# geometrian/simple-spectral

Hardware: AMD Instinct MI355X
Metric: Msamples/s (w*h*spp/s) cornell-srgb 512x512 (higher is better)
Workload: dtype f32

## Files before the change

include/ssx.h:

```cpp
#ifndef SSX_H
#define SSX_H

#include <stddef.h>
#include <stdint.h>

#ifdef __cplusplus
extern "C" {
#endif

#define SSX_ABI_VERSION 2

enum {
	SSX_OK = 0,
	SSX_ERR_DATA = -1,
	SSX_ERR_ARG = -2,
	SSX_ERR_SCENE = -3,
	SSX_ERR_DEVICE = -10,
	SSX_ERR_STATE = -11
};

#define SSX_MAX_DEPTH 10u
#define SSX_TILE_SIZE 8u
#define SSX_SAMPLE_WAVELENGTHS 4u
#define SSX_MAX_TEXTURES 64u
// ... 86 lines not shown
enum { SSX_LIBM_BUILD = 0, SSX_LIBM_GLIBC_2_35 = 1 };


typedef struct ssx_ctx ssx_ctx;

int ssx_create(int device, ssx_ctx** out);
void ssx_destroy(ssx_ctx* ctx);

int ssx_upload_scene(ssx_ctx* ctx, const ssx_scene_desc* scene);

int ssx_render_start(ssx_ctx* ctx, const ssx_render_params* params);
int ssx_render_stop(ssx_ctx* ctx);
int ssx_is_rendering(ssx_ctx* ctx);
float ssx_progress(ssx_ctx* ctx);
uint32_t ssx_done_spp(ssx_ctx* ctx);
uint32_t ssx_done_tiles(ssx_ctx* ctx);
int ssx_render_wait(ssx_ctx* ctx, float* xyza_out);

int ssx_render_device(ssx_ctx* ctx, const ssx_render_params* params, void* d_xyza_out, void* hip_stream);
int ssx_render_device_wait(ssx_ctx* ctx);

void* ssx_device_framebuffer(ssx_ctx* ctx);
int ssx_device_index(ssx_ctx* ctx);
int ssx_read_framebuffer(ssx_ctx* ctx, float* xyza_out);
int ssx_accumulate_peer(ssx_ctx* ctx, void* d_dst, int src_device, const void* d_src, uint32_t width, uint32_t height, void* hip_stream);

int ssx_reduce_rccl(ssx_ctx** ctxs, int n, uint32_t width, uint32_t height);
int ssx_rccl_probe(char* report, size_t report_size);
uint64_t ssx_rccl_groups_made(void);

const char* ssx_last_error(const ssx_ctx* ctx);

int ssx_set_timing(ssx_ctx* ctx, int enable);
int ssx_get_timing(ssx_ctx* ctx, float stage_ms[4]);

int ssx_abi_version(void);
int ssx_kernel_info(ssx_ctx* ctx, int* vgprs, int* sgprs, int* lds_bytes, int* scratch_bytes, int* max_blocks_per_cu);
int ssx_plan_info(ssx_ctx* ctx, float* frames_per_sample, int* fold_in_path_kernel);
int ssx_calibration_info(ssx_ctx* ctx, float* frames_per_sample, float* rays_left_per_sample, int* camera_rays_pretraced);
int ssx_scratch_info(ssx_ctx* ctx, uint64_t* sample_bytes, uint64_t* log_bytes);
int ssx_sums_info(ssx_ctx* ctx, uint64_t* units_parked, uint64_t* units_chained);
int ssx_units_info(ssx_ctx* ctx, uint64_t* units_enqueued);
int ssx_generate_info(ssx_ctx* ctx, uint64_t* generate_launches, uint64_t* fused_launches);
int ssx_kernel_variant(ssx_ctx* ctx);
enum { SSX_JIT_OFF = 0, SSX_JIT_AT_UPLOAD = 1, SSX_JIT_BACKGROUND = 2 };
int ssx_set_jit(ssx_ctx* ctx, int mode);
enum { SSX_JIT_STATE_NONE = 0,
       SSX_JIT_STATE_GENERIC_MEANWHILE = 1,
       SSX_JIT_STATE_SPECIALISED = 2,
       SSX_JIT_STATE_FAILED = -1 };
int ssx_jit_status(ssx_ctx* ctx, int wait_ms, char* message, size_t message_size);
void ssx_jit_counters(uint64_t* compiled, uint64_t* disk_hits);
const char* ssx_kernel_name(ssx_ctx* ctx);


int ssx_render_continue(ssx_ctx* ctx, uint32_t spp_more);

typedef struct ssx_sums_info_t {
	uint32_t struct_size;
	uint32_t width, height;
	uint32_t done_spp;
	uint64_t seed;
	uint32_t indirect_only, no_explicit_light_sampling, no_flat_field_correction, libm;
	uint32_t rgb_mode;
	uint32_t tile_first, tile_stride, tile_skew;
	uint32_t noise_batches;
	uint32_t reserved;
	uint64_t scene_digest;
} ssx_sums_info_t;
uint64_t ssx_scene_digest(ssx_ctx* ctx);
int ssx_sums_export(ssx_ctx* ctx, ssx_sums_info_t* info, double* sums, double* noise_s2);
int ssx_sums_import(ssx_ctx* ctx, const ssx_render_params* params, const ssx_sums_info_t* info, const double* sums, const double* noise_s2);

int ssx_set_noise_estimate(ssx_ctx* ctx, int enable);
int ssx_noise_info(ssx_ctx* ctx, double* v_out, double summary[4]);


int ssx_set_spectral_bins(ssx_ctx* ctx, uint32_t bins);
typedef struct ssx_spectral_info_t {
	uint32_t struct_size;
	uint32_t width, height;
	uint32_t bins;
	uint32_t done_spp;
	uint32_t reserved;
	float lambda_min;
	float bin_width;
} ssx_spectral_info_t;
int ssx_spectral_read(ssx_ctx* ctx, ssx_spectral_info_t* info, float* mean, double* sums, uint32_t* counts);
int ssx_spectral_import(ssx_ctx* ctx, const ssx_spectral_info_t* info, const double* sums , const uint32_t* counts );


int ssx_guides(ssx_ctx* ctx, uint32_t width, uint32_t height, uint32_t* prim, float* depth, float* normal, float* albedo);
typedef struct ssx_denoise_params {
	uint32_t struct_size;
	uint32_t levels;
	float sigma_l, sigma_a;
} ssx_denoise_params;
int ssx_denoise_images(ssx_ctx* ctx, const ssx_denoise_params* params, uint32_t width, uint32_t height, const float* xyza, const float* var,
                       const uint32_t* prim, const float* albedo, float* xyza_out, float* var_out);
int ssx_denoise(ssx_ctx* ctx, const ssx_denoise_params* params, float* xyza_out, float* var_out);


int ssx_denoise_channels(ssx_ctx* ctx, const ssx_denoise_params* params, uint32_t width, uint32_t height, const float* xyza, const float* var,
                         const uint32_t* prim, const float* albedo, uint32_t channels, const float* extra ,
                         float* xyza_out, float* var_out, float* extra_out );
int ssx_denoise_spectral(ssx_ctx* ctx, const ssx_denoise_params* params, float* mean_out , float* xyza_out, float* var_out);
// ... 204 lines not shown
```

simple_spectral_amd/_capi.py:

```python
import ctypes as C
import os

from . import build as _build


class SsxSpectrum(C.Structure):
    _fields_ = [("offset", C.c_uint32), ("n", C.c_uint32), ("low", C.c_float), ("high", C.c_float),
                ("delta_recip", C.c_float)]


class SsxVertex(C.Structure):
    _fields_ = [("pos", C.c_float * 3), ("st", C.c_float * 2)]


class SsxQuad(C.Structure):
    _fields_ = [("v00", SsxVertex), ("v10", SsxVertex), ("v11", SsxVertex), ("v01", SsxVertex),
                ("normal0", C.c_float * 3), ("normal1", C.c_float * 3),
                ("material", C.c_uint32), ("flags", C.c_uint32)]


class SsxMaterial(C.Structure):
    _fields_ = [("kind", C.c_uint32), ("albedo_mode", C.c_uint32), ("albedo_spectrum", C.c_uint32),
                ("albedo_texture", C.c_uint32), ("emission_spectrum", C.c_uint32)]

# ... 47 lines not shown
    _fields_ = [("struct_size", C.c_uint32), ("width", C.c_uint32), ("height", C.c_uint32), ("bins", C.c_uint32), ("done_spp", C.c_uint32),
                ("reserved", C.c_uint32), ("lambda_min", C.c_float), ("bin_width", C.c_float)]


class SsxDemodParams(C.Structure):
    _fields_ = [("struct_size", C.c_uint32), ("supersample", C.c_uint32), ("albedo_floor", C.c_float)]


SSX_DEMOD_DEFAULT_SUPERSAMPLE, SSX_DEMOD_DEFAULT_FLOOR, SSX_DEMOD_DEFAULT_SIGMA_L = 2, 0.0625, 1.0


class SsxDenoiseParams(C.Structure):
    _fields_ = [("struct_size", C.c_uint32), ("levels", C.c_uint32), ("sigma_l", C.c_float), ("sigma_a", C.c_float)]


class SsxOpticsParams(C.Structure):
    _fields_ = [("struct_size", C.c_uint32), ("cx", C.c_float), ("cy", C.c_float), ("max_radius", C.c_uint32),
                ("scale", C.c_void_p), ("radius", C.c_void_p), ("taps", C.c_void_p)]


SSX_OPTICS_MAX_RADIUS = 12


class SsxDefocusParams(C.Structure):
    _fields_ = [("struct_size", C.c_uint32), ("max_radius", C.c_uint32), ("gain", C.c_float), ("focus", C.c_void_p)]


SSX_DEFOCUS_MAX_RADIUS = 12


class SsxSensorParams(C.Structure):
    _fields_ = [("struct_size", C.c_uint32), ("cfa", C.c_uint32 * 4), ("noise", C.c_uint32), ("seed", C.c_uint32), ("frame", C.c_uint32),
                ("exposure", C.c_float), ("inv_exposure", C.c_float), ("read_var", C.c_float), ("dn_per_e", C.c_float), ("e_per_dn", C.c_float),
                ("black", C.c_float), ("white", C.c_float), ("weights", C.c_void_p), ("taps", C.c_void_p), ("ccm", C.c_void_p)]


SSH_DEMOSAIC_BILINEAR, SSH_DEMOSAIC_MHC = 0, 1


class SshSpectrum(C.Structure):
    _fields_ = [("samples", C.POINTER(C.c_float)), ("n", C.c_uint32), ("low", C.c_float), ("high", C.c_float)]


SSH_SPACE_XYZ, SSH_SPACE_LRGB = 0, 1
SSX_LIBM_BUILD, SSX_LIBM_GLIBC_2_35 = 0, 1
LIBM_MODES = {"build": SSX_LIBM_BUILD, "glibc-2.35": SSX_LIBM_GLIBC_2_35}


SSX_MODE_RGB, SSX_UPLIFT_OURS, SSX_UPLIFT_MENG, SSX_UPLIFT_JH = 0, 1, 2, 3
SSX_PRIM_LIGHT, SSX_PRIM_TRI = 1, 0x100
SSX_OK, SSX_ERR_DATA, SSX_ERR_ARG, SSX_ERR_SCENE, SSX_ERR_DEVICE, SSX_ERR_STATE = 0, -1, -2, -3, -10, -11
SSX_ABI_VERSION = 2
SSX_JIT_OFF, SSX_JIT_AT_UPLOAD, SSX_JIT_BACKGROUND = 0, 1, 2
SSX_JIT_STATE_NONE, SSX_JIT_STATE_GENERIC_MEANWHILE, SSX_JIT_STATE_SPECIALISED, SSX_JIT_STATE_FAILED = 0, 1, 2, -1

HIP_SYMBOLS = ["ssx_create", "ssx_destroy", "ssx_upload_scene", "ssx_render_start", "ssx_render_stop",
               "ssx_is_rendering", "ssx_progress", "ssx_render_wait", "ssx_render_device", "ssx_last_error",
               "ssx_abi_version", "ssx_kernel_info", "ssx_plan_info", "ssx_set_timing", "ssx_get_timing",
               "ssx_device_framebuffer", "ssx_device_index", "ssx_read_framebuffer", "ssx_accumulate_peer",
               "ssx_debug_eval", "ssx_debug_samples", "ssx_debug_sweep", "ssx_kernel_variant", "ssx_kernel_name", "ssx_scratch_info", "ssx_calibration_info", "ssx_set_jit", "ssx_debug_pass1_source", "ssx_done_spp", "ssx_reduce_rccl", "ssx_sums_info", "ssx_rccl_groups_made", "ssx_jit_status", "ssx_jit_counters", "ssx_done_tiles", "ssx_render_device_wait", "ssx_units_info", "ssx_rccl_probe",
               "ssx_render_continue", "ssx_scene_digest", "ssx_sums_export", "ssx_sums_import", "ssx_set_noise_estimate", "ssx_noise_info",
               "ssx_set_spectral_bins", "ssx_spectral_read", "ssx_debug_sample_flux",
               "ssx_guides", "ssx_denoise_images", "ssx_denoise", "ssx_denoise_channels", "ssx_denoise_spectral",
               "ssx_develop_images", "ssx_spectral_develop",
               "ssx_albedo_bins", "ssx_denoise_spectral_demod", "ssx_spectral_develop_demod",
               "ssx_spectral_import",
               "ssx_set_spectral_moments", "ssx_spectral_variance", "ssx_spectral_probe", "ssx_probe_arrays",
               "ssx_spectral_noise", "ssx_spectral_noise_reduce",
               "ssx_spectral_moments_import",
               "ssx_spectral_compare", "ssx_spectral_compare_arrays",
               "ssx_delta_e_images", "ssx_spectral_delta_e",
               "ssx_optics_images", "ssx_spectral_develop_optics",
               "ssx_defocus_images", "ssx_spectral_develop_lens",
               "ssx_sensor_images", "ssx_demosaic_images", "ssx_spectral_develop_sensor",
               "ssx_debug_tile_mask", "ssx_debug_spectral_accumulate", "ssx_debug_fold", "ssx_debug_step",
               "ssx_debug_generate", "ssx_generate_info"]
SSX_GENERATE_FILL_BYTE = 0xA6
SSX_FOLD_ROW_WORDS, SSX_FOLD_LAMBDA0, SSX_FOLD_CAM_DIR, SSX_FOLD_HIT, SSX_FOLD_N, SSX_FOLD_LEVEL0, SSX_FOLD_LEVEL_WORDS = 160, 0, 1, 4, 5, 10, 15
SSX_FOLD_L_FS, SSX_FOLD_L_NDL, SSX_FOLD_L_PDF, SSX_FOLD_L_FLAGS, SSX_FOLD_L_EMISSION, SSX_FOLD_L_NEE = 0, 4, 5, 6, 7, 11
SSX_FOLD_EMISSION, SSX_FOLD_NEE, SSX_FOLD_NEE_VISIBLE = 1, 2, 4
SSX_STEP_ROW_WORDS, SSX_STEP_R_ORIG, SSX_STEP_R_DIR, SSX_STEP_R_IGNORE, SSX_STEP_R_DEPTH, SSX_STEP_R_LAMBDA0, SSX_STEP_R_RNG, SSX_STEP_R_PREV_SLOT = 16, 0, 3, 6, 7, 8, 9, 13
SSX_STEP_NO_SLOT, SSX_STEP_OUT_WORDS = 0x1FFF, 40
(SSX_STEP_O_FLAGS, SSX_STEP_O_HIT_TRI, SSX_STEP_O_HIT_DIST, SSX_STEP_O_HIT_ST, SSX_STEP_O_EMISSION, SSX_STEP_O_NEE, SSX_STEP_O_NEE_TERM, SSX_STEP_O_FS, SSX_STEP_O_NDL,
 SSX_STEP_O_PDF, SSX_STEP_O_PREV_SLOT, SSX_STEP_O_TAIL_DEPTH, SSX_STEP_O_TAIL_HIT, SSX_STEP_O_NEXT_ORIG, SSX_STEP_O_NEXT_DIR, SSX_STEP_O_NEXT_IGNORE,
 SSX_STEP_O_NEXT_DEPTH, SSX_STEP_O_RNG, SSX_STEP_O_SLOT) = 0, 1, 2, 3, 5, 9, 13, 17, 21, 22, 23, 24, 25, 26, 29, 32, 33, 34, 36
SSX_STEP_HIT, SSX_STEP_CONTINUED, SSX_STEP_EMISSION, SSX_STEP_PARKED, SSX_STEP_VISIBLE = 1, 2, 4, 8, 16
(SSX_SWEEP_RCP, SSX_SWEEP_SQRT, SSX_SWEEP_INVERSESQRT, SSX_SWEEP_SIN, SSX_SWEEP_COS, SSX_SWEEP_ACOS, SSX_SWEEP_DIV_PI,
 SSX_SWEEP_RCP64, SSX_SWEEP_DIV_PAIRS, SSX_SWEEP_ACOS_SIN, SSX_SWEEP_SIN_PROOF, SSX_SWEEP_COS_PROOF, SSX_SWEEP_ACOS_PROOF) = range(1, 14)
(SSX_DBG_FMATH, SSX_DBG_SPHTRI, SSX_DBG_ARVO, SSX_DBG_SAMPLE_LIGHT, SSX_DBG_COSHEMI, SSX_DBG_TRACE, SSX_DBG_RAND_CHOICE,
 SSX_DBG_ALBEDO, SSX_DBG_FLUX_TO_XYZ, SSX_DBG_RAND_1F) = range(1, 11)
(SSX_DBG_GLIBC_MATH, SSX_DBG_SPHTRI_GLIBC, SSX_DBG_ARVO_GLIBC, SSX_DBG_SAMPLE_LIGHT_GLIBC, SSX_DBG_COSHEMI_GLIBC) = range(11, 16)
(SSX_SWEEP_GLIBC_SIN, SSX_SWEEP_GLIBC_COS, SSX_SWEEP_GLIBC_ACOS, SSX_SWEEP_GLIBC_COS_LDS) = range(14, 18)
SSX_DBG_TRACE_TOPO = 17
SSX_DBG_TRACE_MASKED = 16
HOST_SYMBOLS = ["ssh_scene_create", "ssh_scene_create_ex", "ssh_scene_destroy", "ssh_scene_desc", "ssh_xyza_to_srgba", "ssh_save_image",
                "ssh_load_png_rgb8", "ssh_free", "ssh_color_values", "ssh_last_error", "ssh_checkpoint_save", "ssh_checkpoint_load", "ssh_sums_merge", "ssh_save_npy_f32",
                "ssh_develop_weights", "ssh_relight_gain", "ssh_emitter_spectrum",
                "ssh_checkpoint_save_spectral", "ssh_checkpoint_load_spectral", "ssh_spectral_merge",
                "ssh_probe_derive", "ssh_probe_save_csv", "ssh_spectral_noise_derive", "ssh_spectral_noise_save_csv",
                "ssh_checkpoint_save_moments", "ssh_checkpoint_load_moments", "ssh_moments_merge",
                "ssh_compare_derive", "ssh_compare_save_csv",
                "ssh_delta_e_derive", "ssh_delta_e_save_csv", "ssh_develop_white",
                "ssh_optics_lens", "ssh_defocus_thin_lens", "ssh_scene_vfov",
                "ssh_sensor_bayer", "ssh_sensor_exposure", "ssh_sensor_ccm", "ssh_sensor_standin_curve"]

_hip = None
_host = None


def host_lib():
    global _host
    if _host is None:
        path = _build.HOST_LIB
        if not os.path.exists(path):
            _build.build_host()
        lib = C.CDLL(path)
        vp = C.c_void_p
        lib.ssh_last_error.restype = C.c_char_p
        lib.ssh_scene_create.argtypes = [C.c_char_p, C.c_char_p, C.c_int, vp, C.c_uint32, C.c_uint32, C.c_char_p,
                                         C.c_float, C.POINTER(vp)]
        lib.ssh_scene_create_ex.argtypes = [C.c_char_p, C.c_char_p, C.c_int, vp, C.c_uint32, C.c_uint32, C.c_char_p,
                                            C.c_float, C.c_uint32, C.c_char_p, C.c_uint32, C.POINTER(vp)]
        lib.ssh_scene_destroy.argtypes = [vp]
        lib.ssh_scene_desc.restype = C.POINTER(SsxSceneDesc)
        lib.ssh_scene_desc.argtypes = [vp]
        lib.ssh_xyza_to_srgba.argtypes = [vp, vp, vp, C.c_size_t]
        lib.ssh_save_image.argtypes = [C.c_char_p, vp, C.c_uint32, C.c_uint32]
        lib.ssh_load_png_rgb8.argtypes = [C.c_char_p, C.POINTER(C.POINTER(C.c_uint8)), C.POINTER(C.c_uint32),
                                          C.POINTER(C.c_uint32)]
# ... 183 lines not shown
            lib.ssx_denoise.argtypes = [vp, C.POINTER(SsxDenoiseParams), vp, vp]
        if not override or hasattr(lib, "ssx_denoise_spectral"):
            lib.ssx_denoise_channels.argtypes = [vp, C.POINTER(SsxDenoiseParams), C.c_uint32, C.c_uint32, vp, vp, vp, vp, C.c_uint32, vp, vp, vp, vp]
            lib.ssx_denoise_spectral.argtypes = [vp, C.POINTER(SsxDenoiseParams), vp, vp, vp]
        if not override or hasattr(lib, "ssx_spectral_develop"):
            lib.ssx_develop_images.argtypes = [vp, C.c_uint32, C.c_uint32, C.c_uint32, vp, vp, C.c_uint32, vp]
            lib.ssx_spectral_develop.argtypes = [vp, C.POINTER(SsxDenoiseParams), vp, C.c_uint32, vp]
        if not override or hasattr(lib, "ssx_albedo_bins"):
            lib.ssx_albedo_bins.argtypes = [vp, C.c_uint32, C.c_uint32, C.c_uint32, C.c_uint32, vp]
            lib.ssx_denoise_spectral_demod.argtypes = [vp, C.POINTER(SsxDenoiseParams), C.POINTER(SsxDemodParams), vp, vp, vp, vp]
            lib.ssx_spectral_develop_demod.argtypes = [vp, C.POINTER(SsxDenoiseParams), C.POINTER(SsxDemodParams), vp, vp, C.c_uint32, vp]
        if not override or hasattr(lib, "ssx_spectral_import"):
            lib.ssx_spectral_import.argtypes = [vp, C.POINTER(SsxSpectralInfo), vp, vp]
        if not override or hasattr(lib, "ssx_set_spectral_moments"):
            lib.ssx_set_spectral_moments.argtypes = [vp, C.c_int]
            lib.ssx_spectral_variance.argtypes = [vp, C.POINTER(SsxSpectralInfo), vp, vp]
            lib.ssx_spectral_probe.argtypes = [vp, vp, C.c_uint32, vp, vp, vp, vp]
            lib.ssx_probe_arrays.argtypes = [vp, C.c_uint32, C.c_uint32, C.c_uint32, vp, vp, vp, vp, C.c_uint32, vp, vp, vp, vp]
        if not override or hasattr(lib, "ssx_spectral_noise"):
            lib.ssx_spectral_noise.argtypes = [vp] * 10
            lib.ssx_spectral_noise_reduce.argtypes = [vp, C.c_uint32, C.c_uint32] + [vp] * 8
        if not override or hasattr(lib, "ssx_spectral_compare"):
            lib.ssx_spectral_compare.argtypes = [vp, C.POINTER(SsxSpectralInfo), vp, vp, vp, vp, C.c_uint32, C.c_double] + [vp] * 8
            lib.ssx_spectral_compare_arrays.argtypes = [vp, C.c_uint32, C.c_uint32, C.c_uint32] + [vp] * 7 + [C.c_uint32, C.c_double] + [vp] * 8
        if not override or hasattr(lib, "ssx_delta_e_images"):
            lib.ssx_delta_e_images.argtypes = [vp, C.c_uint32, C.c_uint32] + [vp] * 5 + [C.c_uint32] + [vp] * 9
            lib.ssx_spectral_delta_e.argtypes = [vp, C.POINTER(SsxDenoiseParams), C.c_int, C.c_int] + [vp] * 5 + [C.c_uint32] + [vp] * 9
        if not override or hasattr(lib, "ssx_optics_images"):
            lib.ssx_optics_images.argtypes = [vp, C.c_uint32, C.c_uint32, C.c_uint32, vp, C.POINTER(SsxOpticsParams), vp]
            lib.ssx_spectral_develop_optics.argtypes = [vp, C.POINTER(SsxDenoiseParams), C.POINTER(SsxOpticsParams), vp, C.c_uint32, vp, vp]
        if not override or hasattr(lib, "ssx_defocus_images"):
            lib.ssx_defocus_images.argtypes = [vp, C.c_uint32, C.c_uint32, C.c_uint32, vp, vp, C.POINTER(SsxDefocusParams), vp]
            lib.ssx_spectral_develop_lens.argtypes = [vp, C.POINTER(SsxDenoiseParams), C.POINTER(SsxDefocusParams), C.POINTER(SsxOpticsParams), vp, C.c_uint32, vp, vp]
        if not override or hasattr(lib, "ssx_sensor_images"):
            lib.ssx_sensor_images.argtypes = [vp, C.c_uint32, C.c_uint32, C.c_uint32, vp, C.POINTER(SsxSensorParams), vp, vp]
            lib.ssx_demosaic_images.argtypes = [vp, C.c_uint32, C.c_uint32, vp, C.POINTER(SsxSensorParams), vp]
            lib.ssx_spectral_develop_sensor.argtypes = [vp, C.POINTER(SsxDenoiseParams), C.POINTER(SsxDefocusParams), C.POINTER(SsxOpticsParams), C.POINTER(SsxSensorParams), vp, vp, vp]
        if not override or hasattr(lib, "ssx_spectral_moments_import"):
            lib.ssx_spectral_moments_import.argtypes = [vp, C.POINTER(SsxSpectralInfo), vp]
        if not override or hasattr(lib, "ssx_debug_tile_mask"):
            lib.ssx_debug_tile_mask.argtypes = [vp, C.POINTER(SsxRenderParams), vp]
        if not override or hasattr(lib, "ssx_debug_spectral_accumulate"):
            lib.ssx_debug_spectral_accumulate.argtypes = [vp] + [C.c_uint32] * 6 + [C.c_float, C.c_float, C.c_uint32] + [vp] * 6
        if not override or hasattr(lib, "ssx_debug_fold"):
            lib.ssx_debug_fold.argtypes = [vp, C.POINTER(SsxRenderParams), C.c_uint32, C.c_uint32, vp, C.c_uint32, C.c_uint32, vp, vp, vp]
        if not override or hasattr(lib, "ssx_debug_step"):
            lib.ssx_debug_step.argtypes = [vp, C.POINTER(SsxRenderParams), C.c_uint32, C.c_uint32, vp, vp]
        if not override or hasattr(lib, "ssx_debug_generate"):
            lib.ssx_debug_generate.argtypes = [vp, C.POINTER(SsxRenderParams), C.c_uint32, C.c_uint32, C.c_int, vp, vp, vp]
            lib.ssx_generate_info.argtypes = [vp, C.POINTER(C.c_uint64), C.POINTER(C.c_uint64)]
        lib.ssx_kernel_variant.argtypes = [vp]
        lib.ssx_kernel_name.argtypes = [vp]
        lib.ssx_kernel_name.restype = C.c_char_p
        _hip = lib
    return _hip
```

simple_spectral_amd/csrc/ssx_api.hip:

```cpp
#include "ssx_kernels.hip"
#include "ssx_debug.hip"

#include "../../include/ssx.h"

#include <chrono>
#include <array>
#include <atomic>
#include <cstdarg>
#include <cstdio>
#include <cstdlib>
#include <cmath>
#include <algorithm>
#include <cstring>
#include <mutex>
#include <string>
#include <thread>
#include <vector>

#include <limits.h>
#include <set>

#include "ssx_jit.h"

namespace {
// ... 5 lines not shown
	if (!m || m[0] != '1' || m[1] != '\0') return nullptr;
	return getenv(name);
}
bool env_on(const char* name) { const char* e = debug_env(name); return e && e[0] != '\0' && e[0] != '0'; }

std::string fmt(const char* f, ...) {
	char buf[512];
	va_list ap; va_start(ap, f); vsnprintf(buf, sizeof buf, f, ap); va_end(ap);
	return buf;
}

struct DeviceBuffer {
	void* ptr = nullptr;
	size_t bytes = 0;
	DeviceBuffer() = default;
	DeviceBuffer(DeviceBuffer&& o) noexcept : ptr(o.ptr), bytes(o.bytes) { o.ptr = nullptr; o.bytes = 0; }
	DeviceBuffer& operator=(DeviceBuffer&& o) noexcept { std::swap(ptr, o.ptr); std::swap(bytes, o.bytes); return *this; }
	~DeviceBuffer() { release(); }
	void release() { if (ptr) (void)hipFree(ptr); ptr = nullptr; bytes = 0; }
	hipError_t reserve(size_t n) {
		if (n <= bytes) return hipSuccess;
		release();
		const hipError_t e = hipMalloc(&ptr, n);
		if (e == hipSuccess) bytes = n; else ptr = nullptr;
		return e;
	}
	template <class T> T* as() const { return static_cast<T*>(ptr); }
};

}

#include "ssx_pack.h"

struct ssx_ctx {
	int device = 0;
	int n_cus = 0;
	hipStream_t stream = nullptr;
	DeviceBuffer d_blob;
	uint32_t blob_words = 0;
	uint32_t path_blob_words = 0;
	uint32_t topology = 0;
	int jit_mode = SSX_JIT_BACKGROUND;
	const ssx_jit::Kernels* jit_kernels[ssx_jit::kVariants] = {};
	uint32_t libm = SSX_LIBM_BUILD;
	uint32_t variant = SSX_LIBM_BUILD;
	bool jit_pending = false, jit_requested = false;
	ssx_jit::VidTable jit_vid;
	DeviceBuffer d_blob_jit; uint32_t blob_jit_words = 0, path_blob_jit_words = 0;
	uint64_t generic_samples = 0;
	int jit_state = SSX_JIT_STATE_NONE; std::string jit_message;
	std::vector<DeviceBuffer> d_textures;
	DeviceBuffer d_jh_data;
	bool rgb_mode = false;
	bool fuse_resolve = true;
	float calib_frames = 0.0f;
	float calib_left = 0.0f;
	bool pre_hits = false;
	DeviceBuffer d_accum;
	DeviceBuffer d_unit_counter;
	int resident_blocks = 0;
	int gen_blocks = 0;
	uint32_t max_wave_slots = 0;
	uint32_t queue_words = SSX_QUEUE_WORDS_WIDE;
	DeviceBuffer d_samples;
	DeviceBuffer d_logs;
	DeviceBuffer d_out;
	DeviceBuffer d_peer;
	bool have_scene = false;
	bool have_cam_dir = false;

	std::thread worker;
	std::atomic<int> rendering{0};
	std::atomic<int> stop_flag{0};
	std::atomic<uint32_t> done_spp{0};
	std::atomic<uint32_t> done_tiles{0};
	uint32_t total_spp = 0;
	int worker_rc = 0;
	std::atomic<uint64_t> units_enqueued{0};
	std::atomic<uint64_t> launches_generated{0}, launches_fused{0};
	ssx_render_params cur{};
	struct SumsState { bool continuable = false, noise_valid = false, spectral_valid = false, moments_valid = false, imported = false, spectral_imported = false; uint32_t noise_batches = 0; } sums;
	uint32_t k_begin = 0;
	uint64_t scene_digest = 0;
	bool noise_on = false;
	DeviceBuffer d_noise;
	DeviceBuffer d_stage;
	uint32_t spectral_bins = 0;
	DeviceBuffer d_spectral_sums, d_spectral_counts;
	std::string spectral_note;
	float lambda_min = 0.0f, lambda_step = 0.0f;
	uint32_t n_quads = 0;
	bool spectral_moments = false;
	DeviceBuffer d_spectral_moments, d_probe;
	std::string moments_note;
	DeviceBuffer d_guides, d_denoise, d_denoise_channels;
	DeviceBuffer d_develop;
	DeviceBuffer d_optics;
	DeviceBuffer d_defocus;
	DeviceBuffer d_sensor;
	uint32_t guides_width = 0, guides_height = 0;
	DeviceBuffer d_albedo_bins, d_demod;
	uint32_t abins_width = 0, abins_height = 0, abins_bins = 0, abins_supersample = 0;
	uint64_t abins_serial = 0;
	const void* demod_rc_base = nullptr; uint64_t demod_rc_bins_serial = 0; float demod_rc_floor = 0.0f; std::vector<float> demod_rc_weights;

	bool timing = false;
// ... 47 lines not shown
int begin_render(ssx_ctx* ctx, const ssx_render_params* in, ssx_render_params* out, const char* busy) {
	const int rc = take_params(ctx, in, out);
	if (rc) return rc;
	return ctx->rendering.load() ? fail(ctx, SSX_ERR_STATE, busy) : SSX_OK;
}

int wait_device_pending(ssx_ctx* ctx) {
	if (ctx->device_pending) { SSX_HIP(ctx, hipEventSynchronize(ctx->ev_device_done)); ctx->device_pending = false; }
	return SSX_OK;
}

int idle_on_device(ssx_ctx* ctx) {
	if (ctx->rendering.load()) return fail(ctx, SSX_ERR_STATE, "render in progress");
	SSX_HIP(ctx, hipSetDevice(ctx->device));
	return wait_device_pending(ctx);
}

uint32_t tiles_across(uint32_t pixels) { return (pixels + 7u) / 8u; }
size_t accum_bytes(uint32_t width, uint32_t height) { return (size_t)tiles_across(width) * tiles_across(height) * 64u * 4 * sizeof(double); }
size_t image_bytes(uint32_t width, uint32_t height) { return (size_t)width * height * 4 * sizeof(float); }

SsxPixelGrid pixel_grid(const ssx_render_params* p) {
	const uint32_t tx = tiles_across(p->width);
	return SsxPixelGrid{ p->width, p->height, tx, p->tile_first, p->tile_stride, p->tile_skew % tx };
}
uint32_t owned_tiles(const ssx_render_params& p) {
	const uint32_t n_tiles = tiles_across(p.width) * tiles_across(p.height);
	return n_tiles > p.tile_first ? (n_tiles - p.tile_first + p.tile_stride - 1u) / p.tile_stride : 0u;
}
dim3 pixel_blocks(const ssx_render_params* p) { return dim3((p->width * p->height + 255u) / 256u); }

int clear_sums(ssx_ctx* ctx, uint32_t width, uint32_t height, hipStream_t stream) {
	SSX_HIP(ctx, hipMemsetAsync(ctx->d_accum.ptr, 0, accum_bytes(width, height), stream));
	return SSX_OK;
}
void sums_invalidate(ssx_ctx* ctx) { ctx->sums = ssx_ctx::SumsState{}; }
void sums_publish(ssx_ctx* ctx, uint32_t done_spp, int64_t noise_batches = -1) {
	if (noise_batches >= 0) { ctx->sums.noise_valid = true; ctx->sums.noise_batches = (uint32_t)noise_batches; }
	ctx->done_spp.store(done_spp); ctx->sums.continuable = true;
}

constexpr size_t kSampleBufferBudget = (size_t)16 << 30;
size_t bytes_per_sample(const ssx_ctx* ctx) { return ctx->spectral_bins ? SSX_BYTES_PER_SAMPLE_FLUX : SSX_BYTES_PER_SAMPLE; }
constexpr size_t kAuxWordsPer64Records = 5;
size_t bytes_per_64_records(const ssx_ctx* ctx) { return 64u * bytes_per_sample(ctx) + kAuxWordsPer64Records * sizeof(uint32_t); }
size_t sample_bytes(const ssx_ctx* ctx, size_t records) { return records / 64u * bytes_per_64_records(ctx); }
size_t sample_slots(const ssx_ctx* ctx) { return ctx->d_samples.bytes / bytes_per_64_records(ctx) * 64u; }
size_t log_records(const ssx_ctx* ctx) { return ctx->d_logs.bytes / SSX_LOG_BYTES_PER_RECORD; }
constexpr uint32_t kMinUnits = 3072;
constexpr uint64_t kSamplesPerSync = (uint64_t)32 << 20;

struct LaunchPlan { SsxKernelArgs args; uint32_t max_spp_per_launch; };

LaunchPlan make_plan(ssx_ctx* ctx, const ssx_render_params* p, bool ask_device = true) {
	LaunchPlan pl{};
	SsxKernelArgs& a = pl.args;
	a.blob = ctx->d_blob.as<uint32_t>(); a.blob_words = ctx->path_blob_words;
	a.width = p->width; a.height = p->height;
	a.inv_width = 1.0 / (double)p->width; a.inv_height = 1.0 / (double)p->height;
	a.tiles_x = tiles_across(p->width);
	a.n_tiles = a.tiles_x * tiles_across(p->height);
	a.tile_first = p->tile_first; a.tile_stride = p->tile_stride; a.tile_skew = p->tile_skew % a.tiles_x;
	a.indirect_only = p->indirect_only ? 1u : 0u;
	a.no_els = p->no_explicit_light_sampling ? 1u : 0u;
	a.no_flat_field = p->no_flat_field_correction ? 1u : 0u;
	a.seed = p->seed;
	a.rgb_mode = ctx->rgb_mode ? 1u : 0u;
	a.fuse_resolve = ctx->fuse_resolve ? 1u : 0u;
	a.pre_hits = ctx->pre_hits ? 1u : 0u;
	a.my_tiles = owned_tiles(*p);
	size_t per_spp = (size_t)(a.my_tiles ? a.my_tiles : 1u) * 64u * bytes_per_sample(ctx);
	size_t budget = kSampleBufferBudget, free_b = 0, total_b = 0;
	if (ask_device && hipMemGetInfo(&free_b, &total_b) == hipSuccess) {
		const size_t avail = (size_t)((double)(free_b + sample_slots(ctx) * bytes_per_sample(ctx)) * 0.8);
		if (avail < budget) budget = avail;
	}
	size_t cap = budget / per_spp;
	const size_t idx_cap = (size_t)0xFFFFFFFFu / ((size_t)(a.my_tiles ? a.my_tiles : 1u) * 64u);
	if (cap > idx_cap) cap = idx_cap;
	pl.max_spp_per_launch = (uint32_t)(cap < 1 ? 1 : (cap > 65536 ? 65536 : cap));
	return pl;
}

void cap_to_allocation(const ssx_ctx* ctx, LaunchPlan& pl) {
	const size_t per_spp = (size_t)(pl.args.my_tiles ? pl.args.my_tiles : 1u) * 64u;
	const size_t fit = sample_slots(ctx) / per_spp;
	if (fit >= 1 && fit < pl.max_spp_per_launch) pl.max_spp_per_launch = (uint32_t)fit;
}

int ensure_samples(ssx_ctx* ctx, const LaunchPlan& pl, uint32_t n_k) {
	const size_t need = (size_t)pl.args.my_tiles * 64u * n_k;
	const hipError_t e = ctx->d_samples.reserve(sample_bytes(ctx, need));
	if (e == hipErrorOutOfMemory) { (void)hipGetLastError(); return fail(ctx, SSX_ERR_DEVICE, fmt("out of device memory for %zu samples in flight; lower spp_per_launch", need)); }
	SSX_HIP(ctx, e);
	return SSX_OK;
}

int ensure_logs(ssx_ctx* ctx, uint32_t unit_cohorts) {
	const size_t need = (size_t)ctx->max_wave_slots * 2u * unit_cohorts * SSX_COHORT_RECORDS, bytes = need * SSX_LOG_BYTES_PER_RECORD;
	if (bytes >= ((size_t)1 << 32)) return fail(ctx, SSX_ERR_DEVICE, "level logs beyond 4 GiB: the kernels address them with 32-bit offsets");
	if (ctx->d_logs.bytes >= bytes) return SSX_OK;
	if (ctx->d_logs.ptr) {
		const int rc = wait_device_pending(ctx);
		if (rc) return rc;
		SSX_HIP(ctx, hipStreamSynchronize(ctx->stream));
	}
// ... 39 lines not shown
	return SSX_OK;
}

struct Batch { SsxKernelArgs a; uint32_t units; uint64_t n_rec; hipEvent_t* tev; int rc; };

uint32_t unit_spp_of(const ssx_ctx* ctx) { return ctx->calib_frames >= 2.0f ? SSX_MAX_UNIT_KS / 2u : SSX_MAX_UNIT_KS; }

Batch make_batch(ssx_ctx* ctx, const LaunchPlan& pl, uint32_t k0, uint32_t k1) {
	Batch b{};
	b.a = pl.args;
	SsxKernelArgs& a = b.a;
	const uint32_t n_k = k1 - k0;
	a.k0 = k0; a.k1 = k1;
	a.n_records = (uint64_t)a.my_tiles * n_k * 64u;
	uint32_t g = unit_spp_of(ctx);
	while (g > 1u && (uint64_t)((n_k + g - 1u) / g) * a.my_tiles < kMinUnits) g >>= 1;
	a.group_spp = g;
	if (a.group_spp > n_k) a.group_spp = n_k;
	a.unit_cohorts = (a.group_spp + SSX_COHORT_KS - 1u) / SSX_COHORT_KS;
	a.unit_grab = ctx->calib_frames >= 2.0f ? 1u : 4u;
	if (a.unit_grab < 1u || a.unit_grab > 32u || a.group_spp == 0u || a.unit_cohorts == 0u) {
		b.rc = fail(ctx, SSX_ERR_STATE, fmt("internal: launch with unit_grab = %u (1..32), group_spp = %u, unit_cohorts = %u", a.unit_grab, a.group_spp, a.unit_cohorts));
		return b;
	}
	a.n_groups = (n_k + a.group_spp - 1) / a.group_spp;
	b.units = a.my_tiles * a.n_groups;
	b.n_rec = a.n_records;
	b.rc = ensure_logs(ctx, a.unit_cohorts);
	if (b.rc == SSX_OK) bind_arrays(a, ctx->d_samples.as<uint8_t>(), a.n_records, ctx->d_logs.as<uint8_t>(), log_records(ctx), ctx->spectral_bins != 0u);
	a.accum = ctx->d_accum.as<double>();
	uint32_t* const aux = reinterpret_cast<uint32_t*>(ctx->d_samples.as<uint8_t>() + sample_slots(ctx) * bytes_per_sample(ctx));
	a.unit_state = aux;
	a.tile_mask = aux + b.units;
	if (b.rc == SSX_OK && (size_t)a.my_tiles * 4u + b.units > (sample_slots(ctx) / 64u) * kAuxWordsPer64Records) b.rc = fail(ctx, SSX_ERR_STATE, "internal: launch larger than the sample allocation");
	return b;
}

size_t staged_blob_lds(uint32_t blob_words) { return ((size_t)blob_words + SSX_LDS_PREFIX_WORDS) * 4; }
size_t path_lds_bytes(uint32_t blob_words, uint32_t queue_words) {
	size_t n = staged_blob_lds(blob_words) + 4u * ((size_t)SSX_QUEUE_ENTRIES * queue_words + SSX_WAVE_COUNTER_WORDS) * 4u;
#ifdef SSX_REGTIME
	n += 4u * SSX_NTIME * 8u;
#endif
	return n;
}
struct PathKernel { const char* name; void (*host)(SsxKernelArgs); };
#define SSX_PK(k) { #k, k }
static const PathKernel kPathKernels[ssx_jit::kVariants][3][2] = {
	{ { SSX_PK(ssx_render_kernel), SSX_PK(ssx_render_kernel_nq) }, { SSX_PK(ssx_render_kernel_cornell), SSX_PK(ssx_render_kernel_cornell_nq) },
	  { SSX_PK(ssx_render_kernel_plane), SSX_PK(ssx_render_kernel_plane_nq) } },
	{ { SSX_PK(ssx_render_kernel_glibc), SSX_PK(ssx_render_kernel_nq_glibc) }, { SSX_PK(ssx_render_kernel_cornell_glibc), SSX_PK(ssx_render_kernel_cornell_nq_glibc) },
	  { SSX_PK(ssx_render_kernel_plane_glibc), SSX_PK(ssx_render_kernel_plane_nq_glibc) } },
	{ { SSX_PK(ssx_render_kernel_flux), SSX_PK(ssx_render_kernel_nq_flux) }, { SSX_PK(ssx_render_kernel_cornell_flux), SSX_PK(ssx_render_kernel_cornell_nq_flux) },
	  { SSX_PK(ssx_render_kernel_plane_flux), SSX_PK(ssx_render_kernel_plane_nq_flux) } } };
#undef SSX_PK
static const char* const kJitKernelNames[2] = { "ssx_render_kernel_jit", "ssx_render_kernel_jit_nq" };
const PathKernel& path_kernel_of(const ssx_ctx* ctx, bool narrow) { return kPathKernels[ctx->variant][ctx->topology < 3u ? ctx->topology : 0u][narrow]; }
struct KernelRef { const void* host = nullptr; hipFunction_t mod = nullptr; };
KernelRef path_kernel_ref(const ssx_ctx* ctx, bool narrow) {
	KernelRef k;
	const ssx_jit::Kernels* jk = ctx->jit_kernels[ctx->variant];
	if (ctx->topology == 3u && jk) k.mod = narrow ? jk->path_nq : jk->path;
	else k.host = (const void*)path_kernel_of(ctx, narrow).host;
	return k;
}
int occupancy_of(ssx_ctx* ctx, const KernelRef& k, size_t lds, int* per_cu) {
	if (k.mod) SSX_HIP(ctx, hipModuleOccupancyMaxActiveBlocksPerMultiprocessor(per_cu, k.mod, 256, lds));
	else SSX_HIP(ctx, hipOccupancyMaxActiveBlocksPerMultiprocessor(per_cu, k.host, 256, lds));
	return SSX_OK;
}
int blocks_that_fit(ssx_ctx* ctx, const KernelRef& k, size_t lds, int* blocks) {
	int per_cu = 0;
	const int rc = occupancy_of(ctx, k, lds, &per_cu);
	if (rc) return rc;
	*blocks = (per_cu > 0 ? per_cu : 1) * ctx->n_cus;
	return SSX_OK;
}
int launch_kernel(ssx_ctx* ctx, const KernelRef& k, uint32_t blocks, size_t lds, hipStream_t stream, SsxKernelArgs& a) {
	if (k.mod) {
		size_t size = sizeof a;
		void* config[] = { HIP_LAUNCH_PARAM_BUFFER_POINTER, &a, HIP_LAUNCH_PARAM_BUFFER_SIZE, &size, HIP_LAUNCH_PARAM_END };
		SSX_HIP(ctx, hipModuleLaunchKernel(k.mod, blocks, 1, 1, 256, 1, 1, (unsigned)lds, stream, nullptr, config));
	} else {
		void* args[] = { &a };
		SSX_HIP(ctx, hipLaunchKernel(k.host, dim3(blocks), dim3(256), args, lds, stream));
	}
	return SSX_OK;
}
int pick_queue(ssx_ctx* ctx, uint32_t blob_words, uint32_t* queue_words, int* blocks_per_cu) {
	int wide = 0, narrow = 0, rc;
	if (path_lds_bytes(blob_words, SSX_QUEUE_WORDS_WIDE) <= 65536u)
		if ((rc = occupancy_of(ctx, path_kernel_ref(ctx, false), path_lds_bytes(blob_words, SSX_QUEUE_WORDS_WIDE), &wide))) return rc;
	if ((rc = occupancy_of(ctx, path_kernel_ref(ctx, true), path_lds_bytes(blob_words, SSX_QUEUE_WORDS_NARROW), &narrow))) return rc;
	const bool use_narrow = narrow > wide || env_on("SSX_NARROW_QUEUE");
	*queue_words = use_narrow ? SSX_QUEUE_WORDS_NARROW : SSX_QUEUE_WORDS_WIDE;
	if (blocks_per_cu) *blocks_per_cu = use_narrow ? narrow : wide;
	return SSX_OK;
}

bool fuses_generate(const ssx_ctx* ctx, const SsxKernelArgs& a) {
	const char* fuse_env = debug_env("SSX_FUSE_GEN");
	const bool tiles_fit = a.tiles_x <= 0xFFFFu && tiles_across(a.height) <= 0xFFFFu;
	return ctx->topology == 2u && !a.pre_hits && tiles_fit && !(fuse_env && fuse_env[0] == '0');
}

int enqueue_generate(ssx_ctx* ctx, const Batch& b, hipStream_t stream) {
	SsxKernelArgs ga = b.a;
	ga.blob_words = ctx->blob_words;
	if (ga.pre_hits) {
		hipLaunchKernelGGL(ssx_tile_mask_kernel, dim3((ga.my_tiles + 3u) / 4u), dim3(256), 0, stream, ga);
		SSX_HIP(ctx, hipGetLastError());
	}
	const KernelRef gen_kernel{ (const void*)ssx_generate_kernel };
	const size_t gen_lds = staged_blob_lds(ga.blob_words);
	if (ctx->gen_blocks == 0) { const int rc = blocks_that_fit(ctx, gen_kernel, gen_lds, &ctx->gen_blocks); if (rc) return rc; }
	const uint64_t want = (b.n_rec + 255u) / 256u;
	return launch_kernel(ctx, gen_kernel, (uint32_t)(want < (uint64_t)ctx->gen_blocks ? want : (uint64_t)ctx->gen_blocks), gen_lds, stream, ga);
}

int enqueue_path(ssx_ctx* ctx, Batch& b, const KernelRef& kernel, uint32_t queue_words, uint32_t blob_words, int resident_blocks, hipStream_t stream) {
	if (!ctx->d_unit_counter.ptr) {
		SSX_HIP(ctx, ctx->d_unit_counter.reserve(4 * sizeof(uint32_t)));
		SSX_HIP(ctx, hipMemsetAsync(ctx->d_unit_counter.ptr, 0, 4 * sizeof(uint32_t), stream));
	}
	b.a.blob_words = blob_words; b.a.queue_words = queue_words;
	SSX_HIP(ctx, hipMemsetAsync(ctx->d_unit_counter.ptr, 0, 2 * sizeof(uint32_t), stream));
	SSX_HIP(ctx, hipMemsetAsync(b.a.unit_state, 0, (size_t)b.units * sizeof(uint32_t), stream));
	b.a.unit_counter = ctx->d_unit_counter.as<uint32_t>();
	const uint32_t want_blocks = (b.units + 3u) / 4u;
	uint32_t blocks = want_blocks < (uint32_t)resident_blocks ? want_blocks : (uint32_t)resident_blocks;
	if (blocks * 4u > ctx->max_wave_slots) blocks = ctx->max_wave_slots / 4u;
	return launch_kernel(ctx, kernel, blocks, path_lds_bytes(blob_words, queue_words), stream, b.a);
}

int launch_batch(ssx_ctx* ctx, Batch& b, hipStream_t stream) {
	if (b.rc) return b.rc;
	int rc;
	if (ctx->timing) { if ((rc = timing_events(ctx, &b.tev))) return rc; SSX_HIP(ctx, hipEventRecord(b.tev[0], stream)); }
	b.a.fuse_gen = fuses_generate(ctx, b.a) ? 1u : 0u;
	if (!b.a.fuse_gen && (rc = enqueue_generate(ctx, b, stream))) return rc;
	if (ctx->timing) SSX_HIP(ctx, hipEventRecord(b.tev[1], stream));
	const bool plan = ctx->resident_blocks == 0;
	if (plan && (rc = pick_queue(ctx, b.a.blob_words, &ctx->queue_words, nullptr))) return rc;
	const KernelRef path_kernel = path_kernel_ref(ctx, ctx->queue_words == SSX_QUEUE_WORDS_NARROW);
	if (plan && (rc = blocks_that_fit(ctx, path_kernel, path_lds_bytes(b.a.blob_words, ctx->queue_words), &ctx->resident_blocks))) return rc;
	if ((rc = enqueue_path(ctx, b, path_kernel, ctx->queue_words, b.a.blob_words, ctx->resident_blocks, stream))) return rc;
	ctx->units_enqueued.fetch_add(b.units);
	(b.a.fuse_gen ? ctx->launches_fused : ctx->launches_generated).fetch_add(1u);
	if (ctx->timing) for (int k = 2; k < 6; ++k) SSX_HIP(ctx, hipEventRecord(b.tev[k], stream));
	return SSX_OK;
}

constexpr uint64_t kJitAfterSamples = kSamplesPerSync;
void maybe_swap_jit(ssx_ctx* ctx, uint64_t samples) {
	if (!ctx->jit_pending) return;
	std::string err;
	const ssx_jit::Kernels* k = nullptr;
	const ssx_jit::State st = ssx_jit::lookup(ctx->device, ctx->jit_vid, &k, &err, ctx->variant);
	if (st == ssx_jit::State::Ready) {
		std::swap(ctx->d_blob, ctx->d_blob_jit);
		ctx->blob_words = ctx->blob_jit_words; ctx->path_blob_words = ctx->path_blob_jit_words;
		ctx->topology = 3u;
		ctx->jit_kernels[ctx->variant] = k;
		ctx->resident_blocks = 0; ctx->gen_blocks = 0;
		ctx->jit_pending = false; ctx->jit_state = SSX_JIT_STATE_SPECIALISED;
	} else if (st == ssx_jit::State::Failed) {
		ctx->jit_pending = false; ctx->jit_state = SSX_JIT_STATE_FAILED; ctx->jit_message = err;
	} else {
		ctx->generic_samples += samples;
		if (!ctx->jit_requested && ctx->generic_samples >= kJitAfterSamples) { ssx_jit::request(ctx->jit_vid, ctx->variant); ctx->jit_requested = true; }
	}
}

int ensure_libm_kernels(ssx_ctx* ctx, uint32_t libm) {
	const ssx_jit::Kernels*& have = ctx->jit_kernels[libm];
	if (ctx->topology != 3u || have) return SSX_OK;
	std::string err;
	const ssx_jit::Kernels* k = ssx_jit::get(ctx->device, ctx->jit_vid, &err, libm);
	if (!k) return fail(ctx, SSX_ERR_STATE, "the scene's specialised kernels for this libm could not be compiled: " + err);
	have = k;
	return SSX_OK;
}

int ready_to_launch(ssx_ctx* ctx, const ssx_render_params* p, bool need_out) {
	const uint32_t variant = (ctx->spectral_bins && p->libm == SSX_LIBM_BUILD && !ctx->rgb_mode) ? ssx_jit::kVariantFlux : p->libm;
	const int rc = ensure_libm_kernels(ctx, variant);
	if (rc) return rc;
	ctx->libm = p->libm;
	if (ctx->variant != variant) { ctx->variant = variant; ctx->resident_blocks = 0; ctx->jit_requested = false; }
	SSX_HIP(ctx, ctx->d_accum.reserve(accum_bytes(p->width, p->height)));
	if (need_out) SSX_HIP(ctx, ctx->d_out.reserve(image_bytes(p->width, p->height)));
	return SSX_OK;
}

int launch_range(ssx_ctx* ctx, LaunchPlan& pl, uint32_t k0, uint32_t k1, hipStream_t stream) {
	if (pl.args.my_tiles == 0 || k1 <= k0) return SSX_OK;
	Batch b = make_batch(ctx, pl, k0, k1);
	return launch_batch(ctx, b, stream);
}

int launch_batches(ssx_ctx* ctx, LaunchPlan& pl, uint32_t spp, uint32_t batch, hipStream_t stream) {
	for (uint32_t k0 = 0; k0 < spp; k0 += batch) {
		int rc = launch_range(ctx, pl, k0, (spp - k0 < batch) ? spp : k0 + batch, stream);
		if (rc) return rc;
	}
	return SSX_OK;
}

int calibrate(ssx_ctx* ctx) {
	ssx_render_params cp{};
	cp.struct_size = sizeof cp; cp.width = 64; cp.height = 64; cp.spp = 4; cp.tile_stride = 1;
	ctx->fuse_resolve = false;
	ctx->pre_hits = false;
	LaunchPlan pl = make_plan(ctx, &cp);
	int rc = ensure_samples(ctx, pl, cp.spp);
	if (rc) return rc;
	Batch b = make_batch(ctx, pl, 0, cp.spp);
	if (b.rc) return b.rc;
	if ((rc = enqueue_generate(ctx, b, ctx->stream))) return rc;
	const KernelRef kernel{ (const void*)ssx_calibrate_kernel };
	int blocks = 0;
	if ((rc = blocks_that_fit(ctx, kernel, path_lds_bytes(ctx->blob_words, SSX_QUEUE_WORDS_NARROW), &blocks))) return rc;
	if ((rc = enqueue_path(ctx, b, kernel, SSX_QUEUE_WORDS_NARROW, ctx->blob_words, blocks, ctx->stream))) return rc;
	SSX_HIP(ctx, hipStreamSynchronize(ctx->stream));
	std::vector<uint4> recs((size_t)b.n_rec);
	SSX_HIP(ctx, hipMemcpy(recs.data(), b.a.st, recs.size() * sizeof(uint4), hipMemcpyDeviceToHost));
	uint64_t frames = 0;
	for (const uint4& r : recs) frames += (r.y >> 2) & 0xFu;
	ctx->calib_frames = (float)((double)frames / (double)recs.size());
	uint32_t counters[2] = { 0u, 0u };
	SSX_HIP(ctx, hipMemcpy(counters, ctx->d_unit_counter.ptr, sizeof counters, hipMemcpyDeviceToHost));
	ctx->calib_left = (float)((double)counters[1] / (double)recs.size());
	ctx->pre_hits = ctx->calib_left >= 0.3f;
	if (const char* e = debug_env("SSX_PRE_HITS")) { if (e[0] != '\0') ctx->pre_hits = e[0] != '0'; }
	ctx->fuse_resolve = true;
	return ensure_logs(ctx, (unit_spp_of(ctx) + SSX_COHORT_KS - 1u) / SSX_COHORT_KS);
}

// ... 235 lines not shown
	if ((e = hipSetDevice(device)) != hipSuccess || (e = hipStreamCreateWithFlags(&ctx->stream, hipStreamNonBlocking)) != hipSuccess) {
		g_create_error = hipGetErrorString(e);
		delete ctx;
		return SSX_ERR_DEVICE;
	}
	*out = ctx;
	return SSX_OK;
}

void ssx_destroy(ssx_ctx* ctx) {
	if (!ctx) return;
	if (ctx->worker.joinable()) { ctx->stop_flag.store(1); ctx->worker.join(); }
	(void)hipSetDevice(ctx->device);
	if (ctx->rccl_comm) { std::lock_guard<std::mutex> g(rccl_api().mutex); drop_rccl_comm(ctx); }
	if (ctx->ev_device_done) (void)hipEventDestroy(ctx->ev_device_done);
	for (hipEvent_t e : ctx->ev_pool) (void)hipEventDestroy(e);
	const hipStream_t stream = ctx->stream;
	delete ctx;
	if (stream) (void)hipStreamDestroy(stream);
}

int ssx_upload_scene(ssx_ctx* ctx, const ssx_scene_desc* s) {
	if (!ctx) return SSX_ERR_ARG;
	ssx_scene_desc local;
	bool have_cam_dir = true;
	if (s && (s->struct_size == offsetof(ssx_scene_desc, meng) || s->struct_size == offsetof(ssx_scene_desc, cam_dir))) {
		memset(&local, 0, sizeof local);
		memcpy(&local, s, s->struct_size);
		local.struct_size = sizeof(ssx_scene_desc);
		have_cam_dir = false;
		s = &local;
	}
	if (!s || s->struct_size != sizeof(ssx_scene_desc)) return fail(ctx, SSX_ERR_ARG, "ssx_scene_desc.struct_size mismatch");
	if (ctx->rendering.load()) return fail(ctx, SSX_ERR_STATE, "render in progress");
	SSX_HIP(ctx, hipSetDevice(ctx->device));
	SSX_HIP(ctx, hipDeviceSynchronize());
	ctx->device_pending = false;
	ctx->d_textures.clear();
	ctx->have_scene = false;
	sums_invalidate(ctx); ctx->scene_digest = 0;
	ctx->guides_width = ctx->guides_height = 0;
	ctx->abins_width = ctx->abins_height = 0;
	for (uint32_t i = 0; i < s->n_textures && i < SSX_MAX_TEXTURES; ++i) {
		const ssx_texture& t = s->textures[i];
		if (!t.rgb || t.width == 0 || t.height == 0) return fail(ctx, SSX_ERR_DATA, "Could not load texture");
		const size_t bytes = (size_t)3 * t.width * t.height;
		ctx->d_textures.emplace_back();
		SSX_HIP(ctx, ctx->d_textures.back().reserve(bytes));
		SSX_HIP(ctx, hipMemcpy(ctx->d_textures.back().ptr, t.rgb, bytes, hipMemcpyHostToDevice));
	}
	if (s->uplift != SSX_MODE_RGB && s->uplift != SSX_UPLIFT_OURS && s->uplift != SSX_UPLIFT_JH && s->uplift != SSX_UPLIFT_MENG)
		return fail(ctx, SSX_ERR_SCENE, "unsupported uplift variant (0 = RGB mode, 1 = basis, 2 = Meng et al., 3 = Jakob-Hanika)");
	ctx->rgb_mode = (s->uplift == SSX_MODE_RGB);
	ctx->d_jh_data.release();
	if (s->uplift == SSX_UPLIFT_MENG) {
		const ssx_meng_grid* g = s->meng;
		if (!g || !g->cells || !g->points || g->grid_w == 0 || g->grid_h == 0 || g->grid_w > 4096 || g->grid_h > 4096 ||
		    g->n_points == 0 || g->n_points > (1u << 20) || g->n_samples < 2 || g->n_samples > 4096 || !(g->sample_max > g->sample_min))
			return fail(ctx, SSX_ERR_DATA, "Meng grid missing or invalid");
		const size_t n_cells = (size_t)g->grid_w * g->grid_h;
		for (size_t c = 0; c < n_cells; ++c) {
			const int32_t* cell = g->cells + 8 * c;
			const int32_t inside = cell[0], num = cell[1];
			const bool shape_ok = inside ? (num == 4) : (num == 0 || (num >= 3 && num <= 6));
			if (!shape_ok) return fail(ctx, SSX_ERR_DATA, "Meng grid: cell with an unusable point count");
			for (int32_t k = 0; k < num; ++k) if (cell[2 + k] < 0 || (uint32_t)cell[2 + k] >= g->n_points) return fail(ctx, SSX_ERR_DATA, "Meng grid: point index out of range");
		}
		const size_t words = 16 + n_cells * 8 + (size_t)g->n_points * (4 + (size_t)g->n_samples);
		std::vector<uint32_t> tab(words, 0u);
		tab[0] = g->grid_w; tab[1] = g->grid_h; tab[2] = g->n_points; tab[3] = g->n_samples;
		memcpy(&tab[4], &g->sample_min, 4); memcpy(&tab[5], &g->sample_max, 4);
		memcpy(&tab[6], g->xy_to_uv, 24);
		memcpy(&tab[16], g->cells, n_cells * 32);
		memcpy(&tab[16 + n_cells * 8], g->points, (size_t)g->n_points * (4 + (size_t)g->n_samples) * 4);
		SSX_HIP(ctx, ctx->d_jh_data.reserve(words * 4));
		SSX_HIP(ctx, hipMemcpy(ctx->d_jh_data.ptr, tab.data(), words * 4, hipMemcpyHostToDevice));
	}
	if (s->uplift == SSX_UPLIFT_JH) {
		if (!s->jh_scale || !s->jh_data || s->jh_res < 2 || s->jh_res > 256) return fail(ctx, SSX_ERR_DATA, "Jakob-Hanika model missing or invalid");
		size_t bytes = (size_t)3 * s->jh_res * s->jh_res * s->jh_res * 3 * sizeof(float);
		SSX_HIP(ctx, ctx->d_jh_data.reserve(bytes));
		SSX_HIP(ctx, hipMemcpy(ctx->d_jh_data.ptr, s->jh_data, bytes, hipMemcpyHostToDevice));
	}
	std::vector<uint32_t> blob, blob_jit;
	for (auto& k : ctx->jit_kernels) k = nullptr;
	ctx->jit_pending = ctx->jit_requested = false; ctx->generic_samples = 0; ctx->jit_vid.clear();
	ctx->jit_state = SSX_JIT_STATE_NONE; ctx->jit_message.clear();
	ctx->d_blob_jit.release();
	std::vector<const void*> tex;
	for (const DeviceBuffer& t : ctx->d_textures) tex.push_back(t.ptr);
	PackInfo info;
	std::string pack_err;
	int rc = pack_blob(s, tex, ctx->d_jh_data.ptr, blob, pack_err, -1, &info);
	if (rc) return fail(ctx, rc, pack_err);
	const int jit_mode = env_on("SSX_JIT_PASS1") ? SSX_JIT_AT_UPLOAD : ctx->jit_mode;
	if (info.candidate && jit_mode != SSX_JIT_OFF) {
		std::string err;
		const ssx_jit::Kernels* k = nullptr;
		ssx_jit::State st = ssx_jit::lookup(ctx->device, info.vid, &k, &err);
		if (st != ssx_jit::State::Ready && st != ssx_jit::State::Failed && jit_mode == SSX_JIT_AT_UPLOAD) {
			k = ssx_jit::get(ctx->device, info.vid, &err);
			st = k ? ssx_jit::State::Ready : ssx_jit::State::Failed;
		}
		if (st == ssx_jit::State::Failed) { ctx->jit_state = SSX_JIT_STATE_FAILED; ctx->jit_message = err; }
		else if ((rc = pack_blob(s, tex, ctx->d_jh_data.ptr, blob_jit, pack_err, 3))) return fail(ctx, rc, pack_err);
		else if (st == ssx_jit::State::Ready) { blob.swap(blob_jit); blob_jit.clear(); ctx->jit_kernels[SSX_LIBM_BUILD] = k; ctx->jit_vid = info.vid; ctx->jit_state = SSX_JIT_STATE_SPECIALISED; }
		else { ctx->jit_pending = true; ctx->jit_vid = info.vid; ctx->jit_state = SSX_JIT_STATE_GENERIC_MEANWHILE; ctx->jit_requested = (st == ssx_jit::State::Pending); }
	}
	if (ctx->jit_pending) {
		SSX_HIP(ctx, ctx->d_blob_jit.reserve(blob_jit.size() * 4));
		SSX_HIP(ctx, hipMemcpy(ctx->d_blob_jit.ptr, blob_jit.data(), blob_jit.size() * 4, hipMemcpyHostToDevice));
		const SsxBlobHeader* bh = reinterpret_cast<const SsxBlobHeader*>(blob_jit.data());
		ctx->blob_jit_words = (uint32_t)blob_jit.size(); ctx->path_blob_jit_words = bh->words_without_perm;
	}
	SSX_HIP(ctx, ctx->d_blob.reserve(blob.size() * 4));
	SSX_HIP(ctx, hipMemcpy(ctx->d_blob.ptr, blob.data(), blob.size() * 4, hipMemcpyHostToDevice));
	ctx->blob_words = (uint32_t)blob.size();
	{
		SsxBlobHeader* bh = reinterpret_cast<SsxBlobHeader*>(blob.data());
		ctx->topology = bh->topology;
		ctx->path_blob_words = (bh->topology || bh->perm_hbm) ? bh->words_without_perm : ctx->blob_words;
		if (bh->perm_hbm) {
			const uint64_t at = (uint64_t)(uintptr_t)(ctx->d_blob.as<uint32_t>() + bh->off_perm);
			bh->perm_ptr_lo = (uint32_t)at; bh->perm_ptr_hi = (uint32_t)(at >> 32);
			SSX_HIP(ctx, hipMemcpy(ctx->d_blob.ptr, blob.data(), sizeof(SsxBlobHeader), hipMemcpyHostToDevice));
			ctx->blob_words = bh->words_without_perm;
		}
	}
	ctx->have_cam_dir = have_cam_dir;
	ctx->lambda_min = s->lambda_min; ctx->lambda_step = s->lambda_step;
	ctx->n_quads = s->n_quads;
	ctx->resident_blocks = 0; ctx->gen_blocks = 0;
	ctx->have_scene = true;
	ctx->scene_digest = scene_digest_of(s);
	return calibrate(ctx);
}

static uint32_t device_batch(const ssx_render_params* p, const LaunchPlan& pl) {
	uint32_t batch = p->spp_per_launch ? p->spp_per_launch : p->spp;
	if (batch > p->spp) batch = p->spp;
	if (batch > pl.max_spp_per_launch) {
		const uint32_t n = (p->spp + pl.max_spp_per_launch - 1u) / pl.max_spp_per_launch;
		batch = (p->spp + n - 1u) / n;
	}
	return batch;
}

int ssx_render_device(ssx_ctx* ctx, const ssx_render_params* p_in, void* d_xyza_out, void* hip_stream) {
	if (!ctx) return SSX_ERR_ARG;
	ssx_render_params pp;
	int rc = take_params(ctx, p_in, &pp);
	if (rc) return rc;
	const ssx_render_params* const p = &pp;
	if (!d_xyza_out) return fail(ctx, SSX_ERR_ARG, "d_xyza_out is NULL");
	if (ctx->spectral_bins) return fail(ctx, SSX_ERR_ARG, "spectral output is on (ssx_set_spectral_bins): ssx_render_device does not bin its samples; use ssx_render_start");
	if (ctx->rendering.load()) return fail(ctx, SSX_ERR_STATE, "asynchronous render in progress");
	hipStream_t stream = (hipStream_t)hip_stream;
	SSX_HIP(ctx, hipSetDevice(ctx->device));
	if (!ctx->ev_device_done) SSX_HIP(ctx, hipEventCreateWithFlags(&ctx->ev_device_done, hipEventDisableTiming));
	hipStreamCaptureStatus capture = hipStreamCaptureStatusNone;
	(void)hipStreamIsCapturing(stream, &capture);
	const bool capturing = capture == hipStreamCaptureStatusActive;
	if (ctx->device_pending && capturing) return fail(ctx, SSX_ERR_STATE, "a render of this context may still be queued: ssx_render_device_wait before capturing another into a graph");
	if (capturing && ctx->variant != p->libm) return fail(ctx, SSX_ERR_STATE, "ssx_render_params.libm differs from the context's last render: run it once outside the stream capture first");
	if (ctx->device_pending) SSX_HIP(ctx, hipStreamWaitEvent(stream, ctx->ev_device_done, 0));
	{
		LaunchPlan probe = make_plan(ctx, p, !capturing);
		if (capturing) cap_to_allocation(ctx, probe);
		const uint32_t probe_batch = device_batch(p, probe);
		const size_t need = (size_t)probe.args.my_tiles * 64u * probe_batch;
		const bool grow = ctx->d_accum.bytes < accum_bytes(p->width, p->height) || ctx->d_samples.bytes < sample_bytes(ctx, need);
		if (grow && capturing) return fail(ctx, SSX_ERR_STATE, "the context's buffers have to grow for this render: run it once outside the stream capture first");
		if (grow && (rc = wait_device_pending(ctx))) return rc;
	}
	if ((rc = ready_to_launch(ctx, p, false))) return rc;
	sums_invalidate(ctx);
	if ((rc = clear_sums(ctx, p->width, p->height, stream))) return rc;
	if (!capturing) maybe_swap_jit(ctx, (uint64_t)p->width * p->height * p->spp / p->tile_stride);
	LaunchPlan pl = make_plan(ctx, p, !capturing);
	if (capturing) cap_to_allocation(ctx, pl);
	const uint32_t batch = device_batch(p, pl);
	if ((rc = ensure_samples(ctx, pl, batch))) return rc;
	if ((rc = launch_batches(ctx, pl, p->spp, batch, stream))) return rc;
	if ((rc = launch_finalize(ctx, p, p->spp, (float*)d_xyza_out, stream))) return rc;
	if (!capturing) {
		SSX_HIP(ctx, hipEventRecord(ctx->ev_device_done, stream));
		ctx->device_pending = true;
	}
	return SSX_OK;
}

int ssx_render_device_wait(ssx_ctx* ctx) {
	if (!ctx) return SSX_ERR_ARG;
	if (!ctx->device_pending) return SSX_OK;
	SSX_HIP(ctx, hipSetDevice(ctx->device));
	return wait_device_pending(ctx);
}

int ssx_render_start(ssx_ctx* ctx, const ssx_render_params* p_in) {
	if (!ctx) return SSX_ERR_ARG;
	ssx_render_params pp;
	int rc = begin_render(ctx, p_in, &pp, "render already in progress");
	if (rc) return rc;
	SSX_HIP(ctx, hipSetDevice(ctx->device));
	if ((rc = wait_device_pending(ctx))) return rc;
	return start_worker(ctx, pp, 0, false, pp.spp);
}

int ssx_render_stop(ssx_ctx* ctx) {
	if (!ctx) return SSX_ERR_ARG;
	ctx->stop_flag.store(1);
	return SSX_OK;
}

int ssx_is_rendering(ssx_ctx* ctx) { return ctx ? ctx->rendering.load() : 0; }

float ssx_progress(ssx_ctx* ctx) {
// ... 85 lines not shown
		if (ctx->topology == 0u) return fail(ctx, SSX_ERR_STATE, "SSX_DBG_TRACE_TOPO: the context runs the generic trace (topology 0); that is SSX_DBG_TRACE");
		const uint32_t* d_rows = d_in.as<uint32_t>(); uint32_t* d_res = d_out.as<uint32_t>();
		void* args[] = { &a, &d_rows, &in_words, &d_res, &out_words, &n };
		if (ctx->topology == 3u) {
			std::string err;
			const ssx_jit::Kernels* k = ssx_jit::get(ctx->device, ctx->jit_vid, &err, ssx_jit::kVariantDebug);
			if (!k || !k->debug_trace) return fail(ctx, SSX_ERR_STATE, "SSX_DBG_TRACE_TOPO: the debug kernel of the scene's pattern could not be compiled: " + err);
			SSX_HIP(ctx, hipModuleLaunchKernel(k->debug_trace, (n + 255u) / 256u, 1, 1, 256, 1, 1, (unsigned)lds, ctx->stream, args, nullptr));
		} else {
			const void* host = ctx->topology == 1u ? (const void*)ssx_debug_trace_cornell_kernel : (const void*)ssx_debug_trace_plane_kernel;
			SSX_HIP(ctx, hipLaunchKernel(host, dim3((n + 255u) / 256u), dim3(256), args, lds, ctx->stream));
		}
		SSX_HIP(ctx, hipStreamSynchronize(ctx->stream));
		SSX_HIP(ctx, hipMemcpy(out, d_out.ptr, (size_t)n * out_words * 4, hipMemcpyDeviceToHost));
		return SSX_OK;
	}
	const auto kernel =op >= SSX_DBG_GLIBC_MATH && op <= SSX_DBG_COSHEMI_GLIBC ? ssx_debug_eval_glibc_kernel : ssx_debug_eval_kernel;
	hipLaunchKernelGGL(kernel, dim3((n + 255u) / 256u), dim3(256), lds, ctx->stream, a, op, d_in.as<uint32_t>(), in_words, d_out.as<uint32_t>(), out_words, n);
	SSX_HIP(ctx, hipGetLastError());
	SSX_HIP(ctx, hipStreamSynchronize(ctx->stream));
	SSX_HIP(ctx, hipMemcpy(out, d_out.ptr, (size_t)n * out_words * 4, hipMemcpyDeviceToHost));
	return SSX_OK;
}

int ssx_debug_sweep(ssx_ctx* ctx, uint32_t op, uint32_t lo, uint64_t count, uint64_t result[11]) {
	if (!ctx || !result || count == 0 || count > (1ull << 32)) return SSX_ERR_ARG;
	if (!ctx->have_scene) return fail(ctx, SSX_ERR_STATE, "no scene uploaded");
	if (ctx->rendering.load()) return fail(ctx, SSX_ERR_STATE, "render in progress");
	SSX_HIP(ctx, hipSetDevice(ctx->device));
	DeviceBuffer d_res;
	SSX_HIP(ctx, d_res.reserve(11 * sizeof(unsigned long long)));
	SSX_HIP(ctx, hipMemsetAsync(d_res.ptr, 0, 11 * sizeof(unsigned long long), ctx->stream));
	SsxKernelArgs a{};
	a.blob = ctx->d_blob.as<uint32_t>(); a.blob_words = ctx->blob_words;
	const size_t lds = staged_blob_lds(ctx->blob_words);
	const auto kernel = op >= SSX_SWEEP_GLIBC_SIN ? ssx_debug_sweep_glibc_kernel : ssx_debug_sweep_kernel;
	hipLaunchKernelGGL(kernel, dim3(256 * 16), dim3(256), lds, ctx->stream, a, op, lo, (uint64_t)count, d_res.as<unsigned long long>());
	SSX_HIP(ctx, hipGetLastError());
	SSX_HIP(ctx, hipStreamSynchronize(ctx->stream));
	SSX_HIP(ctx, hipMemcpy(result, d_res.ptr, 11 * sizeof(unsigned long long), hipMemcpyDeviceToHost));
	return SSX_OK;
}

int ssx_debug_samples(ssx_ctx* ctx, const ssx_render_params* p_in, float* xyza, uint64_t* rng_state, uint32_t* levels) {
	if (!ctx) return SSX_ERR_ARG;
	ssx_render_params pp;
	int rc = begin_render(ctx, p_in, &pp, "render in progress");
	if (rc) return rc;
	const ssx_render_params* const p = &pp;
	if (p->tile_first != 0 || p->tile_stride != 1) return fail(ctx, SSX_ERR_ARG, "ssx_debug_samples renders the whole image");
	if ((rc = spectral_refuses(ctx, pp, false))) return rc;
	SSX_HIP(ctx, hipSetDevice(ctx->device));
	if ((rc = wait_device_pending(ctx))) return rc;
	if ((rc = ready_to_launch(ctx, p, false))) return rc;
	LaunchPlan pl = make_plan(ctx, p);
	if (p->spp > pl.max_spp_per_launch) return fail(ctx, SSX_ERR_ARG, "ssx_debug_samples: too many samples for one launch");
	if ((rc = ensure_samples(ctx, pl, p->spp))) return rc;
	sums_invalidate(ctx);
	if ((rc = clear_sums(ctx, p->width, p->height, ctx->stream))) return rc;
	Batch b = make_batch(ctx, pl, 0, p->spp);
	b.a.keep_samples = 1u;
	if ((rc = launch_batch(ctx, b, ctx->stream))) return rc;
	SSX_HIP(ctx, hipStreamSynchronize(ctx->stream));
	std::vector<float4> ray((size_t)b.n_rec);
	std::vector<uint4> st((size_t)b.n_rec);
	SSX_HIP(ctx, hipMemcpy(ray.data(), b.a.ray, ray.size() * sizeof(float4), hipMemcpyDeviceToHost));
	SSX_HIP(ctx, hipMemcpy(st.data(), b.a.st, st.size() * sizeof(uint4), hipMemcpyDeviceToHost));
	const uint32_t spp = p->spp, tiles_x = tiles_across(p->width);
	for (uint32_t j = 0; j < p->height; ++j) for (uint32_t i = 0; i < p->width; ++i) {
		const uint32_t tile = (j >> 3) * tiles_x + (i >> 3), lane = (j & 7u) * 8u + (i & 7u);
		for (uint32_t k = 0; k < spp; ++k) {
			const size_t r = ((size_t)tile * spp + k) * 64u + lane, o = ((size_t)j * p->width + i) * spp + k;
			if (xyza) { xyza[4 * o + 0] = ray[r].x; xyza[4 * o + 1] = ray[r].y; xyza[4 * o + 2] = ray[r].z; xyza[4 * o + 3] = ray[r].w; }
			if (rng_state) rng_state[o] = ((uint64_t)st[r].w << 32) | st[r].z;
			if (levels) levels[o] = (st[r].y >> 2) & 0xFu;
		}
	}
	return SSX_OK;
}

int ssx_debug_tile_mask(ssx_ctx* ctx, const ssx_render_params* p_in, uint32_t* out) {
	if (!ctx || !out) return SSX_ERR_ARG;
	ssx_render_params pp;
	int rc = begin_render(ctx, p_in, &pp, "render in progress");
	if (rc) return rc;
	SSX_HIP(ctx, hipSetDevice(ctx->device));
	if ((rc = wait_device_pending(ctx))) return rc;
	const LaunchPlan pl = make_plan(ctx, &pp);
	SsxKernelArgs ga = pl.args;
	if (ga.my_tiles == 0u) return SSX_OK;
	ga.blob_words = ctx->blob_words;
	const size_t bytes = (size_t)ga.my_tiles * 4u * sizeof(uint32_t);
	DeviceBuffer d_mask;
	if (d_mask.reserve(bytes) != hipSuccess) { (void)hipGetLastError(); return fail(ctx, SSX_ERR_DEVICE, "out of device memory (ssx_debug_tile_mask)"); }
	ga.tile_mask = d_mask.as<uint32_t>();
	hipLaunchKernelGGL(ssx_tile_mask_kernel, dim3((ga.my_tiles + 3u) / 4u), dim3(256), 0, ctx->stream, ga);
	SSX_HIP(ctx, hipGetLastError());
	SSX_HIP(ctx, hipStreamSynchronize(ctx->stream));
	SSX_HIP(ctx, hipMemcpy(out, d_mask.ptr, bytes, hipMemcpyDeviceToHost));
	return SSX_OK;
}

int ssx_debug_generate(ssx_ctx* ctx, const ssx_render_params* p_in, uint32_t k0, uint32_t n_k, int pre_hits, float* ray, uint32_t* st, float* hit) {
	if (!ctx || !ray || !st) return SSX_ERR_ARG;
	ssx_render_params pp;
	int rc = begin_render(ctx, p_in, &pp, "render in progress");
	if (rc) return rc;
// ... 214 lines not shown
}

int ssx_calibration_info(ssx_ctx* ctx, float* frames_per_sample, float* rays_left_per_sample, int* camera_rays_pretraced) {
	if (!ctx) return SSX_ERR_ARG;
	if (!ctx->have_scene) return fail(ctx, SSX_ERR_STATE, "no scene uploaded");
	if (frames_per_sample) *frames_per_sample = ctx->calib_frames;
	if (rays_left_per_sample) *rays_left_per_sample = ctx->calib_left;
	if (camera_rays_pretraced) *camera_rays_pretraced = ctx->pre_hits ? 1 : 0;
	return SSX_OK;
}

int ssx_scratch_info(ssx_ctx* ctx, uint64_t* sample_bytes, uint64_t* log_bytes) {
	if (!ctx) return SSX_ERR_ARG;
	if (sample_bytes) *sample_bytes = (uint64_t)sample_slots(ctx) * bytes_per_sample(ctx) + (ctx->spectral_moments ? (uint64_t)ctx->d_spectral_moments.bytes : 0u);
	if (log_bytes) *log_bytes = (uint64_t)ctx->d_logs.bytes;
	return SSX_OK;
}

int ssx_sums_info(ssx_ctx* ctx, uint64_t* units_parked, uint64_t* units_chained) {
	if (!ctx) return SSX_ERR_ARG;
	uint32_t c[4] = { 0u, 0u, 0u, 0u };
	if (ctx->d_unit_counter.ptr) {
		SSX_HIP(ctx, hipSetDevice(ctx->device));
		const int rc = wait_device_pending(ctx);
		if (rc) return rc;
		SSX_HIP(ctx, hipMemcpy(c, ctx->d_unit_counter.ptr, sizeof c, hipMemcpyDeviceToHost));
	}
	if (units_parked) *units_parked = c[2];
	if (units_chained) *units_chained = c[3];
	return SSX_OK;
}

int ssx_units_info(ssx_ctx* ctx, uint64_t* units_enqueued) {
	if (!ctx) return SSX_ERR_ARG;
	if (units_enqueued) *units_enqueued = ctx->units_enqueued.load();
	return SSX_OK;
}

int ssx_generate_info(ssx_ctx* ctx, uint64_t* generate_launches, uint64_t* fused_launches) {
	if (!ctx) return SSX_ERR_ARG;
	if (generate_launches) *generate_launches = ctx->launches_generated.load();
	if (fused_launches) *fused_launches = ctx->launches_fused.load();
	return SSX_OK;
}

int ssx_kernel_variant(ssx_ctx* ctx) { return (ctx && ctx->have_scene) ? (int)ctx->topology : -1; }

const char* ssx_kernel_name(ssx_ctx* ctx) {
	if (!ctx || !ctx->have_scene) return nullptr;
	if (hipSetDevice(ctx->device) != hipSuccess) return nullptr;
	uint32_t qw = 0;
	if (pick_queue(ctx, ctx->path_blob_words, &qw, nullptr) != SSX_OK) return nullptr;
	const bool narrow = qw == SSX_QUEUE_WORDS_NARROW;
	return ctx->topology == 3u ? kJitKernelNames[narrow] : path_kernel_of(ctx, narrow).name;
}

int ssx_plan_info(ssx_ctx* ctx, float* frames_per_sample, int* fold_in_path_kernel) {
	if (!ctx) return SSX_ERR_ARG;
	if (!ctx->have_scene) return fail(ctx, SSX_ERR_STATE, "no scene uploaded");
	if (frames_per_sample) *frames_per_sample = ctx->calib_frames;
	if (fold_in_path_kernel) *fold_in_path_kernel = ctx->fuse_resolve ? 1 : 0;
	return SSX_OK;
}

int ssx_kernel_info(ssx_ctx* ctx, int* vgprs, int* sgprs, int* lds_bytes, int* scratch_bytes, int* max_blocks_per_cu) {
	if (!ctx) return SSX_ERR_ARG;
	SSX_HIP(ctx, hipSetDevice(ctx->device));
	hipFuncAttributes at;
	uint32_t qw = 0; int nb = 0;
	int r = pick_queue(ctx, ctx->path_blob_words, &qw, &nb);
	if (r) return r;
	const KernelRef k = path_kernel_ref(ctx, qw == SSX_QUEUE_WORDS_NARROW);
	if (k.mod) {
		int v = 0;
		SSX_HIP(ctx, hipFuncGetAttribute(&v, HIP_FUNC_ATTRIBUTE_NUM_REGS, k.mod)); at.numRegs = v;
		SSX_HIP(ctx, hipFuncGetAttribute(&v, HIP_FUNC_ATTRIBUTE_SHARED_SIZE_BYTES, k.mod)); at.sharedSizeBytes = (size_t)v;
		SSX_HIP(ctx, hipFuncGetAttribute(&v, HIP_FUNC_ATTRIBUTE_LOCAL_SIZE_BYTES, k.mod)); at.localSizeBytes = (size_t)v;
	} else SSX_HIP(ctx, hipFuncGetAttributes(&at, k.host));
	if (vgprs) *vgprs = at.numRegs;
	if (sgprs) *sgprs = 0;
	if (lds_bytes) *lds_bytes = (int)at.sharedSizeBytes + (int)path_lds_bytes(ctx->path_blob_words, qw);
	if (scratch_bytes) *scratch_bytes = (int)at.localSizeBytes;
	if (max_blocks_per_cu) *max_blocks_per_cu = nb;
	return SSX_OK;
}

}

#include "ssx_progressive.hip"
#include "ssx_spectral.hip"
#include "ssx_denoise.hip"
#include "ssx_develop.hip"
#include "ssx_optics.hip"
#include "ssx_defocus.hip"
#include "ssx_sensor.hip"
#include "ssx_demod.hip"
#include "ssx_spectral_stats.hip"
#include "ssx_spectral_noise.hip"
#include "ssx_spectral_compare.hip"
#include "ssx_delta_e.hip"
```

simple_spectral_amd/csrc/ssx_jit.h:

```cpp
#pragma once
#include <hip/hip_runtime.h>
#include <dlfcn.h>

#include <sys/stat.h>
#include <unistd.h>

#include <algorithm>
#include <array>
#include <chrono>
#include <condition_variable>
#include <cstdint>
#include <cstdio>
#include <cstdlib>
#include <cstring>
#include <deque>
#include <map>
#include <mutex>
#include <set>
#include <string>
#include <thread>
#include <utility>
#include <vector>

#include "ssx_sources_gen.h"
// ... 84 lines not shown
	void* lib = nullptr;
	typedef void* Program;
	int (*create)(Program*, const char*, const char*, int, const char**, const char**) = nullptr;
	int (*compile)(Program, int, const char**) = nullptr;
	int (*log_size)(Program, size_t*) = nullptr;
	int (*log)(Program, char*) = nullptr;
	int (*code_size)(Program, size_t*) = nullptr;
	int (*code)(Program, char*) = nullptr;
	int (*destroy)(Program*) = nullptr;
	bool open(std::string* err) {
		if (lib) return true;
		for (const char* name : { "libhiprtc.so.7", "libhiprtc.so", "/opt/rocm/lib/libhiprtc.so" }) if ((lib = dlopen(name, RTLD_NOW | RTLD_LOCAL))) break;
		if (!lib) { const char* why = dlerror(); *err = std::string("hipRTC is not available (") + (why ? why : "dlopen failed") + ")"; return false; }
		bool ok = true;
		auto sym = [&](const char* n) { void* s = dlsym(lib, n); ok = ok && s; return s; };
		create = (decltype(create))sym("hiprtcCreateProgram"); compile = (decltype(compile))sym("hiprtcCompileProgram");
		log_size = (decltype(log_size))sym("hiprtcGetProgramLogSize"); log = (decltype(log))sym("hiprtcGetProgramLog");
		code_size = (decltype(code_size))sym("hiprtcGetCodeSize"); code = (decltype(code))sym("hiprtcGetCode");
		destroy = (decltype(destroy))sym("hiprtcDestroyProgram");
		if (!ok) { *err = "hipRTC lacks an entry point"; dlclose(lib); lib = nullptr; }
		return ok;
	}
};

struct Kernels {
	hipModule_t module = nullptr;
	hipFunction_t path = nullptr, path_nq = nullptr;
	hipFunction_t debug_trace = nullptr;
};

enum class State { Missing, Pending, Ready, Failed };

inline uint64_t fnv64(const void* data, size_t n, uint64_t h = 0xCBF29CE484222325ull) {
	const unsigned char* p = static_cast<const unsigned char*>(data);
	for (size_t i = 0; i < n; ++i) { h ^= p[i]; h *= 0x100000001B3ull; }
	return h;
}

struct Shared {
	std::mutex m;
	std::condition_variable cv;
	std::map<std::string, std::string> code, errors;
	std::set<std::string> queued;
	std::deque<std::pair<std::string, std::pair<VidTable, uint32_t>>> jobs;
	bool worker_running = false;
	std::map<std::pair<int, std::string>, Kernels> modules;
	std::set<std::string> disk_missed;
	std::mutex rtc_mutex;
	Rtc rtc;
	uint64_t compiled = 0, disk_hits = 0;
};
inline Shared& shared() { static Shared* s = new Shared; return *s; }

constexpr uint32_t kVariantFlux = 2, kVariants = 3;
constexpr uint32_t kVariantDebug = 3;
inline std::string pattern_key(const VidTable& vids, uint32_t libm = 0) {
	std::string key;
	if (libm == 1u) key = "libm=glibc-2.35|";
	if (libm == kVariantFlux) key = "flux|";
	if (libm == kVariantDebug) key = "debug|";
	for (const auto& r : vids) key.append(reinterpret_cast<const char*>(r.data()), 4);
	return key;
}
inline const char* libm_flag(uint32_t libm) { return libm == kVariantDebug ? "-DSSX_JIT_DEBUG=1" : libm == kVariantFlux ? "-DSSX_JIT_FLUX=1" : libm ? "-DSSX_JIT_GLIBC=1" : nullptr; }

inline const char* const* compile_flags(size_t* n) {
	static const char* const flags[] = { "--offload-arch=gfx950", "-O3", "-std=c++17", "-ffp-contract=off", "-fno-slp-vectorize", "-DSSX_JIT_BUILD",
#ifdef SSX_ACCUM_FORMAL
		"-DSSX_ACCUM_FORMAL",
#endif
	};
	*n = sizeof flags / sizeof flags[0];
	return flags;
}

inline std::string cache_dir_name() {
	if (const char* e = getenv("SSX_CACHE_DIR")) return e;
	if (const char* x = getenv("XDG_CACHE_HOME")) if (x[0]) return std::string(x) + "/ssx";
	if (const char* h = getenv("HOME")) if (h[0]) return std::string(h) + "/.cache/ssx";
	return "";
}
inline std::string cache_dir() {
	const std::string dir = cache_dir_name();
	if (dir.empty()) return dir;
	struct stat st;
	if (lstat(dir.c_str(), &st) != 0) return dir;
	if (!S_ISDIR(st.st_mode) || st.st_uid != geteuid() || (st.st_mode & (S_IWGRP | S_IWOTH))) return "";
	return dir;
}
inline void cache_id(const std::string& key, const VidTable& vids, uint32_t libm, uint64_t id[2]) {
	static const std::pair<uint64_t, uint64_t> base = [] {
		uint64_t a = 0xCBF29CE484222325ull, b = 0x9E3779B97F4A7C15ull;
		const char* texts[] = { ssx_src_kernels_hip, ssx_src_blob_h, ssx_src_exact_h, ssx_src_lanestat_h, ssx_src_fmath_h, ssx_src_pass1_gen_h, ssx_src_glibc_math_h };
		for (const char* t : texts) { a = fnv64(t, strlen(t), a); b = fnv64(t, strlen(t), b); }
		size_t nf = 0; const char* const* flags = compile_flags(&nf);
		for (size_t i = 0; i < nf; ++i) { a = fnv64(flags[i], strlen(flags[i]) + 1, a); b = fnv64(flags[i], strlen(flags[i]) + 1, b); }
		int ver = 0;
		(void)hipRuntimeGetVersion(&ver);
		a = fnv64(&ver, sizeof ver, a); b = fnv64(&ver, sizeof ver, b);
		return std::make_pair(a, b);
	}();
	const std::string pass1 = pass1_source("jit", vids);
	uint64_t a = fnv64(key.data(), key.size(), base.first), b = fnv64(key.data(), key.size(), base.second);
	a = fnv64(pass1.data(), pass1.size(), a); b = fnv64(pass1.data(), pass1.size(), b);
	if (const char* lf = libm_flag(libm)) { a = fnv64(lf, strlen(lf) + 1, a); b = fnv64(lf, strlen(lf) + 1, b); }
	id[0] = a; id[1] = b;
}
inline std::string cache_file(const std::string& dir, const uint64_t id[2]) {
	char name[64];
	snprintf(name, sizeof name, "/pass1-%016llx%016llx.co", (unsigned long long)id[0], (unsigned long long)id[1]);
	return dir + name;
}
inline bool disk_load(const std::string& key, const VidTable& vids, uint32_t libm, std::string* obj) {
	const std::string dir = cache_dir();
	if (dir.empty()) return false;
	uint64_t id[2]; cache_id(key, vids, libm, id);
	FILE* f = fopen(cache_file(dir, id).c_str(), "rb");
// ... 170 lines not shown
```

simple_spectral_amd/csrc/ssx_kernels.hip:

```cpp
#include <hip/hip_runtime.h>
#ifndef __HIPCC_RTC__
#include <stdint.h>
#endif

#include "ssx_blob.h"
#include "ssx_exact.h"
#include "ssx_lanestat.h"
extern __shared__ __attribute__((aligned(16))) uint32_t ssx_lds[];
#define SSX_FM_TABLE (reinterpret_cast<const double*>(ssx_lds))
#ifdef SSX_JIT_BUILD
#include "ssx_fmath.h"
#else
#include "../../include/ssx_fmath.h"
#endif
#define SSX_GM_TABLE (SSX_FM_TABLE + SSX_FM_I_A11)
#ifdef SSX_JIT_BUILD
#include "ssx_glibc_math.h"
#else
#include "../../include/ssx_glibc_math.h"
#endif
__device__ const double ssx_fm_coeff_values[SSX_FM_N_COEFF] = SSX_FM_COEFF_INIT;
__device__ const double ssx_gm_coeff_values[SSX_GM_N_COEFF] = SSX_GM_COEFF_INIT;
static_assert(2 * SSX_FM_N_COEFF <= SSX_LDS_PREFIX_WORDS, "coefficient table");
static_assert(SSX_FM_I_A11 + SSX_GM_N_COEFF <= SSX_FM_N_COEFF, "glibc coefficients in the arc-cosine slots");
// ... 233 lines not shown
			const float area = e0x * e1y - e1x * e0y;
			const float u = uu / area, v = vv / area;
			const float w = 1.0f - u - v;
			if (u < 0.0f || v < 0.0f || w < 0.0f) { uu = -vv; e0x = e1x; e0y = e1y; continue; }
			pa = cell[2]; pb = cell[2 + i + 1]; pc = cell[2 + third];
			wa = w; wb = v; wc = u;
			found = true;
			break;
		}
	}
	if (!found) {
		return out;
	}
	const float* Sa = pts + stride * pa + 4;
	const float* Sb = pts + stride * pb + 4;
	const float* Sc = pts + stride * pc + 4;
	const float* Sd = pts + stride * pd + 4;
#pragma unroll
	for (int k = 0; k < 4; ++k) {
		const float lambda = lambda_0 + (float)k * h.lambda_step;
		const float sb = (lambda - smin) / (smax - smin) * (float)(ns - 1);
		const int sb0 = (int)sb;
		const int sb1 = (int)((sb + 1.0f < (float)ns) ? sb + 1.0f : (float)(ns - 1));
		const float sbf = sb - (float)sb0;
		const float qa = Sa[sb0] * (1.0f - sbf) + Sa[sb1] * sbf;
		const float qb = Sb[sb0] * (1.0f - sbf) + Sb[sb1] * sbf;
		const float qc = Sc[sb0] * (1.0f - sbf) + Sc[sb1] * sbf;
		float ip;
		if (inside) {
			const float qd = Sd[sb0] * (1.0f - sbf) + Sd[sb1] * sbf;
			const float u = wa, v = wb;
			ip = ((qa * (1.0f - u) * (1.0f - v) + qb * (1.0f - u) * v) + qc * u * v) + qd * u * (1.0f - v);
		} else {
			ip = (qa * wa + qb * wb) + qc * wc;
		}
		out.v[k] = ip / norm;
	}
	return out;
}

__device__ __forceinline__ void texel_lrgb(const Lds& L, uint32_t tex_index, float st_x, float st_y, float& r, float& g, float& b) {
	const SsxBlobTexture t = L.texture(tex_index);
	const uint8_t* rgb = reinterpret_cast<const uint8_t*>(((uint64_t)t.ptr_hi << 32) | (uint64_t)t.ptr_lo);
	float uvx = st_x * (float)t.w, uvy = st_y * (float)t.h;
	float index_x = uvx, index_y = (float)t.h - uvy;
	int i = (int)__builtin_floorf(index_x), j = (int)__builtin_floorf(index_y);
	int hi_i = (int)t.w - 1, hi_j = (int)t.h - 1;
	i = (i < 0) ? 0 : i; i = (hi_i < i) ? hi_i : i;
	j = (j < 0) ? 0 : j; j = (hi_j < j) ? hi_j : j;
	const uint8_t* px = rgb + 3u * ((size_t)j * (size_t)t.w + (size_t)i);
	r = L.lut(px[0]); g = L.lut(px[1]); b = L.lut(px[2]);
}

__device__ __forceinline__ Hero texture_sample(const Lds& L, uint32_t tex_index, float st_x, float st_y, float lambda_0) {
	float r, g, b;
	texel_lrgb(L, tex_index, st_x, st_y, r, g, b);
	const SsxBlobHeader& h = L.hdr();
	if (h.uplift == 0u) { Hero o; o.v[0] = r; o.v[1] = g; o.v[2] = b; o.v[3] = 0.0f; return o; }
	if (h.uplift == 3u) return jh_uplift(L, r, g, b, lambda_0);
	if (h.uplift == 2u) return meng_uplift(L, r, g, b, lambda_0);
	Hero br, bg, bb;
	const SsxBlobSpectrum sr = L.spectrum(h.spec_basis_r), sg = L.spectrum(h.spec_basis_g), sb = L.spectrum(h.spec_basis_b);
	if (h.basis_one_grid) {
		hero_gather3(L, h.off_basis4, hero_index(h, sr, lambda_0), br, bg, bb);
	} else {
		br = spectrum_hero(L, sr, lambda_0, h.lambda_step);
		bg = spectrum_hero(L, sg, lambda_0, h.lambda_step);
		bb = spectrum_hero(L, sb, lambda_0, h.lambda_step);
	}
	Hero out;
#pragma unroll
	for (int k = 0; k < 4; ++k) out.v[k] = (r * br.v[k] + g * bg.v[k]) + b * bb.v[k];
	return out;
}

__device__ __forceinline__ Hero material_albedo(const Lds& L, const SsxBlobQuad& Q, float st_x, float st_y, float lambda_0) {
	const SsxBlobHeader& h = L.hdr();
	if (h.uplift == 1u && h.basis_one_grid) {
		const bool tex = Q.albedo_mode != 0u;
		const SsxBlobSpectrum* desc = tex ? reinterpret_cast<const SsxBlobSpectrum*>(L.w + h.off_spectra) + h.spec_basis_r : &Q.albedo;
		const SsxBlobSpectrum sp = *desc;
		const HeroIndex hi = hero_index(h, sp, lambda_0);
		if (!tex) return hero_gather(L, sp.offset, hi);
		float r, g, b;
		texel_lrgb(L, Q.albedo_tex, st_x, st_y, r, g, b);
		Hero br, bg, bb, out;
		hero_gather3(L, h.off_basis4, hi, br, bg, bb);
#pragma unroll
		for (int k = 0; k < 4; ++k) out.v[k] = (r * br.v[k] + g * bg.v[k]) + b * bb.v[k];
		return out;
	}
	if (Q.albedo_mode == 0u) return spectrum_hero(L, Q.albedo, lambda_0, h.lambda_step);
	return texture_sample(L, Q.albedo_tex, st_x, st_y, lambda_0);
}

__device__ __forceinline__ void flux_to_xyz(const Lds& L, const Hero& flux, float lambda_0, float out[3]) {
	const SsxBlobHeader& h = L.hdr();
	Hero bar[3];
	if (h.observer_one_grid) {
		hero_gather3(L, h.off_observer4, hero_index(h, L.spectrum(h.spec_xbar), lambda_0), bar[0], bar[1], bar[2]);
	} else {
		bar[0] = spectrum_hero(L, h.spec_xbar, lambda_0, h.lambda_step);
		bar[1] = spectrum_hero(L, h.spec_ybar, lambda_0, h.lambda_step);
		bar[2] = spectrum_hero(L, h.spec_zbar, lambda_0, h.lambda_step);
	}
#pragma unroll
	for (int ch = 0; ch < 3; ++ch) {
		float acc = 0.0f;
#pragma unroll
		for (int i = 0; i < 4; ++i) acc += (bar[ch].v[i] * flux.v[i]) * h.lambda_step;
		out[ch] = acc;
	}
}

struct RaySetup {
	float okx, oky, okz;
	float Sx, Sy, Sz;
	uint32_t perm;
};

__device__ __forceinline__ RaySetup ray_setup(V3 orig, V3 dir) {
	const float ax = __builtin_fabsf(dir.x), ay = __builtin_fabsf(dir.y), az = __builtin_fabsf(dir.z);
	const bool xy = ax > ay;
	const bool k0 = xy && ax > az;
	const bool k1 = !xy && ay > az;
	const float dkz = k0 ? dir.x : (k1 ? dir.y : dir.z);
	const float da = k0 ? dir.y : dir.x, db = k0 ? dir.z : (k1 ? dir.z : dir.y);
	RaySetup rs;
	const double dkz_recip = ssx_exact::div64_rcp_any(dkz);
	rs.Sx = ssx_exact::div64_by(da, dkz_recip);
	rs.Sy = ssx_exact::div64_by(db, dkz_recip);
	rs.Sz = ssx_exact::div64_by(1.0f, dkz_recip);
	rs.okx = k0 ? orig.y : orig.x; rs.oky = k0 ? orig.z : (k1 ? orig.z : orig.y);
	rs.okz = k0 ? orig.x : (k1 ? orig.y : orig.z);
	rs.perm = k0 ? 0u : (k1 ? 1u : 2u);
	return rs;
}

struct HitInfo {
	int tri;
	float dist;
	float U, V, W, det_recip;
};

__device__ __forceinline__ void load_perm(const float* p, float out[12]) {
	const float4* p4 = reinterpret_cast<const float4*>(p);
// ... 218 lines not shown
	const float denom1 = sin_c * sin_a;
	const float denom2 = sin_a * sin_b;
	const float dsum = (da + db) + dc;
	const bool fast = (dsum == dsum) && denom0 > 0 && denom1 > 0 && denom2 > 0;
	const float cos_alpha = __builtin_amdgcn_fmed3f(numer0 / denom0, -1.0f, 1.0f);
	const float cos_beta  = __builtin_amdgcn_fmed3f(numer1 / denom1, -1.0f, 1.0f);
	const float cos_gamma = __builtin_amdgcn_fmed3f(numer2 / denom2, -1.0f, 1.0f);
	const float alpha = ssx_acos_sin_lds(cos_alpha, under_pi, &sin_alpha, &ok_al);
	if (!ok_al) sin_alpha = ssx_sinf_lds(alpha);
	const float beta  = __builtin_fminf(ssx_acosf_lds(cos_beta ), under_pi);
	const float gamma = __builtin_fminf(ssx_acosf_lds(cos_gamma), under_pi);
	float area = alpha + beta + gamma - SSX_PI_F;
	if (area >= 0); else area = 0;
	t.b = b; t.cos_c = cos_c;
	t.alpha = alpha; t.cos_alpha = cos_alpha; t.sin_alpha = sin_alpha; t.area = area;
	if (!fast) sphtri_make_general(A, B, C, t);
}

__device__ __forceinline__ V3 func_bar(V3 x, V3 y) {
	V3 dir = sub(x, scl(dot3(x, y), y));
	float lensq = dot3(dir, dir);
	if (lensq == 0.0f) return mk(0, 0, 0);
	float is = inversesqrt_(lensq);
	if (lensq < 0x1p-100f) is = 1.0f / __builtin_sqrtf(lensq);
	return mk(dir.x * is, dir.y * is, dir.z * is);
}

template <bool GLIBC = false>
__device__ __forceinline__ V3 rand_toward_sphericaltri(Rng& rng, const SphTri& tri) {
	float r0 = rand_1f(rng);
	float r1 = rand_1f(rng);
	float sin_alpha = tri.sin_alpha;
	float q;
	if (sin_alpha > 0) {
		float random_area = r0 * tri.area;
		float phi = random_area - tri.alpha;
		float s, t;
		if (GLIBC) ssx_glibc_sincosf(phi, &s, &t); else ssx_sincosf(phi, &s, &t);
		float u = t - tri.cos_alpha;
		float v = s + sin_alpha * tri.cos_c;
		float denom = (v * s + u * t) * sin_alpha;
		if (denom != 0.0f) q = ((v * t - u * s) * tri.cos_alpha - v) / denom;
		else q = tri.cos_c;
	} else {
		q = ssx_cosf_lds(tri.b * r0);
	}
	q = clamp_glm(q, -1.0f, 1.0f);
	V3 C_hat = add(scl(q, tri.A), scl(ssx_exact::sqrt_normal(1 - q * q), func_bar(tri.C, tri.A)));
	float z = 1.0f - r1 * (1.0f - dot3(C_hat, tri.B));
	z = clamp_glm(z, -1.0f, 1.0f);
	return add(scl(z, tri.B), scl(ssx_exact::sqrt_normal(1 - z * z), func_bar(C_hat, tri.B)));
}

template <bool GLIBC = false>
__device__ __forceinline__ void sample_light(const Lds& L, Rng& rng, V3 from, V3& dir, uint32_t& light_quad, float& pdf) {
	const uint32_t nl = L.hdr().n_lights;
	uint32_t pick = 0u;
	if (nl == 1u) (void)rng_next(rng); else pick = rand_choice(rng, nl);
	light_quad = L.light(pick);
	const SsxBlobQuad& Q = L.quad(light_quad);
	const bool is_tri = Q.is_tri != 0u;
	bool first = true;
	if (!is_tri) first = rand_1f(rng) <= 0.5f;
	const float* p0 = Q.pos[0];
	const float* p1 = first ? Q.pos[1] : Q.pos[2];
	const float* p2 = first ? Q.pos[2] : Q.pos[3];
	SphTri st;
	sphtri_make<GLIBC>(normalize3_any(sub(mk(p0[0], p0[1], p0[2]), from)),
	            normalize3_any(sub(mk(p1[0], p1[1], p1[2]), from)),
	            normalize3_any(sub(mk(p2[0], p2[1], p2[2]), from)), st);
	dir = rand_toward_sphericaltri<GLIBC>(rng, st);
	pdf = ssx_exact::rcp(st.area);
	if (!is_tri) pdf *= 0.5f;
	pdf = ssx_exact::div64_by(pdf, L.hdr().n_lights_recip);
}

__device__ __forceinline__ void skip_light_draws(const Lds& L, Rng& rng) {
	const uint32_t nl = L.hdr().n_lights;
	uint32_t pick = 0u;
	if (nl == 1u) (void)rng_next(rng); else pick = rand_choice(rng, nl);
	if (L.quad(L.light(pick)).is_tri == 0u) (void)rng_next(rng);
	(void)rng_next(rng); (void)rng_next(rng);
}
__device__ __forceinline__ void skip_coshemi_draws(Rng& rng) {
	float pdf;
	do {
		(void)rng_next(rng);
		pdf = ssx_exact::sqrt_normal(1 - rand_1f(rng));
	} while (pdf <= SSX_EPS);
}

template <bool GLIBC = false>
__device__ __forceinline__ V3 rand_coshemi(Rng& rng, float& pdf) {
	V3 result;
	do {
		float angle = rand_1f(rng) * (2.0f * SSX_PI_F);
		float s, c;
		if (GLIBC) ssx_glibc_sincosf(angle, &s, &c); else ssx_sincosf(angle, &s, &c);
		float radius_sq = rand_1f(rng);
		float radius = ssx_exact::sqrt_normal(radius_sq);
		result = mk(radius * c, ssx_exact::sqrt_normal(1 - radius_sq), radius * s);
		pdf = result.y;
	} while (pdf <= SSX_EPS);
	pdf *= 1.0f / SSX_PI_F;
	return result;
}
__device__ __forceinline__ V3 get_rotated_to(V3 dir, V3 n) {
	float sign = __builtin_copysignf(1.0f, n.z);
	float a = -ssx_exact::rcp(sign + n.z);
	float b = n.x * n.y * a;
	V3 bx = mk(1.0f + sign * n.x * n.x * a, sign * b, -sign * n.x);
	V3 bz = mk(b, sign + n.y * n.y * a, -n.y);
	return add(add(scl(dir.x, bx), scl(dir.y, n)), scl(dir.z, bz));
}
__device__ __forceinline__ V3 reflect3(V3 vec, V3 n) {
	return add(mk(-vec.x, -vec.y, -vec.z), scl(2.0f * dot3(vec, n), n));
}


struct Path {
	Rng rng;
	V3 orig, dir;
	float lambda_0;
	int ignore;
	uint32_t depth;
	uint32_t rec_index;
	uint32_t prev_slot;
	int hit_tri;
	float hit_dist;
	float hit_st_x, hit_st_y;
};

__device__ __forceinline__ float4& log_fs(const SsxKernelArgs& a, uint32_t i) { return *reinterpret_cast<float4*>(a.logs + i * 16u); }
__device__ __forceinline__ float4& log_nee(const SsxKernelArgs& a, uint32_t i) { return *reinterpret_cast<float4*>(a.logs + (a.log_cap * (16u * SSX_MAX_FRAMES) + i * 16u)); }
// ... 9 lines not shown
	__device__ __forceinline__ uint32_t group() const { return tagw & (2u * SSX_UNIT_COHORTS - 1u); }
	__device__ __forceinline__ uint32_t log_rec() const { return (wave_base + ((tagw >> 3) & 7u)) * SSX_COHORT_RECORDS; }
	__device__ __forceinline__ uint32_t rc(uint32_t rec_index) const { return ((tagw >> 8) << 6) | (rec_index & 63u); }
};
__device__ __forceinline__ uint32_t log_tag_word(uint32_t cohort, uint32_t tag, uint32_t unit_cohorts, uint32_t k_in_cohort) {
	return cohort | (tag << 2) | ((tag * unit_cohorts + cohort) << 3) | (k_in_cohort << 8);
}
__device__ __forceinline__ uint32_t log_region(const SsxKernelArgs& a, uint32_t wave_slot, uint32_t tag, uint32_t cohort) {
	return ((wave_slot * 2u + tag) * a.unit_cohorts + cohort) * SSX_COHORT_RECORDS;
}
__device__ __forceinline__ void wave_release(uint32_t* cnt) { (void)__hip_atomic_fetch_add(cnt + 4u * SSX_UNIT_COHORTS, 1u, __ATOMIC_RELEASE, __HIP_MEMORY_SCOPE_WAVEFRONT); }
__device__ __forceinline__ void wave_acquire(uint32_t* cnt) { (void)__hip_atomic_load(cnt + 4u * SSX_UNIT_COHORTS, __ATOMIC_ACQUIRE, __HIP_MEMORY_SCOPE_WAVEFRONT); }
__device__ __forceinline__ uint32_t log_append(const LogRef& lg, uint32_t which) {
	return __hip_atomic_fetch_add(lg.cnt + 2u * lg.group() + which, 1u, __ATOMIC_RELAXED, __HIP_MEMORY_SCOPE_WAVEFRONT);
}
__device__ __forceinline__ uint32_t level_word_none() { return SSX_NO_SLOT << 13; }
__device__ __forceinline__ uint32_t level_word_emission(uint32_t w) { return w | (1u << 26); }
__device__ __forceinline__ uint32_t level_word_nee(uint32_t w, uint32_t nslot) { return (w & ~(SSX_NO_SLOT << 13)) | (nslot << 13); }
__device__ __forceinline__ uint32_t tail_word(uint32_t level_word, uint32_t hit_anything, uint32_t depth, uint32_t prev_slot) {
	return hit_anything | ((level_word >> 26) << 1) | (depth << 2) | (prev_slot << 6) | ((level_word >> 13) << 19);
}
__device__ __forceinline__ void store_emission(const SsxKernelArgs& a, const LogRef& lg, uint32_t depth, uint32_t rec_index, const float (&e)[4]) {
	log_direct(a, lg.log_rec() * SSX_MAX_LEVELS + depth * SSX_COHORT_RECORDS + lg.rc(rec_index)) = make_float4(e[0], e[1], e[2], e[3]);
}
__device__ __forceinline__ uint32_t nee_index(const LogRef& lg, uint32_t nslot) { return lg.log_rec() * SSX_MAX_LEVELS + nslot; }
__device__ __forceinline__ void store_parked_term(const SsxKernelArgs& a, uint32_t ni, const float (&c)[4]) { log_nee(a, ni) = make_float4(c[0], c[1], c[2], c[3]); }
template <bool NARROW>
__device__ __forceinline__ void store_shadow_outcome(const SsxKernelArgs& a, uint32_t ni, bool visible, float c0, float c1, float c2, float c3) {
	if (NARROW) log_vis(a, ni) = visible ? (uint8_t)1 : (uint8_t)0;
	else log_nee(a, ni) = visible ? make_float4(c0, c1, c2, c3) : make_float4(0.0f, 0.0f, 0.0f, 0.0f);
}
__device__ __forceinline__ void store_level_entry(const SsxKernelArgs& a, const LogRef& lg, uint32_t slot, const float (&f_s)[4], float n_dot_l, float pdf, uint32_t prev_slot, uint32_t level_word) {
	const uint32_t entry = lg.log_rec() * SSX_MAX_FRAMES + slot;
	log_fs(a, entry) = make_float4(f_s[0], f_s[1], f_s[2], f_s[3]);
	log_np(a, entry) = make_float2(n_dot_l, pdf);
	log_link(a, entry) = prev_slot | level_word;
}

template <typename Args>
__device__ __forceinline__ void camera_dir(const SsxBlobHeader& h, const Args& a, double x, double y, double& dx, double& dy, double& dz) {
	const bool pow2 = ((a.width & (a.width - 1u)) | (a.height & (a.height - 1u))) == 0u;
	double st_x, st_y;
	if (pow2) { st_x = x * a.inv_width; st_y = y * a.inv_height; }
	else { st_x = x / (double)a.width; st_y = y / (double)a.height; }
	double ndc_x = st_x * 2.0 - 1.0, ndc_y = st_y * 2.0 - 1.0;
	double q[4];
#pragma unroll
	for (int r = 0; r < 4; ++r)
		q[r] = (h.pv_inv[0 * 4 + r] * ndc_x + h.pv_inv[1 * 4 + r] * ndc_y) + h.q_const[r];
	double w = q[3];
	double px = q[0] / w, py = q[1] / w, pz = q[2] / w;
	dx = px - h.cam_pos_d[0]; dy = py - h.cam_pos_d[1]; dz = pz - h.cam_pos_d[2];
}
template <typename Args>
__device__ __forceinline__ void generate_sample(const SsxBlobHeader& h, const Args& a, uint32_t i, uint32_t j, uint32_t k, float4& ray, uint4& st) {
	const uint64_t pixel = (uint64_t)j * (uint64_t)a.width + (uint64_t)i;
	const uint64_t pa = mix64(a.seed + 0x9E3779B97F4A7C15ull * (pixel + 1ull));
	const uint64_t b = mix64(pa + 0x9E3779B97F4A7C15ull * ((uint64_t)k + 1ull));
	Rng rng;
	rng.state = b;
	rng.inc = mix64(b ^ 0xDA3E39CB94B95BDBull) | 1ull;
	double sub_y = rand_1d(rng);
	double sub_x = rand_1d(rng);
	double dx, dy, dz;
	camera_dir(h, a, (double)i + sub_x, (double)j + sub_y, dx, dy, dz);
	double inv = 1.0 / __builtin_sqrt((dx * dx + dy * dy) + dz * dz);
	const float lambda_0 = a.rgb_mode ? 0.0f : h.lambda_min + rand_1f(rng) * h.lambda_step;
	ray = make_float4((float)(dx * inv), (float)(dy * inv), (float)(dz * inv), lambda_0);
	st = make_uint4((uint32_t)rng.state, (uint32_t)(rng.state >> 32), (uint32_t)rng.inc, (uint32_t)(rng.inc >> 32));
}

#define SSX_SQ_FLUSH_AT 64u
#define SSX_SQ_CAPACITY 128u
struct ShadowQ {
	float4* e;
	uint32_t count;
	uint32_t* cnt;
};

__device__ __forceinline__ void hit_st(const SsxBlobQuad& Q, uint32_t which, const HitInfo& hit, float& st_x, float& st_y) {
	float bx = hit.U * hit.det_recip, by = hit.V * hit.det_recip, bz = hit.W * hit.det_recip;
	const float* s0 = Q.st[0];
	const float* s1 = which ? Q.st[2] : Q.st[1];
	const float* s2 = which ? Q.st[3] : Q.st[2];
	st_x = (bx * s0[0] + by * s1[0]) + bz * s2[0];
	st_y = (bx * s0[1] + by * s1[1]) + bz * s2[1];
}

template <int TOPO>
__device__ __forceinline__ void debug_trace_rows(const SsxKernelArgs& a, const uint32_t* in, uint32_t in_words, uint32_t* out, uint32_t out_words, uint32_t n) {
	Lds L; L.w = stage_lds(a);
	const uint32_t gid = blockIdx.x * blockDim.x + threadIdx.x;
	const uint32_t item = gid < n ? gid : n - 1u;
	const uint32_t* x = in + (size_t)item * in_words;
	HitInfo h;
	trace<TOPO>(L, mk(__uint_as_float(x[0]), __uint_as_float(x[1]), __uint_as_float(x[2])), mk(__uint_as_float(x[3]), __uint_as_float(x[4]), __uint_as_float(x[5])),
	            (int)x[6], x[7] != 0u, h);
	uint32_t o[5] = { h.tri < 0 ? 0xFFFFFFFFu : (uint32_t)h.tri >> 1, h.tri < 0 ? 0u : (uint32_t)h.tri & 1u, __float_as_uint(h.dist), 0u, 0u };
	if (h.tri >= 0) { float sx, sy; hit_st(L.quad((uint32_t)h.tri >> 1), (uint32_t)h.tri & 1u, h, sx, sy); o[3] = __float_as_uint(sx); o[4] = __float_as_uint(sy); }
	if (gid < n)
		for (uint32_t k = 0; k < out_words && k < 5u; ++k) out[(size_t)gid * out_words + k] = o[k];
}

template <bool NARROW, bool BLACK, bool GLIBC = false>
__device__ __forceinline__ bool path_step(const Lds& L, const ShadowQ& q, const SsxKernelArgs& a, const LogRef& lg, Path& p, bool& pushed, uint32_t& level_word) {
	const SsxBlobHeader& h = L.hdr();
	level_word = level_word_none();
	SSX_STAT(4);
	const uint32_t hq = (uint32_t)p.hit_tri >> 1, which = (uint32_t)p.hit_tri & 1u;
	const SsxBlobQuad& Q = L.quad(hq);
	const SsxBlobQuad& M = Q;
	V3 N = mk(Q.normal[which][0], Q.normal[which][1], Q.normal[which][2]);

	float direct[4] = { 0.0f, 0.0f, 0.0f, 0.0f };
	const bool els = a.no_els == 0u;
	if ((els ? (p.depth == 0u && !a.indirect_only) : true) && M.is_emissive != 0u) {
		SSX_STAT(5);
		Hero em = spectrum_hero(L, M.emission, p.lambda_0, h.lambda_step);
#pragma unroll
		for (int k = 0; k < 4; ++k) direct[k] += em.v[k];
		store_emission(a, lg, p.depth, p.rec_index, direct);
		level_word = level_word_emission(level_word);
	}
	if (p.depth + 1u >= SSX_MAX_DEPTH_) return false;
	const V3 hit_pos = add(p.orig, scl(p.hit_dist, p.dir));
	p.orig = hit_pos;
	if (M.albedo_mode != 0u) { SSX_STAT(6); } else { SSX_STAT(7); }
	Hero alb = material_albedo(L, Q, p.hit_st_x, p.hit_st_y, p.lambda_0);
	float f_lamb[4];
#pragma unroll
	for (int k = 0; k < 4; ++k) f_lamb[k] = SSX_DIV_CONST(alb.v[k], SSX_PI_F);

	if (BLACK && M.kind == 0u && h.black_ends_path != 0u && f_lamb[0] == 0.0f && f_lamb[1] == 0.0f && f_lamb[2] == 0.0f && f_lamb[3] == 0.0f) {
		SSX_STAT(18);
		if (els && (!a.indirect_only || p.depth > 0u)) skip_light_draws(L, p.rng);
		skip_coshemi_draws(p.rng);
		return false;
	}
	if (els && (!a.indirect_only || p.depth > 0u)) {
		V3 sdir; uint32_t light; float spdf;
		SSX_STAT(8);
		sample_light<GLIBC>(L, p.rng, hit_pos, sdir, light, spdf);
		float n_dot_l = dot3(sdir, N);
		if (n_dot_l > 0.0f) {
			SSX_STAT(9);
			Hero emitted = spectrum_hero(L, L.quad(light).emission, p.lambda_0, h.lambda_step);
			float c[4];
			const double spdf_recip = ssx_exact::div64_rcp_any(spdf);
#pragma unroll
			for (int k = 0; k < 4; ++k) {
				float fs = (M.kind == 0u) ? f_lamb[k] : 0.0f;
				c[k] = ssx_exact::div64_by((emitted.v[k] * n_dot_l) * fs, spdf_recip);
			}
			if (c[0] != 0.0f || c[1] != 0.0f || c[2] != 0.0f || c[3] != 0.0f) {
				SSX_STAT(10);
				const uint64_t pushing = __ballot(1);
				const uint32_t slot = q.count + __builtin_amdgcn_mbcnt_hi((uint32_t)(pushing >> 32), __builtin_amdgcn_mbcnt_lo((uint32_t)pushing, 0u));
				const uint32_t nslot = log_append(lg, 1u);
				const uint32_t ni = nee_index(lg, nslot);
				if (NARROW) {
					store_parked_term(a, ni, c);
					float4* E = q.e + 2u * slot;
					E[0] = make_float4(hit_pos.x, hit_pos.y, hit_pos.z, sdir.x);
					E[1] = make_float4(sdir.y, sdir.z, __uint_as_float((light << 8) | hq), __uint_as_float(ni));
				} else {
					float4* E = q.e + 3u * slot;
					E[0] = make_float4(hit_pos.x, hit_pos.y, hit_pos.z, sdir.x);
					E[1] = make_float4(sdir.y, sdir.z, c[0], c[1]);
					E[2] = make_float4(c[2], c[3], __uint_as_float((light << 8) | hq), __uint_as_float(ni));
				}
				level_word = level_word_nee(level_word, nslot);
				pushed = true;
			}
		}
	}

	V3 w_i; float pdf_w_i; float f_s[4];
	if (M.kind == 0u) {
		SSX_STAT(11);
		w_i = rand_coshemi<GLIBC>(p.rng, pdf_w_i);
		w_i = get_rotated_to(w_i, N);
#pragma unroll
		for (int k = 0; k < 4; ++k) f_s[k] = f_lamb[k];
	} else {
		w_i = reflect3(mk(-p.dir.x, -p.dir.y, -p.dir.z), N);
		pdf_w_i = __builtin_inff();
#pragma unroll
		for (int k = 0; k < 4; ++k) f_s[k] = alb.v[k];
	}
	bool cont = false;
	float n_dot_l = 0.0f;
	float dotfs = (f_s[0] * f_s[0] + f_s[1] * f_s[1]) + (f_s[2] * f_s[2] + f_s[3] * f_s[3]);
	if (dotfs > 0.0f) {
		if (__builtin_isfinite(pdf_w_i)) n_dot_l = dot3(w_i, N);
		else { n_dot_l = 1.0f; pdf_w_i = 1.0f; }
		cont = n_dot_l > 0.0f;
	}
	if (!cont || (els && p.depth + 2u >= SSX_MAX_DEPTH_)) return false;
	SSX_STAT(12);
	const uint32_t slot = log_append(lg, 0u);
	store_level_entry(a, lg, slot, f_s, n_dot_l, pdf_w_i, p.prev_slot, level_word);
	wave_release(lg.cnt);
	p.prev_slot = slot;
	p.dir = w_i; p.ignore = (int)hq;
	++p.depth;
	return true;
}

template <int TOPO, bool NARROW>
__device__ __forceinline__ void shadow_flush(const Lds& L, const SsxKernelArgs& a, const ShadowQ& q, uint32_t first, uint32_t n, SsxTimer& tm) {
	const uint32_t lane = threadIdx.x & 63u;
	const bool have = lane < n;
	const bool narrow = NARROW;
	float4 e0 = make_float4(0.0f, 0.0f, 0.0f, 0.0f), e1 = make_float4(0.0f, 1.0f, 0.0f, 0.0f), e2 = e0;
	if (have) {
		if (narrow) { const float4* E = q.e + 2u * (first + lane); e0 = E[0]; e1 = E[1]; e2.z = e1.z; e2.w = e1.w; }
		else { const float4* E = q.e + 3u * (first + lane); e0 = E[0]; e1 = E[1]; e2 = E[2]; }
	}
	const uint32_t tag = __float_as_uint(e2.z);
	HitInfo sh;
	trace<TOPO>(L, mk(e0.x, e0.y, e0.z), mk(e0.w, e1.x, e1.y), (int)(tag & 0xFFu), have, sh, 2, nullptr, &tm);
	if (have) {
		const bool visible = sh.tri >= 0 && ((uint32_t)sh.tri >> 1) == (tag >> 8);
		store_shadow_outcome<NARROW>(a, __float_as_uint(e2.w), visible, e1.z, e1.w, e2.x, e2.y);
		wave_release(q.cnt);
	}
}

__device__ __forceinline__ const __attribute__((address_space(4))) SsxKernelArgs& cold_args() {
	auto p = __builtin_amdgcn_kernarg_segment_ptr();
	asm volatile("" : "+s"(p));
	return *(const __attribute__((address_space(4))) SsxKernelArgs*)p;
}
__device__ __forceinline__ double ld_agent(const double* p) { return __hip_atomic_load(p, __ATOMIC_RELAXED, __HIP_MEMORY_SCOPE_AGENT); }
__device__ __forceinline__ void st_agent(double* p, double v) { __hip_atomic_store(p, v, __ATOMIC_RELAXED, __HIP_MEMORY_SCOPE_AGENT); }
__device__ __forceinline__ void add_sample(bool rgb_mode, double acc[4], float x, float y, float z, float alpha) {
	if (rgb_mode) { acc[0] += (double)x; acc[1] += (double)y; acc[2] += (double)z; acc[3] += (double)alpha; }
	else { acc[0] += (double)(x * 0.001f); acc[1] += (double)(y * 0.001f); acc[2] += (double)(z * 0.001f); acc[3] += (double)(alpha * 0.001f); }
}
__device__ __forceinline__ void stage_sample(float4* rec, float x, float y, float z, float alpha) {
	uint64_t* const q = reinterpret_cast<uint64_t*>(rec);
	__hip_atomic_store(q, (uint64_t)__float_as_uint(x) | ((uint64_t)__float_as_uint(y) << 32), __ATOMIC_RELAXED, __HIP_MEMORY_SCOPE_AGENT);
	__hip_atomic_store(q + 1, (uint64_t)__float_as_uint(z) | ((uint64_t)__float_as_uint(alpha) << 32), __ATOMIC_RELAXED, __HIP_MEMORY_SCOPE_AGENT);
}
__device__ __forceinline__ void add_staged_sample(bool rgb_mode, double acc[4], const float4* rec) {
	const uint64_t* const q = reinterpret_cast<const uint64_t*>(rec);
	const uint64_t lo = __hip_atomic_load(q, __ATOMIC_RELAXED, __HIP_MEMORY_SCOPE_AGENT), hi = __hip_atomic_load(q + 1, __ATOMIC_RELAXED, __HIP_MEMORY_SCOPE_AGENT);
	add_sample(rgb_mode, acc, __uint_as_float((uint32_t)lo), __uint_as_float((uint32_t)(lo >> 32)), __uint_as_float((uint32_t)hi), __uint_as_float((uint32_t)(hi >> 32)));
}
template <bool NARROW>
__device__ __forceinline__ float4 nee_term(const SsxKernelArgs& a, uint32_t i, bool has) {
	uint32_t v = 1u;
	float4 c = make_float4(0.0f, 0.0f, 0.0f, 0.0f);
	if (has) {
		if (NARROW) v = log_vis(a, i);
		c = log_nee(a, i);
	}
	if (!NARROW) return c;
	return make_float4(v ? c.x : 0.0f, v ? c.y : 0.0f, v ? c.z : 0.0f, v ? c.w : 0.0f);
}
template <uint32_t WAYS, bool NARROW, bool FLUX = false>
__device__ __forceinline__ void resolve_records(const Lds& L, const SsxKernelArgs& a, uint32_t r0, uint32_t stride, uint32_t count, uint32_t fs_base, uint32_t nee_base, uint32_t rc0, double acc[4], bool stage) {
	float rad[WAYS][4];
	uint32_t depth[WAYS];
	uint32_t K[WAYS];
	uint32_t at[WAYS];
	uint32_t top = 0;
	const float4 zero4 = make_float4(0.0f, 0.0f, 0.0f, 0.0f);
#pragma unroll
	for (uint32_t s = 0; s < WAYS; ++s) {
		depth[s] = 0; K[s] = 0; at[s] = 0;
		rad[s][0] = rad[s][1] = rad[s][2] = rad[s][3] = 0.0f;
		if (s < count) {
			const uint32_t y = a.st[r0 + s * stride].y;
			const uint32_t dep = (y >> 2) & 0xFu;
			depth[s] = dep | ((y & 1u) << 4);
			at[s] = (y >> 6) & SSX_NO_SLOT;
			const uint32_t ns = y >> 19;
			float4 last = zero4;
			if ((y >> 1) & 1u) {
				last = log_direct(a, nee_base + dep * SSX_COHORT_RECORDS + rc0 + s * 64u);
				last = make_float4(0.0f + last.x, 0.0f + last.y, 0.0f + last.z, 0.0f + last.w);
			}
			const float4 ne = nee_term<NARROW>(a, nee_base + ns, ns != SSX_NO_SLOT);
			if (dep) K[s] = log_link(a, fs_base + at[s]);
			rad[s][0] = last.x + ne.x; rad[s][1] = last.y + ne.y; rad[s][2] = last.z + ne.z; rad[s][3] = last.w + ne.w;
			top = max(top, dep);
		}
	}
	for (uint32_t d = top; d-- > 0u;) {
		float4 D[WAYS], F[WAYS]; float2 NP[WAYS];
#pragma unroll
		for (uint32_t s = 0; s < WAYS; ++s)
			if (d < (depth[s] & 0xFu)) {
				const uint32_t i = fs_base + at[s];
				F[s] = log_fs(a, i); NP[s] = log_np(a, i);
				const uint32_t ns = (K[s] >> 13) & SSX_NO_SLOT;
				const bool has_ne = ns != SSX_NO_SLOT;
				D[s] = nee_term<NARROW>(a, nee_base + ns, has_ne);
				if ((K[s] >> 26) & 1u) {
					const float4 em = log_direct(a, nee_base + d * SSX_COHORT_RECORDS + rc0 + s * 64u);
					D[s] = make_float4((0.0f + em.x) + D[s].x, (0.0f + em.y) + D[s].y, (0.0f + em.z) + D[s].z, (0.0f + em.w) + D[s].w);
				}
				at[s] = K[s] & SSX_NO_SLOT;
				if (d) K[s] = log_link(a, fs_base + at[s]);
			}
#pragma unroll
		for (uint32_t s = 0; s < WAYS; ++s)
			if (d < (depth[s] & 0xFu)) {
				SSX_STAT(14);
				const double pdf_recip = ssx_exact::div64_rcp_any(NP[s].y);
				rad[s][0] = (0.0f + D[s].x) + ssx_exact::div64_by((rad[s][0] * NP[s].x) * F[s].x, pdf_recip);
				rad[s][1] = (0.0f + D[s].y) + ssx_exact::div64_by((rad[s][1] * NP[s].x) * F[s].y, pdf_recip);
				rad[s][2] = (0.0f + D[s].z) + ssx_exact::div64_by((rad[s][2] * NP[s].x) * F[s].z, pdf_recip);
				rad[s][3] = (0.0f + D[s].w) + ssx_exact::div64_by((rad[s][3] * NP[s].x) * F[s].w, pdf_recip);
			}
	}
	const __attribute__((address_space(4))) SsxKernelArgs& c = cold_args();
	const bool rgb_mode = c.rgb_mode != 0u, keep_samples = c.keep_samples != 0u, no_flat_field = c.no_flat_field != 0u;
#pragma unroll
	for (uint32_t s = 0; s < WAYS; ++s)
		if (s < count) {
			SSX_STAT(15);
			if (no_flat_field) {
				const float4 cr = a.ray[r0 + s * stride];
				const SsxBlobHeader& hh = L.hdr();
				const float d = dot3(mk(cr.x, cr.y, cr.z), mk(hh.cam_dir[0], hh.cam_dir[1], hh.cam_dir[2]));
				rad[s][0] *= d; rad[s][1] *= d; rad[s][2] *= d; rad[s][3] *= d;
			}
			Hero flux; flux.v[0] = rad[s][0]; flux.v[1] = rad[s][1]; flux.v[2] = rad[s][2]; flux.v[3] = rad[s][3];
			if (FLUX) c.flux[r0 + s * stride] = make_float4(rad[s][0], rad[s][1], rad[s][2], rad[s][3]);
			float xyz[3];
			if (rgb_mode) { xyz[0] = rad[s][0]; xyz[1] = rad[s][1]; xyz[2] = rad[s][2]; }
			else flux_to_xyz(L, flux, __uint_as_float(a.st[r0 + s * stride].x), xyz);
			const float alpha = (depth[s] >> 4) ? 1.0f : 0.0f;
			if (stage) stage_sample(a.ray + (r0 + s * stride), xyz[0], xyz[1], xyz[2], alpha);
			else {
				add_sample(rgb_mode, acc, xyz[0], xyz[1], xyz[2], alpha);
				if (keep_samples) a.ray[r0 + s * stride] = make_float4(xyz[0], xyz[1], xyz[2], alpha);
			}
		}
}

}

template <typename Args>
__device__ __forceinline__ uint32_t tile_of_slot(const Args& a, uint32_t slot, uint32_t& tx, uint32_t& ty) {
	const uint32_t t = a.tile_first + slot * a.tile_stride;
	ty = t / a.tiles_x;
	const uint32_t txr = t - ty * a.tiles_x, rot = (ty * a.tile_skew) % a.tiles_x;
	tx = txr >= rot ? txr - rot : txr + a.tiles_x - rot;
	return ty * a.tiles_x + tx;
}
__device__ __forceinline__ void generate_body(const SsxKernelArgs& a) {
	Lds L; L.w = stage_lds(a);
	const SsxBlobHeader& h = L.hdr();
	const V3 cam = mk(h.cam_pos[0], h.cam_pos[1], h.cam_pos[2]);
	const uint32_t n_k = a.k1 - a.k0;
	const uint32_t lane = threadIdx.x & 63u;
	const uint64_t n_waves = a.n_records >> 6;
	for (uint64_t sk = (uint64_t)blockIdx.x * (blockDim.x >> 6) + (threadIdx.x >> 6); sk < n_waves; sk += (uint64_t)gridDim.x * (blockDim.x >> 6)) {
		const uint32_t slot = (uint32_t)(sk / n_k), kk = a.k0 + (uint32_t)(sk % n_k);
		uint32_t tx, ty;
		(void)tile_of_slot(a, slot, tx, ty);
		const uint32_t i = tx * 8u + (lane & 7u), j = ty * 8u + (lane >> 3);
		const bool inside = i < a.width && j < a.height;
		float4 ray = make_float4(0.0f, 0.0f, 1.0f, 0.0f); uint4 st = make_uint4(0u, 0u, 0u, 0u);
		if (inside) generate_sample(h, a, i, j, kk, ray, st);
		const uint64_t r = sk * 64u + lane;
		if (!a.pre_hits) {
			if (inside) { a.ray[r] = ray; a.st[r] = st; }
			continue;
// ... 65 lines not shown
#endif

struct WorkUnit {
	uint32_t slot, grp;
	uint32_t tile;
	uint32_t txy;
	uint32_t dims;
	__device__ __forceinline__ uint32_t tw() const { return dims & 15u; }
	__device__ __forceinline__ uint32_t th() const { return (dims >> 4) & 15u; }
	__device__ __forceinline__ uint32_t n_kq() const { return dims >> 8; }
	__device__ __forceinline__ uint32_t npx() const { return tw() * th(); }
	__device__ __forceinline__ uint32_t n_items() const { return npx() * n_kq(); }
	__device__ __forceinline__ uint32_t k_off(const SsxKernelArgs& a) const { return grp * a.group_spp; }
	__device__ __forceinline__ uint32_t rec_base(const SsxKernelArgs& a) const { return (slot * (a.k1 - a.k0) + grp * a.group_spp) * 64u; }
};
__device__ __forceinline__ void unit_setup(const SsxKernelArgs& hot, uint32_t unit, WorkUnit& u) {
	(void)hot;
	const __attribute__((address_space(4))) SsxKernelArgs& a = cold_args();
	const uint32_t slot = unit % a.my_tiles, grp = unit / a.my_tiles;
	uint32_t tx, ty;
	const uint32_t tile = tile_of_slot(a, slot, tx, ty);
	const uint32_t ka = a.k0 + grp * a.group_spp;
	const uint32_t kb = min(ka + a.group_spp, a.k1);
	u.dims = min(8u, a.width - tx * 8u) | (min(8u, a.height - ty * 8u) << 4) | ((kb - ka) << 8);
	u.slot = slot; u.grp = grp;
	u.tile = tile; u.txy = tx | (ty << 16);
}
__device__ __forceinline__ void sums_release(uint32_t* cnt) {
#ifdef SSX_ACCUM_FORMAL
	wave_release(cnt);
	wave_acquire(cnt);
#else
	(void)cnt;
	__builtin_amdgcn_fence(__ATOMIC_RELEASE, "workgroup");
	asm volatile("s_waitcnt vmcnt(0)" ::: "memory");
#endif
}
__device__ __forceinline__ void sums_acquire(uint32_t* cnt) {
#ifdef SSX_ACCUM_FORMAL
	wave_release(cnt);
	wave_acquire(cnt);
#else
	(void)cnt;
	__builtin_amdgcn_fence(__ATOMIC_ACQUIRE, "workgroup");
#endif
}
#ifdef SSX_ACCUM_FORMAL
#define SSX_SUMS_ACQ __ATOMIC_ACQUIRE
#define SSX_SUMS_ACQ_REL __ATOMIC_ACQ_REL
#else
#define SSX_SUMS_ACQ __ATOMIC_RELAXED
#define SSX_SUMS_ACQ_REL __ATOMIC_RELAXED
#endif
__device__ __forceinline__ void sums_chain(uint32_t slot, uint32_t grp, uint32_t lane, uint32_t* cnt) {
	const __attribute__((address_space(4))) SsxKernelArgs& a = cold_args();
	uint32_t tx, ty;
	const uint32_t tile = tile_of_slot(a, slot, tx, ty);
	const bool has_px = (lane & 7u) < min(8u, a.width - tx * 8u) && (lane >> 3) < min(8u, a.height - ty * 8u);
	double* const px = a.accum + (size_t)tile * 256u + lane;
	uint32_t* state = a.unit_state + (slot * a.n_groups + grp);
	uint32_t rec_at = (slot * (a.k1 - a.k0) + grp * a.group_spp) * 64u;
	double acc[4] = { 0.0, 0.0, 0.0, 0.0 };
	if (has_px) { acc[0] = ld_agent(px); acc[1] = ld_agent(px + 64); acc[2] = ld_agent(px + 128); acc[3] = ld_agent(px + 192); }
	for (;;) {
		const uint32_t n = min(a.group_spp, (a.k1 - a.k0) - grp * a.group_spp);
		if (has_px) {
			for (uint32_t kq = 0; kq < n; ++kq) add_staged_sample(a.rgb_mode != 0u, acc, a.ray + (rec_at + kq * 64u + lane));
			st_agent(px, acc[0]); st_agent(px + 64, acc[1]); st_agent(px + 128, acc[2]); st_agent(px + 192, acc[3]);
		}
		if (++grp >= a.n_groups) return;
		sums_release(cnt);
		++state; rec_at += a.group_spp * 64u;
		uint32_t was = 0u;
		if (lane == 0u) was = __hip_atomic_fetch_or(state, SSX_UNIT_TURN, SSX_SUMS_ACQ_REL, __HIP_MEMORY_SCOPE_AGENT);
		was = (uint32_t)__builtin_amdgcn_readfirstlane((int)was);
		sums_acquire(cnt);
		if (was != SSX_UNIT_PARKED) return;
		if (lane == 0u) atomicAdd(a.unit_counter + 3, 1u);
	}
}
template <bool NARROW, bool FLUX = false>
__device__ __forceinline__ void unit_fold(const Lds& L, const SsxKernelArgs& a, const WorkUnit& u, uint32_t wave_slot, uint32_t tag, uint32_t* cnt) {
	wave_acquire(cnt);
	__builtin_amdgcn_fence(__ATOMIC_RELEASE, "workgroup");
	__builtin_amdgcn_fence(__ATOMIC_ACQUIRE, "agent");
	const uint32_t lane = threadIdx.x & 63u;
	const bool has_px = (lane & 7u) < u.tw() && (lane >> 3) < u.th();
	const __attribute__((address_space(4))) SsxKernelArgs& c = cold_args();
	uint32_t* const state = c.unit_state + (u.slot * c.n_groups + u.grp);
	double* const px = c.accum + (size_t)u.tile * 256u + lane;
	bool mine = true;
	if (u.grp) {
		mine = ((uint32_t)__builtin_amdgcn_readfirstlane((int)__hip_atomic_load(state, SSX_SUMS_ACQ, __HIP_MEMORY_SCOPE_AGENT)) & SSX_UNIT_TURN) != 0u;
		sums_acquire(cnt);
	}
	double acc[4] = { 0.0, 0.0, 0.0, 0.0 };
	if (mine && has_px) { acc[0] = ld_agent(px); acc[1] = ld_agent(px + 64); acc[2] = ld_agent(px + 128); acc[3] = ld_agent(px + 192); }
	if (has_px)
		for (uint32_t kq = 0, n_kq = u.n_kq(), rec_base = u.rec_base(a); kq < n_kq; kq += SSX_COHORT_KS) {
			const uint32_t log_rec = log_region(a, wave_slot, tag, kq / SSX_COHORT_KS);
			resolve_records<SSX_COHORT_KS, NARROW, FLUX>(L, a, rec_base + kq * 64u + lane, 64u, min(SSX_COHORT_KS, n_kq - kq), log_rec * SSX_MAX_FRAMES, log_rec * SSX_MAX_LEVELS, lane, acc, !mine);
		}
	if (mine) {
		if (has_px) { st_agent(px, acc[0]); st_agent(px + 64, acc[1]); st_agent(px + 128, acc[2]); st_agent(px + 192, acc[3]); }
		if (u.grp + 1u >= c.n_groups) return;
		sums_release(cnt);
		uint32_t was = 0u;
		if (lane == 0u) was = __hip_atomic_fetch_or(state + 1, SSX_UNIT_TURN, SSX_SUMS_ACQ_REL, __HIP_MEMORY_SCOPE_AGENT);
		was = (uint32_t)__builtin_amdgcn_readfirstlane((int)was);
		sums_acquire(cnt);
		if (was != SSX_UNIT_PARKED) return;
		if (lane == 0u) atomicAdd(c.unit_counter + 3, 1u);
		sums_chain(u.slot, u.grp + 1u, lane, cnt);
	} else {
		sums_release(cnt);
		uint32_t was = 0u;
		if (lane == 0u) {
			atomicAdd(c.unit_counter + 2, 1u);
			uint32_t expected = 0u;
			(void)__hip_atomic_compare_exchange_strong(state, &expected, SSX_UNIT_PARKED, SSX_SUMS_ACQ_REL, SSX_SUMS_ACQ, __HIP_MEMORY_SCOPE_AGENT);
			was = expected;
		}
		was = (uint32_t)__builtin_amdgcn_readfirstlane((int)was);
		sums_acquire(cnt);
		if (was == SSX_UNIT_TURN) sums_chain(u.slot, u.grp, lane, cnt);
	}
}

template <int TOPO, bool NARROW, bool CALIB = false, bool GLIBC = false, bool FLUX = false>
__device__ __forceinline__ void render_body(const SsxKernelArgs& a) {
	constexpr bool FUSE_GEN = TOPO == 2;
	uint32_t* const lds_words = stage_lds<GLIBC>(a);
	Lds L; L.w = lds_words;

	const uint32_t wave = (uint32_t)__builtin_amdgcn_readfirstlane((int)(threadIdx.x >> 6)), lane = threadIdx.x & 63u;
	const uint32_t wave_slot = blockIdx.x * 4u + wave;
	const SsxBlobHeader& hg = *reinterpret_cast<const SsxBlobHeader*>(a.blob);
	const V3 cam = mk(hg.cam_pos[0], hg.cam_pos[1], hg.cam_pos[2]);

	Path p;
	p.orig = mk(0.0f, 0.0f, 0.0f); p.dir = mk(0.0f, 0.0f, 1.0f); p.ignore = -1; p.depth = 0; p.rec_index = 0; p.lambda_0 = 0.0f; p.prev_slot = SSX_NO_SLOT;
	p.hit_tri = 0; p.hit_dist = 0.0f; p.hit_st_x = p.hit_st_y = 0.0f;
	p.rng.state = 0; p.rng.inc = 1;
	bool active = false;
	uint32_t p_tag = 0;
	constexpr uint32_t queue_words = SSX_QUEUE_ENTRIES * (NARROW ? SSX_QUEUE_WORDS_NARROW : SSX_QUEUE_WORDS_WIDE);
	uint32_t* const log_cnt = lds_words + a.blob_words + 4u * queue_words + wave * SSX_WAVE_COUNTER_WORDS;
	SsxTimer tm;
#ifdef SSX_REGTIME
	tm.acc = reinterpret_cast<unsigned long long*>(lds_words + a.blob_words + 4u * queue_words + 4u * SSX_WAVE_COUNTER_WORDS) + wave * SSX_NTIME;
	if (lane < (uint32_t)SSX_NTIME) tm.acc[lane] = 0ull;
	tm.last = __builtin_amdgcn_s_memtime();
#endif
	ShadowQ sq;
	sq.e = reinterpret_cast<float4*>(lds_words + a.blob_words + wave * queue_words);
	sq.count = 0; sq.cnt = log_cnt;
	WorkUnit cur, old;
	bool cur_valid = false, old_pending = false, more = true;
	uint32_t cur_tag = 0, old_tag = 0;
	uint32_t next_item = 0;
	uint32_t grab = 0;
	auto end_path = [&](uint32_t level_word, uint32_t hit_anything) {
		const uint32_t tail = tail_word(level_word, hit_anything, p.depth, p.prev_slot);
		a.st[p.rec_index] = make_uint4(__float_as_uint(p.lambda_0), tail, (uint32_t)p.rng.state, (uint32_t)(p.rng.state >> 32));
		wave_release(log_cnt);
		active = false;
	};
	auto refill = [&](bool with_hit) {
		const uint32_t n_items = cur.n_items();
		if (!(cur_valid && next_item < n_items)) return;
		const uint64_t idle = __ballot(!active);
		if (!active) {
			const uint32_t item = next_item + __builtin_amdgcn_mbcnt_hi((uint32_t)(idle >> 32), __builtin_amdgcn_mbcnt_lo((uint32_t)idle, 0u));
			if (item < n_items) {
				SSX_STAT(19);
				uint32_t in_tile, kq;
				const uint32_t npx = cur.npx(), tw = cur.tw();
				if (npx == 64u) { in_tile = item & 63u; kq = item >> 6; }
				else { const uint32_t r = item % npx; kq = item / npx; in_tile = (r / tw) * 8u + r % tw; }
				p.rec_index = cur.rec_base(a) + kq * 64u + in_tile;
				float4 ray; uint4 st;
				if (FUSE_GEN && a.fuse_gen) {
					const __attribute__((address_space(4))) SsxKernelArgs& c = cold_args();
					generate_sample(L.hdr(), c, (cur.txy & 0xFFFFu) * 8u + (in_tile & 7u), (cur.txy >> 16) * 8u + (in_tile >> 3), c.k0 + cur.grp * c.group_spp + kq, ray, st);
					if (c.no_flat_field) c.ray[p.rec_index] = ray;
				} else {
					ray = a.ray[p.rec_index];
					st = a.st[p.rec_index];
				}
				p.dir = mk(ray.x, ray.y, ray.z);
				p.lambda_0 = ray.w;
				p.rng.state = ((uint64_t)st.y << 32) | st.x;
				p.rng.inc = ((uint64_t)st.w << 32) | st.z;
				p.orig = cam;
				p.ignore = -1;
				p.depth = 0;
				p.prev_slot = SSX_NO_SLOT;
				const uint32_t cohort = kq / SSX_COHORT_KS;
				p_tag = log_tag_word(cohort, cur_tag, a.unit_cohorts, kq % SSX_COHORT_KS);
				active = true;
				if (with_hit) {
					const float4 ht = a.hit[p.rec_index];
					p.hit_dist = ht.x; p.hit_st_x = ht.y; p.hit_st_y = ht.z; p.hit_tri = __float_as_int(ht.w);
					active = p.hit_tri >= 0;
				}
			}
		}
		next_item = min(n_items, next_item + (uint32_t)__popcll(idle));
	};
	auto flush_fold = [&]() {
		const bool busy = __any(active);
		const bool fold_old = old_pending && !__any(active && ((p_tag >> 2) & 1u) == old_tag);
		const bool drain = (fold_old && a.fuse_resolve) || !busy;
		while (sq.count >= SSX_SQ_FLUSH_AT || (drain && sq.count)) {
			const uint32_t take = min(sq.count, 64u);
			sq.count -= take;
			shadow_flush<TOPO, NARROW>(L, a, sq, sq.count, take, tm);
			SSX_TIME(tm, 5);
		}
		if (fold_old) {
			if (a.fuse_resolve) unit_fold<NARROW, FLUX>(L, a, old, wave_slot, old_tag, log_cnt);
			old_pending = false;
			SSX_TIME(tm, 6);
		}
	};
	auto rotate_fetch = [&]() {
		if (cur_valid && next_item >= cur.n_items() && !old_pending) {
			old = cur; old_tag = cur_tag; old_pending = true;
			cur_valid = false;
		}
		if (!cur_valid && more) {
			const __attribute__((address_space(4))) SsxKernelArgs& c = cold_args();
			uint32_t u = 0;
			const uint32_t total = c.my_tiles * c.n_groups;
			if (TOPO != 1 && ((grab >> 26) & 31u)) { u = grab & 0x3FFFFFFu; grab += 1u - (1u << 26); }
			else {
				const uint32_t single = TOPO != 1 ? grab >> 31 : 1u, want = single ? 1u : c.unit_grab;
				if (lane == 0u) u = atomicAdd(c.unit_counter, want);
				u = (uint32_t)__builtin_amdgcn_readfirstlane((int)u);
				if (u < total) {
					const uint32_t got = min(want, total - u);
					if (TOPO != 1) grab = (u + 1u) | ((got - 1u) << 26) | ((single | (total - u < gridDim.x * 4u * want * 4u ? 1u : 0u)) << 31);
				}
			}
			if (u < total) {
				unit_setup(a, u, cur); cur_tag ^= 1u; next_item = 0; cur_valid = true;
				if (lane < 2u * SSX_UNIT_COHORTS) log_cnt[2u * SSX_UNIT_COHORTS * cur_tag + lane] = 0u;
			}
			else more = false;
		}
	};
	for (;;) {
		{
			bool pushed = false;
			if (active) {
				SSX_STAT(13);
				LogRef lg;
				lg.cnt = log_cnt; lg.wave_base = wave_slot * 2u * a.unit_cohorts; lg.tagw = p_tag;
				uint32_t level_word;
				if (!path_step<NARROW, TOPO != 1, GLIBC>(L, sq, a, lg, p, pushed, level_word)) end_path(level_word, 1u);
			}
			sq.count += (uint32_t)__popcll(__ballot(pushed));
		}
		SSX_TIME(tm, 3);
		rotate_fetch();
		if (!a.pre_hits) refill(false);
		SSX_TIME(tm, 4);
		flush_fold();
		SSX_TIME(tm, 14);
		if (__any(active)) {
			HitInfo hit;
			trace<TOPO>(L, p.orig, p.dir, p.ignore, active, hit, 0, nullptr, &tm);
			p.hit_tri = hit.tri; p.hit_dist = hit.dist;
			float st_x = 0.0f, st_y = 0.0f;
			if (CALIB) { const uint32_t left = (uint32_t)__popcll(__ballot(active && hit.tri < 0)); if (lane == 0u && left) atomicAdd(a.unit_counter + 1, left); }
			if (active) {
				if (hit.tri < 0) end_path(level_word_none(), p.depth ? 1u : 0u);
				else {
					const SsxBlobQuad& Q = L.quad((uint32_t)hit.tri >> 1);
					if (Q.albedo_mode != 0u) hit_st(Q, (uint32_t)hit.tri & 1u, hit, st_x, st_y);
				}
			}
			p.hit_st_x = st_x; p.hit_st_y = st_y;
		}
		SSX_TIME(tm, 9);
		if (a.pre_hits) refill(true);
		SSX_TIME(tm, 10);
		if (!__any(active) && !cur_valid && !more && !old_pending && sq.count == 0u) break;
	}
#ifdef SSX_REGTIME
	if (lane < (uint32_t)SSX_NTIME) atomicAdd(&g_regtime[lane], tm.acc[lane]);
#endif
}

#ifndef SSX_WAVES_PER_EU
#define SSX_WAVES_PER_EU 4
#endif
#ifndef SSX_JIT_GLIBC
#define SSX_JIT_GLIBC 0
#endif
#ifndef SSX_JIT_FLUX
#define SSX_JIT_FLUX 0
#endif
#define SSX_PATH_KERNEL(name, topo, narrow, glibc, flux) \
	extern "C" __global__ void __launch_bounds__(256) __attribute__((amdgpu_waves_per_eu(SSX_WAVES_PER_EU))) name(SsxKernelArgs a) { render_body<topo, narrow, false, glibc, flux>(a); }
#ifdef SSX_JIT_BUILD
#ifdef SSX_JIT_DEBUG
extern "C" __global__ void __launch_bounds__(256) ssx_debug_trace_jit(SsxKernelArgs a, const uint32_t* in, uint32_t in_words, uint32_t* out, uint32_t out_words, uint32_t n) {
	debug_trace_rows<3>(a, in, in_words, out, out_words, n);
}
#else
SSX_PATH_KERNEL(ssx_render_kernel_jit, 3, false, SSX_JIT_GLIBC, SSX_JIT_FLUX)
SSX_PATH_KERNEL(ssx_render_kernel_jit_nq, 3, true, SSX_JIT_GLIBC, SSX_JIT_FLUX)
#endif
#else
SSX_PATH_KERNEL(ssx_render_kernel, 0, false, false, false)
SSX_PATH_KERNEL(ssx_render_kernel_cornell, 1, false, false, false)
#ifndef SSX_PROBE_BUILD
SSX_PATH_KERNEL(ssx_render_kernel_plane, 2, false, false, false)
SSX_PATH_KERNEL(ssx_render_kernel_nq, 0, true, false, false)
SSX_PATH_KERNEL(ssx_render_kernel_cornell_nq, 1, true, false, false)
SSX_PATH_KERNEL(ssx_render_kernel_plane_nq, 2, true, false, false)
SSX_PATH_KERNEL(ssx_render_kernel_glibc, 0, false, true, false)
SSX_PATH_KERNEL(ssx_render_kernel_cornell_glibc, 1, false, true, false)
SSX_PATH_KERNEL(ssx_render_kernel_plane_glibc, 2, false, true, false)
SSX_PATH_KERNEL(ssx_render_kernel_nq_glibc, 0, true, true, false)
SSX_PATH_KERNEL(ssx_render_kernel_cornell_nq_glibc, 1, true, true, false)
SSX_PATH_KERNEL(ssx_render_kernel_plane_nq_glibc, 2, true, true, false)
SSX_PATH_KERNEL(ssx_render_kernel_flux, 0, false, false, true)
SSX_PATH_KERNEL(ssx_render_kernel_cornell_flux, 1, false, false, true)
SSX_PATH_KERNEL(ssx_render_kernel_plane_flux, 2, false, false, true)
SSX_PATH_KERNEL(ssx_render_kernel_nq_flux, 0, true, false, true)
SSX_PATH_KERNEL(ssx_render_kernel_cornell_nq_flux, 1, true, false, true)
SSX_PATH_KERNEL(ssx_render_kernel_plane_nq_flux, 2, true, false, true)
#endif
extern "C" __global__ void __launch_bounds__(256) __attribute__((amdgpu_waves_per_eu(3))) ssx_calibrate_kernel(SsxKernelArgs a) { render_body<0, true, true>(a); }
#endif

#ifndef SSX_JIT_BUILD
#include "ssx_pixel_grid.h"
extern "C" __global__ void __launch_bounds__(256) ssx_finalize_kernel(const double* accum, float4* out, SsxPixelGrid g, uint32_t spp, uint32_t rgb_mode, uint32_t done_tiles) {
	const uint32_t p = blockIdx.x * blockDim.x + threadIdx.x;
	if (p >= g.width * g.height) return;
	const uint32_t i = p % g.width, j = p / g.width;
	const uint32_t tile = ssx_shared_tile(g, i, j);
	float4 o = make_float4(0.0f, 0.0f, 0.0f, 0.0f);
	if (tile % g.tile_stride == g.tile_first && tile / g.tile_stride < done_tiles) {
		const double* const px = accum + ssx_sum_slot(i, j, g.tiles_x);
		if (rgb_mode) {
			const double n = (double)spp;
			o.x = (float)(px[0] / n);
			o.y = (float)(px[64] / n);
			o.z = (float)(px[128] / n);
			o.w = (float)(px[192] / n);
		} else {
			const double sc = 1000.0 / (double)spp;
			o.x = (float)(px[0] * sc);
			o.y = (float)(px[64] * sc);
			o.z = (float)(px[128] * sc);
			o.w = (float)(px[192] * sc);
		}
	}
	out[p] = o;
}

extern "C" __global__ void __launch_bounds__(256) ssx_sum_kernel(float4* dst, const float4* src, uint32_t n) {
	const uint32_t p = blockIdx.x * blockDim.x + threadIdx.x;
	if (p >= n) return;
	const float4 a = dst[p], b = src[p];
	dst[p] = make_float4(a.x + b.x, a.y + b.y, a.z + b.z, a.w + b.w);
}
#endif
```

simple_spectral_amd/renderer.py:

```python
import ctypes as C
import os
from dataclasses import dataclass, field
from typing import Optional, Tuple

import numpy as np

from . import _capi

ROOT = os.path.dirname(os.path.dirname(os.path.abspath(__file__)))
DEFAULT_DATA_DIR = os.path.join(ROOT, "data")


class SsxError(RuntimeError):
    def __init__(self, code, message):
        super().__init__("ssx error %d: %s" % (code, message))
        self.code = code


def _host(fn, *args):
    host = _capi.host_lib()
    rc = getattr(host, fn)(*args)
    if rc != 0:
        raise SsxError(rc, host.ssh_last_error().decode())

# ... 1165 lines not shown
        self._check(self._lib.ssx_debug_fold(self._ctx, C.byref(self.params(**over)), n_pixels, int(spp), x.ctypes.data, int(order_seed) & 0xFFFFFFFF, int(bool(parked)),
                                             None if fl is None else fl.ctypes.data, xyza.ctypes.data, sums.ctypes.data))
        return fl, xyza, sums

    def debug_step(self, rows, n_rounds, **over):
        x = np.ascontiguousarray(rows, dtype=np.uint32)
        if x.ndim != 2 or x.shape[1] != _capi.SSX_STEP_ROW_WORDS:
            raise ValueError("debug_step: rows must be [n, %d] words" % _capi.SSX_STEP_ROW_WORDS)
        out = np.zeros((x.shape[0], _capi.SSX_STEP_OUT_WORDS), dtype=np.uint32)
        self._check(self._lib.ssx_debug_step(self._ctx, C.byref(self.params(**over)), x.shape[0], int(n_rounds), x.ctypes.data, out.ctypes.data))
        return out

    def debug_spectral_accumulate(self, flux, lambda_0, bins, lambda_min, lambda_step, n_k=None, tile_first=0, tile_stride=1, tile_skew=0, moments=True):
        flux, lambda_0 = np.ascontiguousarray(flux, dtype=np.float32), np.ascontiguousarray(lambda_0, dtype=np.float32)
        if flux.ndim != 4 or flux.shape[3] != 4 or lambda_0.shape != flux.shape[:3]:
            raise ValueError("debug_spectral_accumulate: flux must have shape [H, W, K, 4], lambda_0 [H, W, K]")
        H, W, K = lambda_0.shape
        n_k = np.ascontiguousarray([K] if n_k is None else n_k, dtype=np.uint32)
        if n_k.ndim != 1 or int(n_k.astype(np.uint64).sum()) != K:
            raise ValueError("debug_spectral_accumulate: the launch lengths n_k must add up to K = %d" % K)
        B = int(bins)
        sums, counts = np.zeros((H, W, B), dtype=np.float64), np.zeros((H, W, max(B // 4, 1)), dtype=np.uint32)
        q = np.zeros((H, W, B), dtype=np.float64) if moments else None
        self._check(self._lib.ssx_debug_spectral_accumulate(self._ctx, W, H, B, int(tile_first), int(tile_stride), int(tile_skew), float(lambda_min), float(lambda_step),
                                                            len(n_k), n_k.ctypes.data, flux.ctypes.data, lambda_0.ctypes.data, sums.ctypes.data, counts.ctypes.data,
                                                            None if q is None else q.ctypes.data))
        return sums, counts, q

    def set_timing(self, enable=True):
        self._check(self._lib.ssx_set_timing(self._ctx, int(enable)))

    def get_timing(self):
        ms = (C.c_float * 4)()
        self._check(self._lib.ssx_get_timing(self._ctx, ms))
        return dict(zip(("generate", "path", "resolve", "accumulate"), [float(x) for x in ms]))

    def kernel_info(self):
        v = [C.c_int() for _ in range(5)]
        self._check(self._lib.ssx_kernel_info(self._ctx, *[C.byref(x) for x in v]))
        return dict(zip(("vgprs", "sgprs", "lds_bytes", "scratch_bytes", "max_blocks_per_cu"), [x.value for x in v]))

    def plan_info(self):
        f, k = C.c_float(), C.c_int()
        self._check(self._lib.ssx_plan_info(self._ctx, C.byref(f), C.byref(k)))
        variant = {0: "generic", 1: "cornell topology", 2: "plane topology", 3: "scene topology (compiled at upload)"}.get(self._lib.ssx_kernel_variant(self._ctx), "?")
        name = self._lib.ssx_kernel_name(self._ctx)
        left, pre = C.c_float(), C.c_int()
        if hasattr(self._lib, "ssx_calibration_info"):
            self._check(self._lib.ssx_calibration_info(self._ctx, None, C.byref(left), C.byref(pre)))
        fused = (not pre.value) and variant == "plane topology" and not (os.environ.get("SSX_DEBUG_ENV") == "1" and os.environ.get("SSX_FUSE_GEN", "")[:1] == "0")
        return {"frames_per_sample": round(f.value, 3), "fold": "path kernel", "pass1": variant,
                "rays_left_per_sample": round(left.value, 3), "camera_rays": "pre-traced (generate kernel)" if pre.value else "path loop",
                "samples_made_in": "path kernel (refill)" if fused else "generate kernel",
                "kernel": name.decode() if name else None}

    def scratch_info(self):
        a, b = C.c_uint64(), C.c_uint64()
        if hasattr(self._lib, "ssx_scratch_info"):
            self._check(self._lib.ssx_scratch_info(self._ctx, C.byref(a), C.byref(b)))
        return {"sample_bytes": a.value, "log_bytes": b.value}

    def sums_info(self):
        a, b = C.c_uint64(), C.c_uint64()
        if hasattr(self._lib, "ssx_sums_info"):
            self._check(self._lib.ssx_sums_info(self._ctx, C.byref(a), C.byref(b)))
        u = C.c_uint64()
        if hasattr(self._lib, "ssx_units_info"):
            self._check(self._lib.ssx_units_info(self._ctx, C.byref(u)))
        return {"units_parked": a.value, "units_chained": b.value, "units": u.value}

    def save(self, path):
        fb = np.ascontiguousarray(self.framebuffer, dtype=np.float32)
        _host("ssh_save_image", path.encode(), fb.ctypes.data, fb.shape[1], fb.shape[0])

    def close(self):
        if self._ctx:
            self._lib.ssx_destroy(self._ctx)
            self._ctx = C.c_void_p()

    def __del__(self):
        try:
            self.close()
        except Exception:
            pass
```

Before: 3051.

## Add plain kernel variant with runtime switches compiled out for default renders

```diff
diff --git a/include/ssx.h b/include/ssx.h
--- a/include/ssx.h
+++ b/include/ssx.h
@@ -162,6 +162,12 @@
 int ssx_jit_status(ssx_ctx* ctx, int wait_ms, char* message, size_t message_size);
 void ssx_jit_counters(uint64_t* compiled, uint64_t* disk_hits);
 const char* ssx_kernel_name(ssx_ctx* ctx);
+enum { SSX_TRAIT_INDIRECT_ONLY = 1u, SSX_TRAIT_NO_ELS = 2u, SSX_TRAIT_MIRROR = 4u, SSX_TRAIT_TRI_LIGHT = 8u, SSX_TRAIT_UPLIFT = 16u,
+       SSX_TRAIT_RGB_MODE = 32u, SSX_TRAIT_NO_FLAT_FIELD = 64u, SSX_TRAIT_KEEP_SAMPLES = 128u,
+       SSX_TRAIT_LIBM = 256u, SSX_TRAIT_SPECTRAL_BINS = 512u, SSX_TRAIT_FORCED_OFF = 1024u };
+int ssx_scene_traits(const ssx_scene_desc* scene);
+int ssx_render_traits(const ssx_render_params* params);
+int ssx_switches_info(ssx_ctx* ctx);
 
 
 int ssx_render_continue(ssx_ctx* ctx, uint32_t spp_more);
diff --git a/simple_spectral_amd/_capi.py b/simple_spectral_amd/_capi.py
--- a/simple_spectral_amd/_capi.py
+++ b/simple_spectral_amd/_capi.py
@@ -123,6 +123,8 @@
 SSX_OK, SSX_ERR_DATA, SSX_ERR_ARG, SSX_ERR_SCENE, SSX_ERR_DEVICE, SSX_ERR_STATE = 0, -1, -2, -3, -10, -11
 SSX_ABI_VERSION = 2
 SSX_JIT_OFF, SSX_JIT_AT_UPLOAD, SSX_JIT_BACKGROUND = 0, 1, 2
+(SSX_TRAIT_INDIRECT_ONLY, SSX_TRAIT_NO_ELS, SSX_TRAIT_MIRROR, SSX_TRAIT_TRI_LIGHT, SSX_TRAIT_UPLIFT, SSX_TRAIT_RGB_MODE, SSX_TRAIT_NO_FLAT_FIELD,
+ SSX_TRAIT_KEEP_SAMPLES, SSX_TRAIT_LIBM, SSX_TRAIT_SPECTRAL_BINS, SSX_TRAIT_FORCED_OFF) = (1 << i for i in range(11))
 SSX_JIT_STATE_NONE, SSX_JIT_STATE_GENERIC_MEANWHILE, SSX_JIT_STATE_SPECIALISED, SSX_JIT_STATE_FAILED = 0, 1, 2, -1
 
 HIP_SYMBOLS = ["ssx_create", "ssx_destroy", "ssx_upload_scene", "ssx_render_start", "ssx_render_stop",
@@ -145,7 +147,8 @@
                "ssx_defocus_images", "ssx_spectral_develop_lens",
                "ssx_sensor_images", "ssx_demosaic_images", "ssx_spectral_develop_sensor",
                "ssx_debug_tile_mask", "ssx_debug_spectral_accumulate", "ssx_debug_fold", "ssx_debug_step",
-               "ssx_debug_generate", "ssx_generate_info"]
+               "ssx_debug_generate", "ssx_generate_info",
+               "ssx_scene_traits", "ssx_render_traits", "ssx_switches_info"]
 SSX_GENERATE_FILL_BYTE = 0xA6
 SSX_FOLD_ROW_WORDS, SSX_FOLD_LAMBDA0, SSX_FOLD_CAM_DIR, SSX_FOLD_HIT, SSX_FOLD_N, SSX_FOLD_LEVEL0, SSX_FOLD_LEVEL_WORDS = 160, 0, 1, 4, 5, 10, 15
 SSX_FOLD_L_FS, SSX_FOLD_L_NDL, SSX_FOLD_L_PDF, SSX_FOLD_L_FLAGS, SSX_FOLD_L_EMISSION, SSX_FOLD_L_NEE = 0, 4, 5, 6, 7, 11
@@ -435,5 +438,9 @@
         lib.ssx_kernel_variant.argtypes = [vp]
         lib.ssx_kernel_name.argtypes = [vp]
         lib.ssx_kernel_name.restype = C.c_char_p
+        if hasattr(lib, "ssx_switches_info"):
+            lib.ssx_switches_info.argtypes = [vp]
+            lib.ssx_scene_traits.argtypes = [vp]
+            lib.ssx_render_traits.argtypes = [vp]
         _hip = lib
     return _hip
diff --git a/simple_spectral_amd/csrc/ssx_api.hip b/simple_spectral_amd/csrc/ssx_api.hip
--- a/simple_spectral_amd/csrc/ssx_api.hip
+++ b/simple_spectral_amd/csrc/ssx_api.hip
@@ -81,6 +81,7 @@
 	std::vector<DeviceBuffer> d_textures;
 	DeviceBuffer d_jh_data;
 	bool rgb_mode = false;
+	uint32_t scene_traits = 0;
 	bool fuse_resolve = true;
 	float calib_frames = 0.0f;
 	float calib_left = 0.0f;
@@ -234,6 +235,27 @@
 
 struct LaunchPlan { SsxKernelArgs args; uint32_t max_spp_per_launch; };
 
+uint32_t scene_traits_of(const ssx_scene_desc* s) {
+	uint32_t t = 0;
+	for (uint32_t q = 0; q < s->n_quads; ++q) if (s->quads[q].material < s->n_materials && s->materials[s->quads[q].material].kind != SSX_MTL_LAMBERTIAN) t |= SSX_TRAIT_MIRROR;
+	for (uint32_t i = 0; i < s->n_lights; ++i) if (s->lights[i] < s->n_quads && (s->quads[s->lights[i]].flags & SSX_PRIM_TRI)) t |= SSX_TRAIT_TRI_LIGHT;
+	if (s->uplift == SSX_MODE_RGB) t |= SSX_TRAIT_RGB_MODE;
+	else if (s->uplift != SSX_UPLIFT_OURS) t |= SSX_TRAIT_UPLIFT;
+	return t;
+}
+uint32_t render_traits_of(const ssx_render_params* p, bool keep_samples) {
+	return (p->indirect_only ? SSX_TRAIT_INDIRECT_ONLY : 0u) | (p->no_explicit_light_sampling ? SSX_TRAIT_NO_ELS : 0u) |
+	       (p->no_flat_field_correction ? SSX_TRAIT_NO_FLAT_FIELD : 0u) | (keep_samples ? SSX_TRAIT_KEEP_SAMPLES : 0u) | (p->libm != SSX_LIBM_BUILD ? SSX_TRAIT_LIBM : 0u);
+}
+uint32_t traits_of(const ssx_ctx* ctx, const ssx_render_params* p, bool keep_samples) {
+	const char* e = debug_env("SSX_PLAIN_KERNEL");
+	return ctx->scene_traits | render_traits_of(p, keep_samples) | (ctx->spectral_bins ? SSX_TRAIT_SPECTRAL_BINS : 0u) | (e && e[0] == '0' ? SSX_TRAIT_FORCED_OFF : 0u);
+}
+uint32_t variant_of(const ssx_ctx* ctx, const ssx_render_params* p, bool keep_samples = false) {
+	if (ctx->spectral_bins && p->libm == SSX_LIBM_BUILD && !ctx->rgb_mode) return ssx_jit::kVariantFlux;
+	return traits_of(ctx, p, keep_samples) == 0u ? (uint32_t)ssx_jit::kVariantPlain : p->libm;
+}
+
 LaunchPlan make_plan(ssx_ctx* ctx, const ssx_render_params* p, bool ask_device = true) {
 	LaunchPlan pl{};
 	SsxKernelArgs& a = pl.args;
@@ -379,7 +401,9 @@
 	{ { SSX_PK(ssx_render_kernel_glibc), SSX_PK(ssx_render_kernel_nq_glibc) }, { SSX_PK(ssx_render_kernel_cornell_glibc), SSX_PK(ssx_render_kernel_cornell_nq_glibc) },
 	  { SSX_PK(ssx_render_kernel_plane_glibc), SSX_PK(ssx_render_kernel_plane_nq_glibc) } },
 	{ { SSX_PK(ssx_render_kernel_flux), SSX_PK(ssx_render_kernel_nq_flux) }, { SSX_PK(ssx_render_kernel_cornell_flux), SSX_PK(ssx_render_kernel_cornell_nq_flux) },
-	  { SSX_PK(ssx_render_kernel_plane_flux), SSX_PK(ssx_render_kernel_plane_nq_flux) } } };
+	  { SSX_PK(ssx_render_kernel_plane_flux), SSX_PK(ssx_render_kernel_plane_nq_flux) } },
+	{ { SSX_PK(ssx_render_kernel_plain), SSX_PK(ssx_render_kernel_nq_plain) }, { SSX_PK(ssx_render_kernel_cornell_plain), SSX_PK(ssx_render_kernel_cornell_nq_plain) },
+	  { SSX_PK(ssx_render_kernel_plane_plain), SSX_PK(ssx_render_kernel_plane_nq_plain) } } };
 #undef SSX_PK
 static const char* const kJitKernelNames[2] = { "ssx_render_kernel_jit", "ssx_render_kernel_jit_nq" };
 const PathKernel& path_kernel_of(const ssx_ctx* ctx, bool narrow) { return kPathKernels[ctx->variant][ctx->topology < 3u ? ctx->topology : 0u][narrow]; }
@@ -463,6 +487,8 @@
 int launch_batch(ssx_ctx* ctx, Batch& b, hipStream_t stream) {
 	if (b.rc) return b.rc;
 	int rc;
+	if (ctx->variant == ssx_jit::kVariantPlain && (b.a.indirect_only | b.a.no_els | b.a.no_flat_field | b.a.rgb_mode | b.a.keep_samples | ctx->scene_traits))
+		return fail(ctx, SSX_ERR_STATE, "internal: a render with a switch set was about to launch the kernel with the switches compiled in");
 	if (ctx->timing) { if ((rc = timing_events(ctx, &b.tev))) return rc; SSX_HIP(ctx, hipEventRecord(b.tev[0], stream)); }
 	b.a.fuse_gen = fuses_generate(ctx, b.a) ? 1u : 0u;
 	if (!b.a.fuse_gen && (rc = enqueue_generate(ctx, b, stream))) return rc;
@@ -509,8 +535,8 @@
 	return SSX_OK;
 }
 
-int ready_to_launch(ssx_ctx* ctx, const ssx_render_params* p, bool need_out) {
-	const uint32_t variant = (ctx->spectral_bins && p->libm == SSX_LIBM_BUILD && !ctx->rgb_mode) ? ssx_jit::kVariantFlux : p->libm;
+int ready_to_launch(ssx_ctx* ctx, const ssx_render_params* p, bool need_out, bool keep_samples = false) {
+	const uint32_t variant = variant_of(ctx, p, keep_samples);
 	const int rc = ensure_libm_kernels(ctx, variant);
 	if (rc) return rc;
 	ctx->libm = p->libm;
@@ -852,6 +878,7 @@
 	if (s->uplift != SSX_MODE_RGB && s->uplift != SSX_UPLIFT_OURS && s->uplift != SSX_UPLIFT_JH && s->uplift != SSX_UPLIFT_MENG)
 		return fail(ctx, SSX_ERR_SCENE, "unsupported uplift variant (0 = RGB mode, 1 = basis, 2 = Meng et al., 3 = Jakob-Hanika)");
 	ctx->rgb_mode = (s->uplift == SSX_MODE_RGB);
+	ctx->scene_traits = scene_traits_of(s);
 	ctx->d_jh_data.release();
 	if (s->uplift == SSX_UPLIFT_MENG) {
 		const ssx_meng_grid* g = s->meng;
@@ -894,17 +921,20 @@
 	int rc = pack_blob(s, tex, ctx->d_jh_data.ptr, blob, pack_err, -1, &info);
 	if (rc) return fail(ctx, rc, pack_err);
 	const int jit_mode = env_on("SSX_JIT_PASS1") ? SSX_JIT_AT_UPLOAD : ctx->jit_mode;
+	ssx_render_params defaults{};
+	const uint32_t upload_variant = variant_of(ctx, &defaults) == ssx_jit::kVariantPlain ? (uint32_t)ssx_jit::kVariantPlain : (uint32_t)SSX_LIBM_BUILD;
+	if (ctx->variant == SSX_LIBM_BUILD || ctx->variant == ssx_jit::kVariantPlain) ctx->variant = upload_variant;
 	if (info.candidate && jit_mode != SSX_JIT_OFF) {
 		std::string err;
 		const ssx_jit::Kernels* k = nullptr;
-		ssx_jit::State st = ssx_jit::lookup(ctx->device, info.vid, &k, &err);
+		ssx_jit::State st = ssx_jit::lookup(ctx->device, info.vid, &k, &err, upload_variant);
 		if (st != ssx_jit::State::Ready && st != ssx_jit::State::Failed && jit_mode == SSX_JIT_AT_UPLOAD) {
-			k = ssx_jit::get(ctx->device, info.vid, &err);
+			k = ssx_jit::get(ctx->device, info.vid, &err, upload_variant);
 			st = k ? ssx_jit::State::Ready : ssx_jit::State::Failed;
 		}
 		if (st == ssx_jit::State::Failed) { ctx->jit_state = SSX_JIT_STATE_FAILED; ctx->jit_message = err; }
 		else if ((rc = pack_blob(s, tex, ctx->d_jh_data.ptr, blob_jit, pack_err, 3))) return fail(ctx, rc, pack_err);
-		else if (st == ssx_jit::State::Ready) { blob.swap(blob_jit); blob_jit.clear(); ctx->jit_kernels[SSX_LIBM_BUILD] = k; ctx->jit_vid = info.vid; ctx->jit_state = SSX_JIT_STATE_SPECIALISED; }
+		else if (st == ssx_jit::State::Ready) { blob.swap(blob_jit); blob_jit.clear(); ctx->jit_kernels[upload_variant] = k; ctx->jit_vid = info.vid; ctx->jit_state = SSX_JIT_STATE_SPECIALISED; }
 		else { ctx->jit_pending = true; ctx->jit_vid = info.vid; ctx->jit_state = SSX_JIT_STATE_GENERIC_MEANWHILE; ctx->jit_requested = (st == ssx_jit::State::Pending); }
 	}
 	if (ctx->jit_pending) {
@@ -962,7 +992,7 @@
 	(void)hipStreamIsCapturing(stream, &capture);
 	const bool capturing = capture == hipStreamCaptureStatusActive;
 	if (ctx->device_pending && capturing) return fail(ctx, SSX_ERR_STATE, "a render of this context may still be queued: ssx_render_device_wait before capturing another into a graph");
-	if (capturing && ctx->variant != p->libm) return fail(ctx, SSX_ERR_STATE, "ssx_render_params.libm differs from the context's last render: run it once outside the stream capture first");
+	if (capturing && ctx->variant != variant_of(ctx, p)) return fail(ctx, SSX_ERR_STATE, "ssx_render_params.libm differs from the context's last render: run it once outside the stream capture first");
 	if (ctx->device_pending) SSX_HIP(ctx, hipStreamWaitEvent(stream, ctx->ev_device_done, 0));
 	{
 		LaunchPlan probe = make_plan(ctx, p, !capturing);
@@ -1154,7 +1184,7 @@
 	if ((rc = spectral_refuses(ctx, pp, false))) return rc;
 	SSX_HIP(ctx, hipSetDevice(ctx->device));
 	if ((rc = wait_device_pending(ctx))) return rc;
-	if ((rc = ready_to_launch(ctx, p, false))) return rc;
+	if ((rc = ready_to_launch(ctx, p, false, true))) return rc;
 	LaunchPlan pl = make_plan(ctx, p);
 	if (p->spp > pl.max_spp_per_launch) return fail(ctx, SSX_ERR_ARG, "ssx_debug_samples: too many samples for one launch");
 	if ((rc = ensure_samples(ctx, pl, p->spp))) return rc;
@@ -1475,7 +1505,18 @@
 	uint32_t qw = 0;
 	if (pick_queue(ctx, ctx->path_blob_words, &qw, nullptr) != SSX_OK) return nullptr;
 	const bool narrow = qw == SSX_QUEUE_WORDS_NARROW;
-	return ctx->topology == 3u ? kJitKernelNames[narrow] : path_kernel_of(ctx, narrow).name;
+	const uint32_t named = ctx->variant == ssx_jit::kVariantPlain ? (uint32_t)SSX_LIBM_BUILD : ctx->variant;
+	return ctx->topology == 3u ? kJitKernelNames[narrow] : kPathKernels[named][ctx->topology][narrow].name;
+}
+
+int ssx_switches_info(ssx_ctx* ctx) { return (ctx && ctx->have_scene) ? (ctx->variant == ssx_jit::kVariantPlain ? 1 : 0) : -1; }
+int ssx_scene_traits(const ssx_scene_desc* s) {
+	if (!s || s->struct_size != sizeof(ssx_scene_desc) || (s->n_quads && (!s->quads || !s->materials)) || (s->n_lights && !s->lights)) return -1;
+	return (int)scene_traits_of(s);
+}
+int ssx_render_traits(const ssx_render_params* p) {
+	if (!p || p->struct_size != sizeof(ssx_render_params)) return -1;
+	return (int)render_traits_of(p, false);
 }
 
 int ssx_plan_info(ssx_ctx* ctx, float* frames_per_sample, int* fold_in_path_kernel) {
diff --git a/simple_spectral_amd/csrc/ssx_jit.h b/simple_spectral_amd/csrc/ssx_jit.h
--- a/simple_spectral_amd/csrc/ssx_jit.h
+++ b/simple_spectral_amd/csrc/ssx_jit.h
@@ -160,17 +160,18 @@
 };
 inline Shared& shared() { static Shared* s = new Shared; return *s; }
 
-constexpr uint32_t kVariantFlux = 2, kVariants = 3;
-constexpr uint32_t kVariantDebug = 3;
+constexpr uint32_t kVariantFlux = 2, kVariantPlain = 3, kVariants = 4;
+constexpr uint32_t kVariantDebug = 4;
 inline std::string pattern_key(const VidTable& vids, uint32_t libm = 0) {
 	std::string key;
 	if (libm == 1u) key = "libm=glibc-2.35|";
 	if (libm == kVariantFlux) key = "flux|";
+	if (libm == kVariantPlain) key = "plain|";
 	if (libm == kVariantDebug) key = "debug|";
 	for (const auto& r : vids) key.append(reinterpret_cast<const char*>(r.data()), 4);
 	return key;
 }
-inline const char* libm_flag(uint32_t libm) { return libm == kVariantDebug ? "-DSSX_JIT_DEBUG=1" : libm == kVariantFlux ? "-DSSX_JIT_FLUX=1" : libm ? "-DSSX_JIT_GLIBC=1" : nullptr; }
+inline const char* libm_flag(uint32_t libm) { return libm == kVariantDebug ? "-DSSX_JIT_DEBUG=1" : libm == kVariantFlux ? "-DSSX_JIT_FLUX=1" : libm == kVariantPlain ? "-DSSX_JIT_PLAIN=1" : libm ? "-DSSX_JIT_GLIBC=1" : nullptr; }
 
 inline const char* const* compile_flags(size_t* n) {
 	static const char* const flags[] = { "--offload-arch=gfx950", "-O3", "-std=c++17", "-ffp-contract=off", "-fno-slp-vectorize", "-DSSX_JIT_BUILD",
diff --git a/simple_spectral_amd/csrc/ssx_kernels.hip b/simple_spectral_amd/csrc/ssx_kernels.hip
--- a/simple_spectral_amd/csrc/ssx_kernels.hip
+++ b/simple_spectral_amd/csrc/ssx_kernels.hip
@@ -309,13 +309,16 @@
 	r = L.lut(px[0]); g = L.lut(px[1]); b = L.lut(px[2]);
 }
 
+template <bool PLAIN = false>
 __device__ __forceinline__ Hero texture_sample(const Lds& L, uint32_t tex_index, float st_x, float st_y, float lambda_0) {
 	float r, g, b;
 	texel_lrgb(L, tex_index, st_x, st_y, r, g, b);
 	const SsxBlobHeader& h = L.hdr();
-	if (h.uplift == 0u) { Hero o; o.v[0] = r; o.v[1] = g; o.v[2] = b; o.v[3] = 0.0f; return o; }
-	if (h.uplift == 3u) return jh_uplift(L, r, g, b, lambda_0);
-	if (h.uplift == 2u) return meng_uplift(L, r, g, b, lambda_0);
+	if constexpr (!PLAIN) {
+		if (h.uplift == 0u) { Hero o; o.v[0] = r; o.v[1] = g; o.v[2] = b; o.v[3] = 0.0f; return o; }
+		if (h.uplift == 3u) return jh_uplift(L, r, g, b, lambda_0);
+		if (h.uplift == 2u) return meng_uplift(L, r, g, b, lambda_0);
+	}
 	Hero br, bg, bb;
 	const SsxBlobSpectrum sr = L.spectrum(h.spec_basis_r), sg = L.spectrum(h.spec_basis_g), sb = L.spectrum(h.spec_basis_b);
 	if (h.basis_one_grid) {
@@ -331,9 +334,10 @@
 	return out;
 }
 
+template <bool PLAIN = false>
 __device__ __forceinline__ Hero material_albedo(const Lds& L, const SsxBlobQuad& Q, float st_x, float st_y, float lambda_0) {
 	const SsxBlobHeader& h = L.hdr();
-	if (h.uplift == 1u && h.basis_one_grid) {
+	if ((PLAIN || h.uplift == 1u) && h.basis_one_grid) {
 		const bool tex = Q.albedo_mode != 0u;
 		const SsxBlobSpectrum* desc = tex ? reinterpret_cast<const SsxBlobSpectrum*>(L.w + h.off_spectra) + h.spec_basis_r : &Q.albedo;
 		const SsxBlobSpectrum sp = *desc;
@@ -348,7 +352,7 @@
 		return out;
 	}
 	if (Q.albedo_mode == 0u) return spectrum_hero(L, Q.albedo, lambda_0, h.lambda_step);
-	return texture_sample(L, Q.albedo_tex, st_x, st_y, lambda_0);
+	return texture_sample<PLAIN>(L, Q.albedo_tex, st_x, st_y, lambda_0);
 }
 
 __device__ __forceinline__ void flux_to_xyz(const Lds& L, const Hero& flux, float lambda_0, float out[3]) {
@@ -673,14 +677,14 @@
 	return add(scl(z, tri.B), scl(ssx_exact::sqrt_normal(1 - z * z), func_bar(C_hat, tri.B)));
 }
 
-template <bool GLIBC = false>
+template <bool GLIBC = false, bool PLAIN = false>
 __device__ __forceinline__ void sample_light(const Lds& L, Rng& rng, V3 from, V3& dir, uint32_t& light_quad, float& pdf) {
 	const uint32_t nl = L.hdr().n_lights;
 	uint32_t pick = 0u;
 	if (nl == 1u) (void)rng_next(rng); else pick = rand_choice(rng, nl);
 	light_quad = L.light(pick);
 	const SsxBlobQuad& Q = L.quad(light_quad);
-	const bool is_tri = Q.is_tri != 0u;
+	const bool is_tri = !PLAIN && Q.is_tri != 0u;
 	bool first = true;
 	if (!is_tri) first = rand_1f(rng) <= 0.5f;
 	const float* p0 = Q.pos[0];
@@ -696,11 +700,12 @@
 	pdf = ssx_exact::div64_by(pdf, L.hdr().n_lights_recip);
 }
 
+template <bool PLAIN = false>
 __device__ __forceinline__ void skip_light_draws(const Lds& L, Rng& rng) {
 	const uint32_t nl = L.hdr().n_lights;
 	uint32_t pick = 0u;
 	if (nl == 1u) (void)rng_next(rng); else pick = rand_choice(rng, nl);
-	if (L.quad(L.light(pick)).is_tri == 0u) (void)rng_next(rng);
+	if (PLAIN || L.quad(L.light(pick)).is_tri == 0u) (void)rng_next(rng);
 	(void)rng_next(rng); (void)rng_next(rng);
 }
 __device__ __forceinline__ void skip_coshemi_draws(Rng& rng) {
@@ -816,7 +821,7 @@
 	double px = q[0] / w, py = q[1] / w, pz = q[2] / w;
 	dx = px - h.cam_pos_d[0]; dy = py - h.cam_pos_d[1]; dz = pz - h.cam_pos_d[2];
 }
-template <typename Args>
+template <bool PLAIN = false, typename Args>
 __device__ __forceinline__ void generate_sample(const SsxBlobHeader& h, const Args& a, uint32_t i, uint32_t j, uint32_t k, float4& ray, uint4& st) {
 	const uint64_t pixel = (uint64_t)j * (uint64_t)a.width + (uint64_t)i;
 	const uint64_t pa = mix64(a.seed + 0x9E3779B97F4A7C15ull * (pixel + 1ull));
@@ -829,7 +834,7 @@
 	double dx, dy, dz;
 	camera_dir(h, a, (double)i + sub_x, (double)j + sub_y, dx, dy, dz);
 	double inv = 1.0 / __builtin_sqrt((dx * dx + dy * dy) + dz * dz);
-	const float lambda_0 = a.rgb_mode ? 0.0f : h.lambda_min + rand_1f(rng) * h.lambda_step;
+	const float lambda_0 = (!PLAIN && a.rgb_mode) ? 0.0f : h.lambda_min + rand_1f(rng) * h.lambda_step;
 	ray = make_float4((float)(dx * inv), (float)(dy * inv), (float)(dz * inv), lambda_0);
 	st = make_uint4((uint32_t)rng.state, (uint32_t)(rng.state >> 32), (uint32_t)rng.inc, (uint32_t)(rng.inc >> 32));
 }
@@ -866,7 +871,7 @@
 		for (uint32_t k = 0; k < out_words && k < 5u; ++k) out[(size_t)gid * out_words + k] = o[k];
 }
 
-template <bool NARROW, bool BLACK, bool GLIBC = false>
+template <bool NARROW, bool BLACK, bool GLIBC = false, bool PLAIN = false>
 __device__ __forceinline__ bool path_step(const Lds& L, const ShadowQ& q, const SsxKernelArgs& a, const LogRef& lg, Path& p, bool& pushed, uint32_t& level_word) {
 	const SsxBlobHeader& h = L.hdr();
 	level_word = level_word_none();
@@ -877,8 +882,9 @@
 	V3 N = mk(Q.normal[which][0], Q.normal[which][1], Q.normal[which][2]);
 
 	float direct[4] = { 0.0f, 0.0f, 0.0f, 0.0f };
-	const bool els = a.no_els == 0u;
-	if ((els ? (p.depth == 0u && !a.indirect_only) : true) && M.is_emissive != 0u) {
+	const bool els = PLAIN || a.no_els == 0u, indirect_only = !PLAIN && a.indirect_only != 0u;
+	const bool lambert = PLAIN || M.kind == 0u;
+	if ((els ? (p.depth == 0u && !indirect_only) : true) && M.is_emissive != 0u) {
 		SSX_STAT(5);
 		Hero em = spectrum_hero(L, M.emission, p.lambda_0, h.lambda_step);
 #pragma unroll
@@ -890,21 +896,21 @@
 	const V3 hit_pos = add(p.orig, scl(p.hit_dist, p.dir));
 	p.orig = hit_pos;
 	if (M.albedo_mode != 0u) { SSX_STAT(6); } else { SSX_STAT(7); }
-	Hero alb = material_albedo(L, Q, p.hit_st_x, p.hit_st_y, p.lambda_0);
+	Hero alb = material_albedo<PLAIN>(L, Q, p.hit_st_x, p.hit_st_y, p.lambda_0);
 	float f_lamb[4];
 #pragma unroll
 	for (int k = 0; k < 4; ++k) f_lamb[k] = SSX_DIV_CONST(alb.v[k], SSX_PI_F);
 
-	if (BLACK && M.kind == 0u && h.black_ends_path != 0u && f_lamb[0] == 0.0f && f_lamb[1] == 0.0f && f_lamb[2] == 0.0f && f_lamb[3] == 0.0f) {
+	if (BLACK && lambert && h.black_ends_path != 0u && f_lamb[0] == 0.0f && f_lamb[1] == 0.0f && f_lamb[2] == 0.0f && f_lamb[3] == 0.0f) {
 		SSX_STAT(18);
-		if (els && (!a.indirect_only || p.depth > 0u)) skip_light_draws(L, p.rng);
+		if (els && (!indirect_only || p.depth > 0u)) skip_light_draws<PLAIN>(L, p.rng);
 		skip_coshemi_draws(p.rng);
 		return false;
 	}
-	if (els && (!a.indirect_only || p.depth > 0u)) {
+	if (els && (!indirect_only || p.depth > 0u)) {
 		V3 sdir; uint32_t light; float spdf;
 		SSX_STAT(8);
-		sample_light<GLIBC>(L, p.rng, hit_pos, sdir, light, spdf);
+		sample_light<GLIBC, PLAIN>(L, p.rng, hit_pos, sdir, light, spdf);
 		float n_dot_l = dot3(sdir, N);
 		if (n_dot_l > 0.0f) {
 			SSX_STAT(9);
@@ -913,7 +919,7 @@
 			const double spdf_recip = ssx_exact::div64_rcp_any(spdf);
 #pragma unroll
 			for (int k = 0; k < 4; ++k) {
-				float fs = (M.kind == 0u) ? f_lamb[k] : 0.0f;
+				float fs = lambert ? f_lamb[k] : 0.0f;
 				c[k] = ssx_exact::div64_by((emitted.v[k] * n_dot_l) * fs, spdf_recip);
 			}
 			if (c[0] != 0.0f || c[1] != 0.0f || c[2] != 0.0f || c[3] != 0.0f) {
@@ -940,7 +946,7 @@
 	}
 
 	V3 w_i; float pdf_w_i; float f_s[4];
-	if (M.kind == 0u) {
+	if (lambert) {
 		SSX_STAT(11);
 		w_i = rand_coshemi<GLIBC>(p.rng, pdf_w_i);
 		w_i = get_rotated_to(w_i, N);
@@ -1023,7 +1029,7 @@
 	if (!NARROW) return c;
 	return make_float4(v ? c.x : 0.0f, v ? c.y : 0.0f, v ? c.z : 0.0f, v ? c.w : 0.0f);
 }
-template <uint32_t WAYS, bool NARROW, bool FLUX = false>
+template <uint32_t WAYS, bool NARROW, bool FLUX = false, bool PLAIN = false>
 __device__ __forceinline__ void resolve_records(const Lds& L, const SsxKernelArgs& a, uint32_t r0, uint32_t stride, uint32_t count, uint32_t fs_base, uint32_t nee_base, uint32_t rc0, double acc[4], bool stage) {
 	float rad[WAYS][4];
 	uint32_t depth[WAYS];
@@ -1081,7 +1087,7 @@
 			}
 	}
 	const __attribute__((address_space(4))) SsxKernelArgs& c = cold_args();
-	const bool rgb_mode = c.rgb_mode != 0u, keep_samples = c.keep_samples != 0u, no_flat_field = c.no_flat_field != 0u;
+	const bool rgb_mode = !PLAIN && c.rgb_mode != 0u, keep_samples = !PLAIN && c.keep_samples != 0u, no_flat_field = !PLAIN && c.no_flat_field != 0u;
 #pragma unroll
 	for (uint32_t s = 0; s < WAYS; ++s)
 		if (s < count) {
@@ -1253,6 +1259,7 @@
 #define SSX_SUMS_ACQ __ATOMIC_RELAXED
 #define SSX_SUMS_ACQ_REL __ATOMIC_RELAXED
 #endif
+template <bool PLAIN = false>
 __device__ __forceinline__ void sums_chain(uint32_t slot, uint32_t grp, uint32_t lane, uint32_t* cnt) {
 	const __attribute__((address_space(4))) SsxKernelArgs& a = cold_args();
 	uint32_t tx, ty;
@@ -1266,7 +1273,7 @@
 	for (;;) {
 		const uint32_t n = min(a.group_spp, (a.k1 - a.k0) - grp * a.group_spp);
 		if (has_px) {
-			for (uint32_t kq = 0; kq < n; ++kq) add_staged_sample(a.rgb_mode != 0u, acc, a.ray + (rec_at + kq * 64u + lane));
+			for (uint32_t kq = 0; kq < n; ++kq) add_staged_sample(!PLAIN && a.rgb_mode != 0u, acc, a.ray + (rec_at + kq * 64u + lane));
 			st_agent(px, acc[0]); st_agent(px + 64, acc[1]); st_agent(px + 128, acc[2]); st_agent(px + 192, acc[3]);
 		}
 		if (++grp >= a.n_groups) return;
@@ -1280,7 +1287,7 @@
 		if (lane == 0u) atomicAdd(a.unit_counter + 3, 1u);
 	}
 }
-template <bool NARROW, bool FLUX = false>
+template <bool NARROW, bool FLUX = false, bool PLAIN = false>
 __device__ __forceinline__ void unit_fold(const Lds& L, const SsxKernelArgs& a, const WorkUnit& u, uint32_t wave_slot, uint32_t tag, uint32_t* cnt) {
 	wave_acquire(cnt);
 	__builtin_amdgcn_fence(__ATOMIC_RELEASE, "workgroup");
@@ -1300,7 +1307,7 @@
 	if (has_px)
 		for (uint32_t kq = 0, n_kq = u.n_kq(), rec_base = u.rec_base(a); kq < n_kq; kq += SSX_COHORT_KS) {
 			const uint32_t log_rec = log_region(a, wave_slot, tag, kq / SSX_COHORT_KS);
-			resolve_records<SSX_COHORT_KS, NARROW, FLUX>(L, a, rec_base + kq * 64u + lane, 64u, min(SSX_COHORT_KS, n_kq - kq), log_rec * SSX_MAX_FRAMES, log_rec * SSX_MAX_LEVELS, lane, acc, !mine);
+			resolve_records<SSX_COHORT_KS, NARROW, FLUX, PLAIN>(L, a, rec_base + kq * 64u + lane, 64u, min(SSX_COHORT_KS, n_kq - kq), log_rec * SSX_MAX_FRAMES, log_rec * SSX_MAX_LEVELS, lane, acc, !mine);
 		}
 	if (mine) {
 		if (has_px) { st_agent(px, acc[0]); st_agent(px + 64, acc[1]); st_agent(px + 128, acc[2]); st_agent(px + 192, acc[3]); }
@@ -1312,7 +1319,7 @@
 		sums_acquire(cnt);
 		if (was != SSX_UNIT_PARKED) return;
 		if (lane == 0u) atomicAdd(c.unit_counter + 3, 1u);
-		sums_chain(u.slot, u.grp + 1u, lane, cnt);
+		sums_chain<PLAIN>(u.slot, u.grp + 1u, lane, cnt);
 	} else {
 		sums_release(cnt);
 		uint32_t was = 0u;
@@ -1324,11 +1331,11 @@
 		}
 		was = (uint32_t)__builtin_amdgcn_readfirstlane((int)was);
 		sums_acquire(cnt);
-		if (was == SSX_UNIT_TURN) sums_chain(u.slot, u.grp, lane, cnt);
-	}
-}
-
-template <int TOPO, bool NARROW, bool CALIB = false, bool GLIBC = false, bool FLUX = false>
+		if (was == SSX_UNIT_TURN) sums_chain<PLAIN>(u.slot, u.grp, lane, cnt);
+	}
+}
+
+template <int TOPO, bool NARROW, bool CALIB = false, bool GLIBC = false, bool FLUX = false, bool PLAIN = false>
 __device__ __forceinline__ void render_body(const SsxKernelArgs& a) {
 	constexpr bool FUSE_GEN = TOPO == 2;
 	uint32_t* const lds_words = stage_lds<GLIBC>(a);
@@ -1383,8 +1390,8 @@
 				float4 ray; uint4 st;
 				if (FUSE_GEN && a.fuse_gen) {
 					const __attribute__((address_space(4))) SsxKernelArgs& c = cold_args();
-					generate_sample(L.hdr(), c, (cur.txy & 0xFFFFu) * 8u + (in_tile & 7u), (cur.txy >> 16) * 8u + (in_tile >> 3), c.k0 + cur.grp * c.group_spp + kq, ray, st);
-					if (c.no_flat_field) c.ray[p.rec_index] = ray;
+					generate_sample<PLAIN>(L.hdr(), c, (cur.txy & 0xFFFFu) * 8u + (in_tile & 7u), (cur.txy >> 16) * 8u + (in_tile >> 3), c.k0 + cur.grp * c.group_spp + kq, ray, st);
+					if (!PLAIN && c.no_flat_field) c.ray[p.rec_index] = ray;
 				} else {
 					ray = a.ray[p.rec_index];
 					st = a.st[p.rec_index];
@@ -1420,7 +1427,7 @@
 			SSX_TIME(tm, 5);
 		}
 		if (fold_old) {
-			if (a.fuse_resolve) unit_fold<NARROW, FLUX>(L, a, old, wave_slot, old_tag, log_cnt);
+			if (a.fuse_resolve) unit_fold<NARROW, FLUX, PLAIN>(L, a, old, wave_slot, old_tag, log_cnt);
 			old_pending = false;
 			SSX_TIME(tm, 6);
 		}
@@ -1459,7 +1466,7 @@
 				LogRef lg;
 				lg.cnt = log_cnt; lg.wave_base = wave_slot * 2u * a.unit_cohorts; lg.tagw = p_tag;
 				uint32_t level_word;
-				if (!path_step<NARROW, TOPO != 1, GLIBC>(L, sq, a, lg, p, pushed, level_word)) end_path(level_word, 1u);
+				if (!path_step<NARROW, TOPO != 1, GLIBC, PLAIN>(L, sq, a, lg, p, pushed, level_word)) end_path(level_word, 1u);
 			}
 			sq.count += (uint32_t)__popcll(__ballot(pushed));
 		}
@@ -1503,37 +1510,48 @@
 #ifndef SSX_JIT_FLUX
 #define SSX_JIT_FLUX 0
 #endif
-#define SSX_PATH_KERNEL(name, topo, narrow, glibc, flux) \
-	extern "C" __global__ void __launch_bounds__(256) __attribute__((amdgpu_waves_per_eu(SSX_WAVES_PER_EU))) name(SsxKernelArgs a) { render_body<topo, narrow, false, glibc, flux>(a); }
+#ifndef SSX_JIT_PLAIN
+#define SSX_JIT_PLAIN 0
+#endif
+#define SSX_PATH_KERNEL(name, topo, narrow, glibc, flux, plain) \
+	extern "C" __global__ void __launch_bounds__(256) __attribute__((amdgpu_waves_per_eu(SSX_WAVES_PER_EU))) name(SsxKernelArgs a) { render_body<topo, narrow, false, glibc, flux, plain>(a); }
 #ifdef SSX_JIT_BUILD
 #ifdef SSX_JIT_DEBUG
 extern "C" __global__ void __launch_bounds__(256) ssx_debug_trace_jit(SsxKernelArgs a, const uint32_t* in, uint32_t in_words, uint32_t* out, uint32_t out_words, uint32_t n) {
 	debug_trace_rows<3>(a, in, in_words, out, out_words, n);
 }
 #else
-SSX_PATH_KERNEL(ssx_render_kernel_jit, 3, false, SSX_JIT_GLIBC, SSX_JIT_FLUX)
-SSX_PATH_KERNEL(ssx_render_kernel_jit_nq, 3, true, SSX_JIT_GLIBC, SSX_JIT_FLUX)
+SSX_PATH_KERNEL(ssx_render_kernel_jit, 3, false, SSX_JIT_GLIBC, SSX_JIT_FLUX, SSX_JIT_PLAIN)
+SSX_PATH_KERNEL(ssx_render_kernel_jit_nq, 3, true, SSX_JIT_GLIBC, SSX_JIT_FLUX, SSX_JIT_PLAIN)
 #endif
 #else
-SSX_PATH_KERNEL(ssx_render_kernel, 0, false, false, false)
-SSX_PATH_KERNEL(ssx_render_kernel_cornell, 1, false, false, false)
+SSX_PATH_KERNEL(ssx_render_kernel, 0, false, false, false, false)
+SSX_PATH_KERNEL(ssx_render_kernel_cornell, 1, false, false, false, false)
+SSX_PATH_KERNEL(ssx_render_kernel_plain, 0, false, false, false, true)
+SSX_PATH_KERNEL(ssx_render_kernel_cornell_plain, 1, false, false, false, true)
+#if !defined(SSX_PROBE_BUILD) || defined(SSX_PROBE_PLANE)
+SSX_PATH_KERNEL(ssx_render_kernel_plane, 2, false, false, false, false)
+SSX_PATH_KERNEL(ssx_render_kernel_plane_plain, 2, false, false, false, true)
+#endif
 #ifndef SSX_PROBE_BUILD
-SSX_PATH_KERNEL(ssx_render_kernel_plane, 2, false, false, false)
-SSX_PATH_KERNEL(ssx_render_kernel_nq, 0, true, false, false)
-SSX_PATH_KERNEL(ssx_render_kernel_cornell_nq, 1, true, false, false)
-SSX_PATH_KERNEL(ssx_render_kernel_plane_nq, 2, true, false, false)
-SSX_PATH_KERNEL(ssx_render_kernel_glibc, 0, false, true, false)
-SSX_PATH_KERNEL(ssx_render_kernel_cornell_glibc, 1, false, true, false)
-SSX_PATH_KERNEL(ssx_render_kernel_plane_glibc, 2, false, true, false)
-SSX_PATH_KERNEL(ssx_render_kernel_nq_glibc, 0, true, true, false)
-SSX_PATH_KERNEL(ssx_render_kernel_cornell_nq_glibc, 1, true, true, false)
-SSX_PATH_KERNEL(ssx_render_kernel_plane_nq_glibc, 2, true, true, false)
-SSX_PATH_KERNEL(ssx_render_kernel_flux, 0, false, false, true)
-SSX_PATH_KERNEL(ssx_render_kernel_cornell_flux, 1, false, false, true)
-SSX_PATH_KERNEL(ssx_render_kernel_plane_flux, 2, false, false, true)
-SSX_PATH_KERNEL(ssx_render_kernel_nq_flux, 0, true, false, true)
-SSX_PATH_KERNEL(ssx_render_kernel_cornell_nq_flux, 1, true, false, true)
-SSX_PATH_KERNEL(ssx_render_kernel_plane_nq_flux, 2, true, false, true)
+SSX_PATH_KERNEL(ssx_render_kernel_nq, 0, true, false, false, false)
+SSX_PATH_KERNEL(ssx_render_kernel_cornell_nq, 1, true, false, false, false)
+SSX_PATH_KERNEL(ssx_render_kernel_plane_nq, 2, true, false, false, false)
+SSX_PATH_KERNEL(ssx_render_kernel_nq_plain, 0, true, false, false, true)
+SSX_PATH_KERNEL(ssx_render_kernel_cornell_nq_plain, 1, true, false, false, true)
+SSX_PATH_KERNEL(ssx_render_kernel_plane_nq_plain, 2, true, false, false, true)
+SSX_PATH_KERNEL(ssx_render_kernel_glibc, 0, false, true, false, false)
+SSX_PATH_KERNEL(ssx_render_kernel_cornell_glibc, 1, false, true, false, false)
+SSX_PATH_KERNEL(ssx_render_kernel_plane_glibc, 2, false, true, false, false)
+SSX_PATH_KERNEL(ssx_render_kernel_nq_glibc, 0, true, true, false, false)
+SSX_PATH_KERNEL(ssx_render_kernel_cornell_nq_glibc, 1, true, true, false, false)
+SSX_PATH_KERNEL(ssx_render_kernel_plane_nq_glibc, 2, true, true, false, false)
+SSX_PATH_KERNEL(ssx_render_kernel_flux, 0, false, false, true, false)
+SSX_PATH_KERNEL(ssx_render_kernel_cornell_flux, 1, false, false, true, false)
+SSX_PATH_KERNEL(ssx_render_kernel_plane_flux, 2, false, false, true, false)
+SSX_PATH_KERNEL(ssx_render_kernel_nq_flux, 0, true, false, true, false)
+SSX_PATH_KERNEL(ssx_render_kernel_cornell_nq_flux, 1, true, false, true, false)
+SSX_PATH_KERNEL(ssx_render_kernel_plane_nq_flux, 2, true, false, true, false)
 #endif
 extern "C" __global__ void __launch_bounds__(256) __attribute__((amdgpu_waves_per_eu(3))) ssx_calibrate_kernel(SsxKernelArgs a) { render_body<0, true, true>(a); }
 #endif
diff --git a/simple_spectral_amd/renderer.py b/simple_spectral_amd/renderer.py
--- a/simple_spectral_amd/renderer.py
+++ b/simple_spectral_amd/renderer.py
@@ -1241,7 +1241,8 @@
         return {"frames_per_sample": round(f.value, 3), "fold": "path kernel", "pass1": variant,
                 "rays_left_per_sample": round(left.value, 3), "camera_rays": "pre-traced (generate kernel)" if pre.value else "path loop",
                 "samples_made_in": "path kernel (refill)" if fused else "generate kernel",
-                "kernel": name.decode() if name else None}
+                "kernel": name.decode() if name else None,
+                "switches": "compiled in" if hasattr(self._lib, "ssx_switches_info") and self._lib.ssx_switches_info(self._ctx) == 1 else "run time"}
 
     def scratch_info(self):
         a, b = C.c_uint64(), C.c_uint64()
```

Result: faster. 3107 (median of 6 runs) (+1.8%).
